# vlc-robot/robot-3dlotus

Measured on AMD Instinct MI355X. Metric: keystep-samples/sec (train fwd+bwd) 3D-LOTUS GemBench, higher is better.
Workload: dtype f32; 1 GPU; 3D-LOTUS v1 (68.18M params), 16 key-step clouds x 4096 pts per GPU, fwd+loss+bwd, train mode (dropout on), fp32 exact (MFMA f32); global_batch=16, parallelism=dp1, rccl_ranks=0

## Files before the change

### include/lotus_hip.h

```cpp
#ifndef LOTUS_HIP_H
#define LOTUS_HIP_H
#include <stddef.h>
#ifdef __cplusplus
extern "C" {
#endif

#define LOTUS_OK 0
#define LOTUS_E_ARG (-1)
#define LOTUS_E_LAUNCH (-2)
#define LOTUS_E_UNSUPPORTED (-3)
#define LOTUS_E_WORKSPACE (-4)
#ifdef LOTUS_ACT_BF16
typedef unsigned short lotus_act_t;
#else
typedef float lotus_act_t;
#endif

#define LOTUS_ACT_NONE 0
#define LOTUS_ACT_GELU 1
#define LOTUS_ACT_LEAKY 2

const char* lotus_last_error(void);
int lotus_abi_version(void);

unsigned long long lotus_streamlink_create(int nevents);
int lotus_streamlink_wait(unsigned long long link, void* from_stream, void* to_stream);
int lotus_streamlink_destroy(unsigned long long link);

int lotus_comm_load(const char* path);
int lotus_comm_version(void);
int lotus_comm_unique_id(void* id128_host);
unsigned long long lotus_comm_create(const void* id128_host, int nranks, int rank);
int lotus_comm_allreduce(unsigned long long comm, void* buf, size_t count, int dtype, int op, void* stream);
int lotus_comm_destroy(unsigned long long comm);
int lotus_stream_probe(void* blocked, void* other, int timeout_ms);


int lotus_fe_grid(const float* coord, long ld, int n, float grid_size, int* grid, int* gmax, unsigned* scratch,
                  void* stream);
int lotus_fe_encode(const int* grid, const int* batch, int n, const int* gmax, const int* perm4, int depth_bound,
                    int* state, long long* code, long slot_stride, void* stream);
size_t lotus_fe_sort_workspace(int n_max);
int lotus_fe_sort(const long long* code, long slot_stride, const int* n_ptr, int n_max, int key_bits,
                  long long* skeys, int* order, int* inverse, void* workspace, size_t workspace_bytes, void* stream);
int lotus_fe_pool(const long long* pcode, const long long* skey0, const int* order0, const int* pgrid,
                  const int* pbatch, const int* n_ptr, int n_max, const int* perm4, int nbatch, int* cluster,
                  int* seg_start, int* n_child, long long* ccode, int* cgrid, int* cbatch, int* ccounts,
                  int* n_dup, void* stream);
int lotus_fe_pool_coord(const float* pcoord, const int* order0, const int* seg_start, int n_child, float* ccoord,
                        void* stream);
int lotus_fe_patch(const int* order, const int* off, const int* offp, int B, int K, int npad, int* gidx, int* owner,
                   int* kext, int* ext_pos, void* stream);
size_t lotus_fe_neighbours_workspace(int n);
int lotus_fe_neighbours(const int* grid, const int* batch, int n, int ksize, int* nbr, void* workspace,
                        size_t workspace_bytes, void* stream);
size_t lotus_fe_tap_plan_ints(int n);
int lotus_fe_tap_plan(const int* nbr27, const int* rowidx, int n, int* plan, void* stream);

size_t lotus_linear_workspace(int M, int N, int K);
size_t lotus_splitk_counters_bytes(void);
int lotus_linear_fwd(const lotus_act_t* x, const float* w, const float* bias, const lotus_act_t* residual, lotus_act_t* y,
                     lotus_act_t* pre, int M, int N, int K, int act, float drop_p, unsigned long long drop_seed,
                     int precision, void* workspace, size_t workspace_bytes, void* counters, void* stream);
int lotus_linear_dgrad(const lotus_act_t* dy, const float* w, lotus_act_t* dx, const lotus_act_t* pre, const lotus_act_t* add, int M,
                       int N, int K, int act, float drop_p, unsigned long long drop_seed, int precision, void* workspace,
                       size_t workspace_bytes, void* counters, void* stream);
size_t lotus_linear_wgrad_workspace(int M, int N, int K);
int lotus_linear_wgrad(const lotus_act_t* dy, const lotus_act_t* x, float* dw, float* db, int M, int N, int K,
                       int accumulate, int precision, void* workspace, size_t workspace_bytes, void* counters,
                       void* stream);

size_t lotus_subm_conv_workspace(int n, int cin, int cout);
int lotus_conv_tap_eligible(int n, int cin, int cout);
int lotus_conv_weight_transpose(const float* w, float* w_t, int cout, int T, int cin, int precision, void* stream);
int lotus_subm_conv(int mode, const lotus_act_t* x, const float* w, const float* w_t, const float* bias, const lotus_act_t* add,
                    lotus_act_t* y, const int* nbr, const int* rowidx, int n, int T, int cin, int cout, int precision,
                    const int* tap_plan, void* workspace, size_t workspace_bytes, void* stream);
int lotus_conv_dup_fold(const lotus_act_t* dy, const long long* code0, const int* order0, int n, int C, lotus_act_t* dyr,
                        void* stream);
int lotus_conv_dup_mask(lotus_act_t* dx, const lotus_act_t* add, const int* rep, int n, int C, void* stream);
size_t lotus_subm_conv_wgrad_workspace(int n, int T, int cin, int cout);
int lotus_subm_conv_wgrad(const lotus_act_t* dy, const lotus_act_t* x, float* dw, float* db, const int* nbr, int n, int T,
                          int cin, int cout, int accumulate, int precision, void* workspace, size_t workspace_bytes,
                          void* stream);

int lotus_layernorm_fwd(const lotus_act_t* x, const lotus_act_t* res, const float* gamma, const float* beta, lotus_act_t* y,
                        float* mean, float* rstd, int M, int C, float eps, void* stream);
size_t lotus_layernorm_bwd_workspace(int M, int C);
int lotus_layernorm_bwd(const lotus_act_t* dy, const lotus_act_t* x, const float* mean, const float* rstd, const float* gamma,
                        const lotus_act_t* add, lotus_act_t* dx, float* dgamma, float* dbeta, int M, int C, int accumulate,
                        lotus_act_t* dz, float drop_p, unsigned long long drop_seed, void* workspace, size_t workspace_bytes,
                        void* stream);
int lotus_layernorm_bwd_parts(int M, int C);
int lotus_layernorm_bwd_params_n(const void* workspace, int nparts, int C, float* dgamma, float* dbeta, int accumulate, void* stream);
int lotus_linear_dgrad_ln(const lotus_act_t* dy, const float* w, const lotus_act_t* x, const float* mean, const float* rstd,
                          const float* gamma, const lotus_act_t* add, lotus_act_t* dx, lotus_act_t* dn, lotus_act_t* dz, float dz_p,
                          unsigned long long dz_seed, int M, int N, int K, int precision, void* workspace, size_t workspace_bytes,
                          void* counters, void* ln_workspace, size_t ln_workspace_bytes, int* nparts, void* stream);
int lotus_layernorm_bwd_params(const void* workspace, int M, int C, float* dgamma, float* dbeta, int accumulate,
                               void* stream);
size_t lotus_batchnorm_workspace(int M, int C);
int lotus_batchnorm_stats(const lotus_act_t* x, double* sums, int M, int C, void* workspace, size_t workspace_bytes,
                          void* stream);
int lotus_batchnorm_finalize(const double* sums, float* mean, float* invstd, float* running_mean,
                             float* running_var, int C, float eps, float momentum, void* stream);
size_t lotus_bn_counters_offset(void);
int lotus_batchnorm_stats_fused(const lotus_act_t* x, double* sums, float* mean, float* invstd, float* running_mean, float* running_var,
                                int M, int C, float eps, float momentum, void* workspace, size_t workspace_bytes, void* counter,
                                void* stream);
int lotus_batchnorm_bwd_stats_fused(const lotus_act_t* dy, const lotus_act_t* x, const float* mean, const float* invstd, const float* gamma,
                                    const float* beta, double* sums, int M, int C, int act, void* workspace, size_t workspace_bytes,
                                    void* counter, void* stream);
int lotus_batchnorm_bwd_stats_fused_params(const lotus_act_t* dy, const lotus_act_t* x, const float* mean, const float* invstd,
                                           const float* gamma, const float* beta, double* sums, float* dgamma, float* dbeta, int M,
                                           int C, int act, void* workspace, size_t workspace_bytes, void* counter, void* stream);
int lotus_batchnorm_eval_stats(const float* running_mean, const float* running_var, float* mean, float* invstd, int C,
                               float eps, void* stream);
int lotus_batchnorm_apply(const lotus_act_t* x, const float* mean, const float* invstd, const float* gamma,
                          const float* beta, lotus_act_t* y, int M, int C, int act, void* stream);
int lotus_batchnorm_apply_sums(const lotus_act_t* x, const double* sums, const float* gamma, const float* beta, lotus_act_t* y,
                               float* mean, float* invstd, float* running_mean, float* running_var, int M, int C, int act,
                               float eps, float momentum, void* stream);
int lotus_batchnorm_bwd_stats(const lotus_act_t* dy, const lotus_act_t* x, const float* mean, const float* invstd,
                              const float* gamma, const float* beta, double* sums, int M, int C, int act,
                              void* workspace, size_t workspace_bytes, void* stream);
int lotus_batchnorm_bwd_apply(const lotus_act_t* dy, const lotus_act_t* x, const float* mean, const float* invstd,
                              const float* gamma, const float* beta, const double* sums, lotus_act_t* dx, float* dgamma,
                              float* dbeta, int M, int C, int act, int train, int accumulate, void* stream);

int lotus_attention_fwd(const lotus_act_t* q, long q_ld, int q_off, const lotus_act_t* kv, long kv_ld, int k_off, int v_off,
                        const int* qidx, const int* kidx, const int* owner, const int* tiles, int ntiles,
                        const float* qn_w, const float* qn_b, const float* kn_w, const float* kn_b, lotus_act_t* out,
                        long out_ld, float* lse, int H, int d, float scale, float eps, float drop_p,
                        unsigned long long drop_seed, int precision, int k_max, void* stream);
size_t lotus_attention_bwd_workspace(int nblocks, int H);
int lotus_attention_bwd(const lotus_act_t* q, long q_ld, int q_off, const lotus_act_t* kv, long kv_ld, int k_off, int v_off,
                        const int* qidx, const int* kidx, const int* owner, const int* tiles, const int* blocks,
                        int nblocks, const float* qn_w, const float* qn_b, const float* kn_w, const float* kn_b,
                        const lotus_act_t* out, const lotus_act_t* dout, long out_ld, const float* lse, lotus_act_t* dq, long dq_ld,
                        int dq_off, lotus_act_t* dkv, long dkv_ld, int dk_off, int dv_off, long dkv_part_stride,
                        int atomic_out, const int* kext, const int* ext_pos, int n_extra, lotus_act_t* dkv_extra, float* dqn_w, float* dqn_b, float* dkn_w, float* dkn_b, int accumulate,
                        int H, int d, float scale, float eps, float drop_p, unsigned long long drop_seed,
                        int precision, int k_max, void* workspace, size_t workspace_bytes, void* stream);

size_t lotus_ffn_saved_floats(int M, int C, int Hd);
size_t lotus_ffn_grads_floats(int C, int Hd);
size_t lotus_ffn_tmp_floats(int M, int C, int Hd);
size_t lotus_ffn_ws_main_bytes(int M, int C, int Hd);
size_t lotus_ffn_ws_side_bytes(int M, int C, int Hd);
int lotus_ffn_fwd(const lotus_act_t* x, const float* g, const float* b, const float* w1, const float* b1, const float* w2,
                  const float* b2, lotus_act_t* y, float* saved, int M, int C, int Hd, float drop_p, unsigned long long seed1,
                  unsigned long long seed2, int precision, void* ws, size_t ws_bytes, void* counters, void* stream);
int lotus_ffn_bwd(const lotus_act_t* dy, const lotus_act_t* dz_in, const lotus_act_t* x, const float* g, const float* w1, const float* w2,
                  const float* saved, lotus_act_t* dx, lotus_act_t* dz_out, float dz_out_p, unsigned long long dz_out_seed, float* grads,
                  float* tmp, int M, int C, int Hd, float drop_p, unsigned long long seed1, unsigned long long seed2,
                  int precision, void* ws_main, size_t ws_main_bytes, void* ws_side, size_t ws_side_bytes, void* counters_main,
                  void* counters_side, unsigned long long link, int join, void* stream, void* side);

size_t lotus_selfattn_saved_floats(int M, int C, int H, int npad);
size_t lotus_selfattn_grads_floats(int C, int H);
size_t lotus_selfattn_tmp_floats(int M, int C, int n_extra);
size_t lotus_selfattn_ws_main_bytes(int M, int C, int H, int nblocks);
size_t lotus_selfattn_ws_side_bytes(int M, int C);
int lotus_selfattn_fwd(const lotus_act_t* x, const float* g, const float* b, const float* wqkv, const float* bqkv, const float* qnw,
                       const float* qnb, const float* knw, const float* knb, const float* wp, const float* bp, lotus_act_t* y,
                       float* saved, const int* gidx, const int* owner, const int* tiles, int ntiles, int npad, int M, int C,
                       int H, float scale, float drop_p, unsigned long long seed, float attn_p, unsigned long long attn_seed,
                       int precision, void* ws, size_t ws_bytes, void* counters, void* stream);
int lotus_selfattn_bwd(const lotus_act_t* dy, const lotus_act_t* dz_in, const lotus_act_t* x, const float* g, const float* wqkv, const float* qnw,
                       const float* qnb, const float* knw, const float* knb, const float* wp, const float* saved, lotus_act_t* dx,
                       float* grads, float* tmp, const int* gidx, const int* owner, const int* tiles, const int* blocks, int nblocks,
                       const int* kext, const int* ext_pos, int n_extra, int npad, int M, int C, int H, float scale, float drop_p,
                       unsigned long long seed, float attn_p, unsigned long long attn_seed, int precision, void* ws_main,
                       size_t ws_main_bytes, void* ws_side, size_t ws_side_bytes, void* counters_main, void* counters_side,
                       unsigned long long link, int join, void* stream, void* side);
size_t lotus_crossattn_saved_floats(int M, int C, int H, int L);
size_t lotus_crossattn_grads_floats(int C, int H, int Cc);
size_t lotus_crossattn_tmp_floats(int M, int C, int L, int G);
size_t lotus_crossattn_ws_main_bytes(int M, int C, int H, int L, int Cc, int nblocks);
size_t lotus_crossattn_ws_side_bytes(int M, int C, int L, int Cc);
int lotus_crossattn_fwd(const lotus_act_t* x, const lotus_act_t* context, const float* g, const float* b, const float* wq, const float* bq,
// ... 148 lines not shown
```

### include/lotus_hip_b16.h

```cpp
#ifndef LOTUS_HIP_B16_H
#define LOTUS_HIP_B16_H
#include <stddef.h>
#include "lotus_hip.h"
#ifdef __cplusplus
extern "C" {
#endif

typedef unsigned short lotus_bf16_t;

size_t lotus_b16_linear_workspace(int M, int N, int K);
size_t lotus_b16_splitk_counters_bytes(void);
int lotus_b16_linear_fwd(const lotus_bf16_t* x, const float* w, const float* bias, const lotus_bf16_t* residual, lotus_bf16_t* y, lotus_bf16_t* pre, int M, int N, int K, int act, float drop_p, unsigned long long drop_seed, int precision, void* workspace, size_t workspace_bytes, void* counters, void* stream);
int lotus_b16_linear_dgrad(const lotus_bf16_t* dy, const float* w, lotus_bf16_t* dx, const lotus_bf16_t* pre, const lotus_bf16_t* add, int M, int N, int K, int act, float drop_p, unsigned long long drop_seed, int precision, void* workspace, size_t workspace_bytes, void* counters, void* stream);
size_t lotus_b16_linear_wgrad_workspace(int M, int N, int K);
int lotus_b16_linear_wgrad(const lotus_bf16_t* dy, const lotus_bf16_t* x, float* dw, float* db, int M, int N, int K, int accumulate, int precision, void* workspace, size_t workspace_bytes, void* counters, void* stream);
size_t lotus_b16_subm_conv_workspace(int n, int cin, int cout);
int lotus_b16_conv_tap_eligible(int n, int cin, int cout);
int lotus_b16_conv_weight_transpose(const float* w, float* w_t, int cout, int T, int cin, int precision, void* stream);
int lotus_b16_subm_conv(int mode, const lotus_bf16_t* x, const float* w, const float* w_t, const float* bias, const lotus_bf16_t* add, lotus_bf16_t* y, const int* nbr, const int* rowidx, int n, int T, int cin, int cout, int precision, const int* tap_plan, void* workspace, size_t workspace_bytes, void* stream);
int lotus_b16_conv_dup_fold(const lotus_bf16_t* dy, const long long* code0, const int* order0, int n, int C, lotus_bf16_t* dyr, void* stream);
int lotus_b16_conv_dup_mask(lotus_bf16_t* dx, const lotus_bf16_t* add, const int* rep, int n, int C, void* stream);
size_t lotus_b16_subm_conv_wgrad_workspace(int n, int T, int cin, int cout);
int lotus_b16_subm_conv_wgrad(const lotus_bf16_t* dy, const lotus_bf16_t* x, float* dw, float* db, const int* nbr, int n, int T, int cin, int cout, int accumulate, int precision, void* workspace, size_t workspace_bytes, void* stream);
int lotus_b16_layernorm_fwd(const lotus_bf16_t* x, const lotus_bf16_t* res, const float* gamma, const float* beta, lotus_bf16_t* y, float* mean, float* rstd, int M, int C, float eps, void* stream);
size_t lotus_b16_layernorm_bwd_workspace(int M, int C);
int lotus_b16_layernorm_bwd(const lotus_bf16_t* dy, const lotus_bf16_t* x, const float* mean, const float* rstd, const float* gamma, const lotus_bf16_t* add, lotus_bf16_t* dx, float* dgamma, float* dbeta, int M, int C, int accumulate, lotus_bf16_t* dz, float drop_p, unsigned long long drop_seed, void* workspace, size_t workspace_bytes, void* stream);
int lotus_b16_layernorm_bwd_parts(int M, int C);
int lotus_b16_layernorm_bwd_params_n(const void* workspace, int nparts, int C, float* dgamma, float* dbeta, int accumulate, void* stream);
int lotus_b16_linear_dgrad_ln(const lotus_bf16_t* dy, const float* w, const lotus_bf16_t* x, const float* mean, const float* rstd, const float* gamma, const lotus_bf16_t* add, lotus_bf16_t* dx, lotus_bf16_t* dn, lotus_bf16_t* dz, float dz_p, unsigned long long dz_seed, int M, int N, int K, int precision, void* workspace, size_t workspace_bytes, void* counters, void* ln_workspace, size_t ln_workspace_bytes, int* nparts, void* stream);
int lotus_b16_layernorm_bwd_params(const void* workspace, int M, int C, float* dgamma, float* dbeta, int accumulate, void* stream);
size_t lotus_b16_batchnorm_workspace(int M, int C);
int lotus_b16_batchnorm_stats(const lotus_bf16_t* x, double* sums, int M, int C, void* workspace, size_t workspace_bytes, void* stream);
int lotus_b16_batchnorm_finalize(const double* sums, float* mean, float* invstd, float* running_mean, float* running_var, int C, float eps, float momentum, void* stream);
size_t lotus_b16_bn_counters_offset(void);
int lotus_b16_batchnorm_stats_fused(const lotus_bf16_t* x, double* sums, float* mean, float* invstd, float* running_mean, float* running_var, int M, int C, float eps, float momentum, void* workspace, size_t workspace_bytes, void* counter, void* stream);
int lotus_b16_batchnorm_bwd_stats_fused(const lotus_bf16_t* dy, const lotus_bf16_t* x, const float* mean, const float* invstd, const float* gamma, const float* beta, double* sums, int M, int C, int act, void* workspace, size_t workspace_bytes, void* counter, void* stream);
int lotus_b16_batchnorm_bwd_stats_fused_params(const lotus_bf16_t* dy, const lotus_bf16_t* x, const float* mean, const float* invstd, const float* gamma, const float* beta, double* sums, float* dgamma, float* dbeta, int M, int C, int act, void* workspace, size_t workspace_bytes, void* counter, void* stream);
int lotus_b16_batchnorm_eval_stats(const float* running_mean, const float* running_var, float* mean, float* invstd, int C, float eps, void* stream);
int lotus_b16_batchnorm_apply(const lotus_bf16_t* x, const float* mean, const float* invstd, const float* gamma, const float* beta, lotus_bf16_t* y, int M, int C, int act, void* stream);
int lotus_b16_batchnorm_apply_sums(const lotus_bf16_t* x, const double* sums, const float* gamma, const float* beta, lotus_bf16_t* y, float* mean, float* invstd, float* running_mean, float* running_var, int M, int C, int act, float eps, float momentum, void* stream);
int lotus_b16_batchnorm_bwd_stats(const lotus_bf16_t* dy, const lotus_bf16_t* x, const float* mean, const float* invstd, const float* gamma, const float* beta, double* sums, int M, int C, int act, void* workspace, size_t workspace_bytes, void* stream);
int lotus_b16_batchnorm_bwd_apply(const lotus_bf16_t* dy, const lotus_bf16_t* x, const float* mean, const float* invstd, const float* gamma, const float* beta, const double* sums, lotus_bf16_t* dx, float* dgamma, float* dbeta, int M, int C, int act, int train, int accumulate, void* stream);
int lotus_b16_attention_fwd(const lotus_bf16_t* q, long q_ld, int q_off, const lotus_bf16_t* kv, long kv_ld, int k_off, int v_off, const int* qidx, const int* kidx, const int* owner, const int* tiles, int ntiles, const float* qn_w, const float* qn_b, const float* kn_w, const float* kn_b, lotus_bf16_t* out, long out_ld, float* lse, int H, int d, float scale, float eps, float drop_p, unsigned long long drop_seed, int precision, int k_max, void* stream);
size_t lotus_b16_attention_bwd_workspace(int nblocks, int H);
int lotus_b16_attention_bwd(const lotus_bf16_t* q, long q_ld, int q_off, const lotus_bf16_t* kv, long kv_ld, int k_off, int v_off, const int* qidx, const int* kidx, const int* owner, const int* tiles, const int* blocks, int nblocks, const float* qn_w, const float* qn_b, const float* kn_w, const float* kn_b, const lotus_bf16_t* out, const lotus_bf16_t* dout, long out_ld, const float* lse, lotus_bf16_t* dq, long dq_ld, int dq_off, lotus_bf16_t* dkv, long dkv_ld, int dk_off, int dv_off, long dkv_part_stride, int atomic_out, const int* kext, const int* ext_pos, int n_extra, lotus_bf16_t* dkv_extra, float* dqn_w, float* dqn_b, float* dkn_w, float* dkn_b, int accumulate, int H, int d, float scale, float eps, float drop_p, unsigned long long drop_seed, int precision, int k_max, void* workspace, size_t workspace_bytes, void* stream);
size_t lotus_b16_ffn_saved_floats(int M, int C, int Hd);
size_t lotus_b16_ffn_grads_floats(int C, int Hd);
size_t lotus_b16_ffn_tmp_floats(int M, int C, int Hd);
size_t lotus_b16_ffn_ws_main_bytes(int M, int C, int Hd);
size_t lotus_b16_ffn_ws_side_bytes(int M, int C, int Hd);
int lotus_b16_ffn_fwd(const lotus_bf16_t* x, const float* g, const float* b, const float* w1, const float* b1, const float* w2, const float* b2, lotus_bf16_t* y, float* saved, int M, int C, int Hd, float drop_p, unsigned long long seed1, unsigned long long seed2, int precision, void* ws, size_t ws_bytes, void* counters, void* stream);
int lotus_b16_ffn_bwd(const lotus_bf16_t* dy, const lotus_bf16_t* dz_in, const lotus_bf16_t* x, const float* g, const float* w1, const float* w2, const float* saved, lotus_bf16_t* dx, lotus_bf16_t* dz_out, float dz_out_p, unsigned long long dz_out_seed, float* grads, float* tmp, int M, int C, int Hd, float drop_p, unsigned long long seed1, unsigned long long seed2, int precision, void* ws_main, size_t ws_main_bytes, void* ws_side, size_t ws_side_bytes, void* counters_main, void* counters_side, unsigned long long link, int join, void* stream, void* side);
size_t lotus_b16_selfattn_saved_floats(int M, int C, int H, int npad);
size_t lotus_b16_selfattn_grads_floats(int C, int H);
size_t lotus_b16_selfattn_tmp_floats(int M, int C, int n_extra);
size_t lotus_b16_selfattn_ws_main_bytes(int M, int C, int H, int nblocks);
size_t lotus_b16_selfattn_ws_side_bytes(int M, int C);
int lotus_b16_selfattn_fwd(const lotus_bf16_t* x, const float* g, const float* b, const float* wqkv, const float* bqkv, const float* qnw, const float* qnb, const float* knw, const float* knb, const float* wp, const float* bp, lotus_bf16_t* y, float* saved, const int* gidx, const int* owner, const int* tiles, int ntiles, int npad, int M, int C, int H, float scale, float drop_p, unsigned long long seed, float attn_p, unsigned long long attn_seed, int precision, void* ws, size_t ws_bytes, void* counters, void* stream);
int lotus_b16_selfattn_bwd(const lotus_bf16_t* dy, const lotus_bf16_t* dz_in, const lotus_bf16_t* x, const float* g, const float* wqkv, const float* qnw, const float* qnb, const float* knw, const float* knb, const float* wp, const float* saved, lotus_bf16_t* dx, float* grads, float* tmp, const int* gidx, const int* owner, const int* tiles, const int* blocks, int nblocks, const int* kext, const int* ext_pos, int n_extra, int npad, int M, int C, int H, float scale, float drop_p, unsigned long long seed, float attn_p, unsigned long long attn_seed, int precision, void* ws_main, size_t ws_main_bytes, void* ws_side, size_t ws_side_bytes, void* counters_main, void* counters_side, unsigned long long link, int join, void* stream, void* side);
size_t lotus_b16_crossattn_saved_floats(int M, int C, int H, int L);
size_t lotus_b16_crossattn_grads_floats(int C, int H, int Cc);
size_t lotus_b16_crossattn_tmp_floats(int M, int C, int L, int G);
size_t lotus_b16_crossattn_ws_main_bytes(int M, int C, int H, int L, int Cc, int nblocks);
size_t lotus_b16_crossattn_ws_side_bytes(int M, int C, int L, int Cc);
int lotus_b16_crossattn_fwd(const lotus_bf16_t* x, const lotus_bf16_t* context, const float* g, const float* b, const float* wq, const float* bq, const float* wkv, const float* bkv, const float* qnw, const float* qnb, const float* knw, const float* knb, const float* wp, const float* bp, lotus_bf16_t* y, float* saved, const int* tiles, int ntiles, int M, int C, int H, int L, int Cc, float scale, float drop_p, unsigned long long seed, float attn_p, unsigned long long attn_seed, int precision, int k_max, void* ws, size_t ws_bytes, void* counters, void* stream);
int lotus_b16_crossattn_bwd(const lotus_bf16_t* dy, const lotus_bf16_t* dz_in, const lotus_bf16_t* x, const lotus_bf16_t* context, const float* g, const float* wq, const float* wkv, const float* qnw, const float* qnb, const float* knw, const float* knb, const float* wp, const float* saved, lotus_bf16_t* dx, lotus_bf16_t* dctx, lotus_bf16_t* dz_out, float dz_out_p, unsigned long long dz_out_seed, float* grads, float* tmp, const int* tiles, const int* blocks, int nblocks, int G, int M, int C, int H, int L, int Cc, float scale, float drop_p, unsigned long long seed, float attn_p, unsigned long long attn_seed, int precision, int k_max, void* ws_main, size_t ws_main_bytes, void* ws_side, size_t ws_side_bytes, void* counters_main, void* counters_side, unsigned long long link, int join, void* stream, void* side);
size_t lotus_b16_cpe_saved_floats(int n, int C);
size_t lotus_b16_cpe_grads_floats(int C);
size_t lotus_b16_cpe_tmp_floats(int n, int C);
size_t lotus_b16_cpe_ws_main_bytes(int n, int C);
size_t lotus_b16_cpe_ws_conv_bytes(int n, int C);
size_t lotus_b16_cpe_ws_side_bytes(int n, int C);
int lotus_b16_cpe_fwd(const lotus_bf16_t* x, const lotus_bf16_t* xs, const float* cw, const float* cw_packed, const float* cb, const float* lw, const float* lb, const float* g, const float* b, lotus_bf16_t* y, float* saved, const int* nbr27, const int* order0, const int* tap_plan, int n, int C, int precision, void* ws, size_t ws_bytes, void* ws_conv, size_t ws_conv_bytes, void* counters, void* stream);
int lotus_b16_cpe_bwd(const lotus_bf16_t* dy, const lotus_bf16_t* xs, const float* cw, const float* cw_packed, const float* lw, const float* g, const float* saved, lotus_bf16_t* dx_conv, int add_dy, float* grads, float* tmp, const int* nbr27, const int* order0, const int* tap_plan, const long long* code0, int n_dup, int n, int C, int precision, void* ws_main, size_t ws_main_bytes, void* ws_conv, size_t ws_conv_bytes, void* ws_side, size_t ws_side_bytes, void* counters_main, void* counters_side, unsigned long long link, int join, void* stream, void* side);
size_t lotus_b16_pair_acts_floats(int M, int C);
size_t lotus_b16_pair_saved_floats(int M, int C, int H, int Hd, int npad);
size_t lotus_b16_pair_grads_floats(int C, int H, int Hd);
size_t lotus_b16_pair_tmp_floats(int M, int C, int Hd, int n_extra, int L, int G);
size_t lotus_b16_pair_ws_main_bytes(int M, int C, int H, int Hd, int nblocks_self, int nblocks_ca);
size_t lotus_b16_pair_ws_side_bytes(int M, int C, int Hd);
size_t lotus_b16_pair_ws_conv_bytes(int M, int C);
int lotus_b16_pair_nptr(void);
int lotus_b16_pair_nint(void);
int lotus_b16_pair_fwd(const void* const* P, const long long* I, const double* F);
int lotus_b16_pair_bwd(const void* const* P, const long long* I, const double* F);
int lotus_b16_sum_slabs(const lotus_bf16_t* part, lotus_bf16_t* out, long n, long stride, int nz, void* stream);
int lotus_b16_sum_slabs_ld(const lotus_bf16_t* part, lotus_bf16_t* out, int rows, int cols, long out_ld, long stride, int nz, void* stream);
size_t lotus_b16_crossattn_kv_saved_floats(int M, int C, int H);
size_t lotus_b16_crossattn_kv_grads_floats(int C, int H);
size_t lotus_b16_crossattn_kv_tmp_floats(int M, int C, int L, int G);
size_t lotus_b16_crossattn_kv_ws_main_bytes(int M, int C, int H, int nblocks);
size_t lotus_b16_crossattn_kv_ws_side_bytes(int M, int C);
int lotus_b16_crossattn_kv_fwd(const lotus_bf16_t* x, const lotus_bf16_t* kv, long kv_ld, const float* g, const float* b, const float* wq, const float* bq, const float* qnw, const float* qnb, const float* knw, const float* knb, const float* wp, const float* bp, lotus_bf16_t* y, float* saved, const int* tiles, int ntiles, int M, int C, int H, float scale, float drop_p, unsigned long long seed, float attn_p, unsigned long long attn_seed, int precision, int k_max, void* ws, size_t ws_bytes, void* counters, void* stream);
int lotus_b16_crossattn_kv_bwd(const lotus_bf16_t* dy, const lotus_bf16_t* dz_in, const lotus_bf16_t* x, const lotus_bf16_t* kv, long kv_ld, const float* g, const float* wq, const float* qnw, const float* qnb, const float* knw, const float* knb, const float* wp, const float* saved, lotus_bf16_t* dx, lotus_bf16_t* dkv, long dkv_ld, lotus_bf16_t* dz_out, float dz_out_p, unsigned long long dz_out_seed, float* grads, float* tmp, const int* tiles, const int* blocks, int nblocks, int G, int M, int C, int H, int L, float scale, float drop_p, unsigned long long seed, float attn_p, unsigned long long attn_seed, int precision, int k_max, void* ws_main, size_t ws_main_bytes, void* ws_side, size_t ws_side_bytes, void* counters_main, void* counters_side, unsigned long long link, int join, void* stream, void* side);
int lotus_b16_pool_max_fwd(const lotus_bf16_t* x, const int* members, const int* seg, int nc, int C, lotus_bf16_t* y, int* arg, void* stream);
int lotus_b16_pool_max_bwd(const lotus_bf16_t* dy, const int* arg, const int* cluster, int n, int C, lotus_bf16_t* dx, void* stream);
int lotus_b16_unpool_fwd(const lotus_bf16_t* skip, const lotus_bf16_t* up, const int* cluster, int n, int C, lotus_bf16_t* x, void* stream);
int lotus_b16_unpool_bwd(const lotus_bf16_t* dx, const int* members, const int* seg, int nc, int C, lotus_bf16_t* dup, void* stream);
size_t lotus_b16_cloud_max_workspace(int B, int C);
int lotus_b16_cloud_max_fwd(const lotus_bf16_t* x, const int* off, int B, int C, lotus_bf16_t* y, int* arg, void* workspace, size_t workspace_bytes, void* stream);
int lotus_b16_cloud_max_bwd(const lotus_bf16_t* dy, const int* arg, const int* batch, int n, int C, const lotus_bf16_t* add, lotus_bf16_t* dx, void* stream);
size_t lotus_b16_loss_stats_floats(int B);
int lotus_b16_loss_fwd(const lotus_bf16_t* xt, const lotus_bf16_t* ae, const float* tgt, const float* gt, const int* off, int B, int nb, int nrot, int ga, float pos_w, float rot_w, float* losses, float* pos_stats, float* dae, void* stream);
int lotus_b16_loss_bwd(const lotus_bf16_t* xt, const float* tgt, const int* off, const int* batch, const float* pos_stats, const float* dae_saved, const float* gl, float pos_w, float rot_w, int B, int n, int nb, int nrot, lotus_bf16_t* dxt, lotus_bf16_t* dae_out, void* stream);
int lotus_b16_pos_ce_fwd(const lotus_bf16_t* xt, const float* tgt, const int* off, int B, int nb, float* pos_stats, void* stream);
int lotus_b16_pos_ce_bwd(const lotus_bf16_t* xt, const float* tgt, const int* off, const int* batch, const float* pos_stats, const float* g, int B, int n, int nb, lotus_bf16_t* dxt, void* stream);
int lotus_b16_mp_loss_fwd(const lotus_bf16_t* ae, const float* gt, const float* stop, const float* mask, const float* ce, int B, int T, int nrot, int ga, float pos_w, float rot_w, float* losses, float* dae, float* dce, void* stream);
int lotus_b16_mp_loss_bwd(const float* dae, const float* dce, const float* g, float pos_w, float rot_w, int B, int T, int nrot, lotus_bf16_t* dae_out, float* dce_out, void* stream);
int lotus_b16_step_act_fwd(const lotus_bf16_t* base, const float* bias, lotus_bf16_t* out, int M, int C, int act, float drop_p, unsigned long long drop_seed, void* stream);
size_t lotus_b16_step_act_bwd_workspace(int M, int C);
int lotus_b16_step_act_bwd(const lotus_bf16_t* dh, const lotus_bf16_t* base, const float* bias, lotus_bf16_t* dbase, float* dbias, int M, int C, int act, float drop_p, unsigned long long drop_seed, int accumulate, void* workspace, size_t workspace_bytes, void* stream);
int lotus_b16_add(const lotus_bf16_t* a, const lotus_bf16_t* b, lotus_bf16_t* y, long n, void* stream);
// ... 11 lines not shown
```

### robot-3dlotus_amd/csrc/blocks.cpp

```cpp
#include <stddef.h>
#include <stdint.h>

#include <hip/hip_runtime.h>

#include "../../include/lotus_hip.h"

extern __attribute__((visibility("hidden"))) __thread hipEvent_t lotus_tls_stop_event;
hipEvent_t lotus_link_next_event(unsigned long long link);
void lotus_set_error(const char* fmt, ...);

#define CHECK(x)        \
  do {                  \
    int rc_ = (x);      \
    if (rc_) return rc_; \
  } while (0)

static inline size_t al4(size_t n) { return (n + 3) & ~(size_t)3; }

typedef lotus_act_t act_t;
static inline size_t actf(size_t n) { return al4((n * sizeof(act_t) + 3) / 4); }
struct Carve {
  char* p;
  explicit Carve(const void* base) : p((char*)base) {}
  act_t* act(size_t n) { act_t* r = (act_t*)p; p += actf(n) * 4; return r; }
  float* f32(size_t n) { float* r = (float*)p; p += al4(n) * 4; return r; }
};

static inline int noshadow(int precision) { return precision == 5 ? 1 : precision; }

static inline int fork_side(unsigned long long link, void* main_s, void* side) {
  return side ? lotus_streamlink_wait(link, main_s, side) : 0;
}

struct ForkAfter {
  hipEvent_t ev;
  void* side;
  ForkAfter(unsigned long long link, void* side_) : ev(side_ ? lotus_link_next_event(link) : nullptr), side(side_) {
    lotus_tls_stop_event = ev;
  }
  ~ForkAfter() { lotus_tls_stop_event = nullptr; }
  int wait() {
    lotus_tls_stop_event = nullptr;
    if (!side) return 0;
    hipError_t e = hipStreamWaitEvent((hipStream_t)side, ev, 0);
    if (e != hipSuccess) {
      lotus_set_error("lotus composite: hipStreamWaitEvent: %s", hipGetErrorString(e));
      return LOTUS_E_LAUNCH;
    }
    return 0;
  }
};
#define PRODUCE_THEN_FORK(call) \
  do {                          \
    ForkAfter fa_(link, side);  \
    CHECK(call);                \
    CHECK(fa_.wait());          \
  } while (0)

static int dgrad_ln(const act_t* dyl, const float* w, act_t* dn, const act_t* x, const float* mean, const float* rstd, const float* g,
                    const act_t* add, act_t* dx, act_t* dz, float dz_p, unsigned long long dz_seed, float* dg, float* db, int M, int N,
                    int C, int precision, void* ws, size_t ws_bytes, void* counters, float* lnp, size_t lnp_bytes,
                    unsigned long long link, void* stream, void* side) {
  int nparts = 0;
  act_t* dzo = dz_p > 0.f ? dz : nullptr;
  if (side) {
    PRODUCE_THEN_FORK(lotus_linear_dgrad_ln(dyl, w, x, mean, rstd, g, add, dx, dn, dzo, dz_p, dz_seed, M, N, C, precision, ws, ws_bytes,
                                            counters, lnp, lnp_bytes, &nparts, stream));
    CHECK(lotus_layernorm_bwd_params_n(lnp, nparts, C, dg, db, 0, side));
  } else {
    CHECK(lotus_linear_dgrad_ln(dyl, w, x, mean, rstd, g, add, dx, dn, dzo, dz_p, dz_seed, M, N, C, precision, ws, ws_bytes, counters, lnp,
                                lnp_bytes, &nparts, stream));
    CHECK(lotus_layernorm_bwd_params_n(lnp, nparts, C, dg, db, 0, stream));
  }
  return LOTUS_OK;
}

extern "C" {

size_t lotus_ffn_saved_floats(int M, int C, int Hd) { return actf((size_t)M * C) + 2 * actf((size_t)M * Hd) + 2 * al4((size_t)M); }
size_t lotus_ffn_grads_floats(int C, int Hd) { return 2 * al4(C) + al4((size_t)Hd * C + Hd) + al4((size_t)C * Hd + C); }
size_t lotus_ffn_tmp_floats(int M, int C, int Hd) {
  return 2 * actf((size_t)M * C) + actf((size_t)M * Hd) + lotus_layernorm_bwd_workspace(M, C) / sizeof(float);
}
size_t lotus_ffn_ws_main_bytes(int M, int C, int Hd) {
  const size_t a = lotus_linear_workspace(M, Hd, C), b = lotus_linear_workspace(M, C, Hd);
  return a > b ? a : b;
}
size_t lotus_ffn_ws_side_bytes(int M, int C, int Hd) {
  const size_t a = lotus_linear_wgrad_workspace(M, Hd, C), b = lotus_linear_wgrad_workspace(M, C, Hd);
  return a > b ? a : b;
}

int lotus_ffn_fwd(const act_t* x, const float* g, const float* b, const float* w1, const float* b1, const float* w2,
                  const float* b2, act_t* y, float* saved, int M, int C, int Hd, float drop_p, unsigned long long seed1,
                  unsigned long long seed2, int precision, void* ws, size_t ws_bytes, void* counters, void* stream) {
  Carve sv(saved);
  act_t* n = sv.act((size_t)M * C);
  act_t* hpre = sv.act((size_t)M * Hd);
  act_t* a = sv.act((size_t)M * Hd);
  float* mean = sv.f32(M);
  float* rstd = sv.f32(M);
  const bool big = M > 8192;
  CHECK(lotus_layernorm_fwd(x, nullptr, g, b, n, mean, rstd, M, C, 1e-5f, stream));
  CHECK(lotus_linear_fwd(n, w1, b1, nullptr, a, hpre, M, Hd, C, LOTUS_ACT_GELU, drop_p, seed1, precision, big ? nullptr : ws,
                         big ? 0 : ws_bytes, big ? nullptr : counters, stream));
  return lotus_linear_fwd(a, w2, b2, x, y, nullptr, M, C, Hd, LOTUS_ACT_NONE, drop_p, seed2, precision, big ? nullptr : ws,
                          big ? 0 : ws_bytes, big ? nullptr : counters, stream);
}

int lotus_ffn_bwd(const act_t* dy, const act_t* dz_in, const act_t* x, const float* g, const float* w1, const float* w2,
                  const float* saved, act_t* dx, act_t* dz_out, float dz_out_p, unsigned long long dz_out_seed, float* grads,
                  float* tmp, int M, int C, int Hd, float drop_p, unsigned long long seed1, unsigned long long seed2,
                  int precision, void* ws_main, size_t ws_main_bytes, void* ws_side, size_t ws_side_bytes, void* counters_main,
                  void* counters_side, unsigned long long link, int join, void* stream, void* side) {
  Carve sv(saved);
  const act_t* n = sv.act((size_t)M * C);
  const act_t* hpre = sv.act((size_t)M * Hd);
  const act_t* a = sv.act((size_t)M * Hd);
  const float* mean = sv.f32(M);
  const float* rstd = sv.f32(M);
  float* dg = grads;
  float* db = dg + al4(C);
  float* dw1 = db + al4(C);
  float* db1 = dw1 + (size_t)Hd * C;
  float* dw2 = dw1 + al4((size_t)Hd * C + Hd);
  float* db2 = dw2 + (size_t)C * Hd;
  Carve tp(tmp);
  act_t* dz2 = tp.act((size_t)M * C);
  act_t* dh = tp.act((size_t)M * Hd);
  act_t* dn = tp.act((size_t)M * C);
  float* lnp = tp.f32(0);
  const size_t lnp_bytes = lotus_layernorm_bwd_workspace(M, C);
  void* sw = side ? side : stream;
  void* wws = side ? ws_side : ws_main;
  const size_t wws_bytes = side ? ws_side_bytes : ws_main_bytes;
  void* wcnt = side ? counters_side : counters_main;
  const bool big = M > 8192;
  const act_t* dz = dz_in;
  if (!dz) {
    if (drop_p > 0.f) {
      PRODUCE_THEN_FORK(lotus_dropout(dy, dz2, (long)M * C, drop_p, seed2, stream));
      dz = dz2;
    } else {
      dz = dy;
      CHECK(fork_side(link, stream, side));
    }
  }
  CHECK(lotus_linear_wgrad(dz, a, dw2, db2, M, C, Hd, 0, precision, wws, wws_bytes, wcnt, sw));
  PRODUCE_THEN_FORK(lotus_linear_dgrad(dz, w2, dh, hpre, nullptr, M, C, Hd, LOTUS_ACT_GELU, drop_p, seed1, precision,
                                       big ? nullptr : ws_main, big ? 0 : ws_main_bytes, big ? nullptr : counters_main, stream));
  CHECK(lotus_linear_wgrad(dh, n, dw1, db1, M, Hd, C, 0, precision, wws, wws_bytes, wcnt, sw));
  CHECK(dgrad_ln(dh, w1, dn, x, mean, rstd, g, dy, dx, dz_out, dz_out_p, dz_out_seed, dg, db, M, Hd, C, precision, big ? nullptr : ws_main,
                 big ? 0 : ws_main_bytes, big ? nullptr : counters_main, lnp, lnp_bytes, link, stream, side));
  if (side && join) CHECK(lotus_streamlink_wait(link, side, stream));
  return LOTUS_OK;
}

size_t lotus_selfattn_saved_floats(int M, int C, int H, int npad) {
  return 2 * actf((size_t)M * C) + actf((size_t)M * 3 * C) + al4((size_t)npad * H) + 2 * al4((size_t)M);
}
size_t lotus_selfattn_grads_floats(int C, int H) {
  return 2 * al4(C) + al4((size_t)3 * C * C + 3 * C) + 4 * al4(C / H) + al4((size_t)C * C + C);
}
size_t lotus_selfattn_tmp_floats(int M, int C, int n_extra) {
  return 3 * actf((size_t)M * C) + actf((size_t)M * 3 * C) + actf((size_t)(n_extra > 1 ? n_extra : 1) * 2 * C) +
         lotus_layernorm_bwd_workspace(M, C) / sizeof(float);
}
size_t lotus_selfattn_ws_main_bytes(int M, int C, int H, int nblocks) {
  size_t a = lotus_linear_workspace(M, 3 * C, C), b = lotus_linear_workspace(M, C, C), c = lotus_attention_bwd_workspace(nblocks, H);
  if (b > a) a = b;
  return c > a ? c : a;
}
size_t lotus_selfattn_ws_side_bytes(int M, int C) {
  const size_t a = lotus_linear_wgrad_workspace(M, 3 * C, C), b = lotus_linear_wgrad_workspace(M, C, C);
  return a > b ? a : b;
}

int lotus_selfattn_fwd(const act_t* x, const float* g, const float* b, const float* wqkv, const float* bqkv, const float* qnw,
                       const float* qnb, const float* knw, const float* knb, const float* wp, const float* bp, act_t* y,
                       float* saved, const int* gidx, const int* owner, const int* tiles, int ntiles, int npad, int M, int C,
                       int H, float scale, float drop_p, unsigned long long seed, float attn_p, unsigned long long attn_seed,
                       int precision, void* ws, size_t ws_bytes, void* counters, void* stream) {
  const int d = C / H;
  Carve sv(saved);
  act_t* n = sv.act((size_t)M * C);
  act_t* qkv = sv.act((size_t)M * 3 * C);
  act_t* att = sv.act((size_t)M * C);
  float* lse = sv.f32((size_t)npad * H);
  float* mean = sv.f32(M);
  float* rstd = sv.f32(M);
  const bool big = M > 8192;
  CHECK(lotus_layernorm_fwd(x, nullptr, g, b, n, mean, rstd, M, C, 1e-5f, stream));
  CHECK(lotus_linear_fwd(n, wqkv, bqkv, nullptr, qkv, nullptr, M, 3 * C, C, LOTUS_ACT_NONE, 0.f, 0, precision, big ? nullptr : ws,
                         big ? 0 : ws_bytes, big ? nullptr : counters, stream));
  CHECK(lotus_attention_fwd(qkv, 3L * C, 0, qkv, 3L * C, C, 2 * C, gidx, gidx, owner, tiles, ntiles, qnw, qnb, knw, knb, att, (long)C, lse,
                            H, d, scale, 1e-6f, attn_p, attn_seed, noshadow(precision), 0, stream));
  return lotus_linear_fwd(att, wp, bp, x, y, nullptr, M, C, C, LOTUS_ACT_NONE, drop_p, seed, precision, big ? nullptr : ws,
                          big ? 0 : ws_bytes, big ? nullptr : counters, stream);
}

int lotus_selfattn_bwd(const act_t* dy, const act_t* dz_in, const act_t* x, const float* g, const float* wqkv, const float* qnw,
                       const float* qnb, const float* knw, const float* knb, const float* wp, const float* saved, act_t* dx,
                       float* grads, float* tmp, const int* gidx, const int* owner, const int* tiles, const int* blocks, int nblocks,
                       const int* kext, const int* ext_pos, int n_extra, int npad, int M, int C, int H, float scale, float drop_p,
                       unsigned long long seed, float attn_p, unsigned long long attn_seed, int precision, void* ws_main,
                       size_t ws_main_bytes, void* ws_side, size_t ws_side_bytes, void* counters_main, void* counters_side,
                       unsigned long long link, int join, void* stream, void* side) {
  const int d = C / H;
  Carve sv(saved);
  const act_t* n = sv.act((size_t)M * C);
  const act_t* qkv = sv.act((size_t)M * 3 * C);
  const act_t* att = sv.act((size_t)M * C);
  const float* lse = sv.f32((size_t)npad * H);
  const float* mean = sv.f32(M);
  const float* rstd = sv.f32(M);
  float* dg = grads;
  float* db = dg + al4(C);
  float* dwqkv = db + al4(C);
  float* dbqkv = dwqkv + (size_t)3 * C * C;
  float* gq = dwqkv + al4((size_t)3 * C * C + 3 * C);
  float* bq = gq + al4(d);
  float* gk = bq + al4(d);
  float* bk = gk + al4(d);
  float* dwp = bk + al4(d);
  float* dbp = dwp + (size_t)C * C;
  Carve tp(tmp);
  act_t* dzb = tp.act((size_t)M * C);
  act_t* datt = tp.act((size_t)M * C);
  act_t* dqkv = tp.act((size_t)M * 3 * C);
  act_t* extra = tp.act((size_t)(n_extra > 1 ? n_extra : 1) * 2 * C);
  act_t* dn = tp.act((size_t)M * C);
  float* lnp = tp.f32(0);
  const size_t lnp_bytes = lotus_layernorm_bwd_workspace(M, C);
  void* sw = side ? side : stream;
  void* wws = side ? ws_side : ws_main;
  const size_t wws_bytes = side ? ws_side_bytes : ws_main_bytes;
  void* wcnt = side ? counters_side : counters_main;
  const bool big = M > 8192;
  const act_t* dz = dz_in;
  if (!dz) {
    if (drop_p > 0.f) {
      PRODUCE_THEN_FORK(lotus_dropout(dy, dzb, (long)M * C, drop_p, seed, stream));
      dz = dzb;
    } else {
      dz = dy;
      CHECK(fork_side(link, stream, side));
    }
  }
  CHECK(lotus_linear_wgrad(dz, att, dwp, dbp, M, C, C, 0, precision, wws, wws_bytes, wcnt, sw));
  CHECK(lotus_linear_dgrad(dz, wp, datt, nullptr, nullptr, M, C, C, LOTUS_ACT_NONE, 0.f, 0, precision, big ? nullptr : ws_main,
                           big ? 0 : ws_main_bytes, big ? nullptr : counters_main, stream));
  PRODUCE_THEN_FORK(lotus_attention_bwd(qkv, 3L * C, 0, qkv, 3L * C, C, 2 * C, gidx, gidx, owner, tiles, blocks, nblocks, qnw, qnb, knw, knb,
                                        att, datt, (long)C, lse, dqkv, 3L * C, 0, dqkv, 3L * C, C, 2 * C, 0, 0, kext, ext_pos, n_extra, extra,
                                        gq, bq, gk, bk, 0, H, d, scale, 1e-6f, attn_p, attn_seed, noshadow(precision), 0, ws_main, ws_main_bytes, stream));
  CHECK(lotus_linear_wgrad(dqkv, n, dwqkv, dbqkv, M, 3 * C, C, 0, precision, wws, wws_bytes, wcnt, sw));
  CHECK(dgrad_ln(dqkv, wqkv, dn, x, mean, rstd, g, dy, dx, nullptr, 0.f, 0, dg, db, M, 3 * C, C, precision, big ? nullptr : ws_main,
                 big ? 0 : ws_main_bytes, big ? nullptr : counters_main, lnp, lnp_bytes, link, stream, side));
  if (side && join) CHECK(lotus_streamlink_wait(link, side, stream));
  return LOTUS_OK;
}

size_t lotus_crossattn_saved_floats(int M, int C, int H, int L) {
  return 3 * actf((size_t)M * C) + actf((size_t)L * 2 * C) + al4((size_t)M * H) + 2 * al4((size_t)M);
}
size_t lotus_crossattn_grads_floats(int C, int H, int Cc) {
  return 2 * al4(C) + 2 * al4((size_t)C * C + C) + al4((size_t)2 * C * Cc + 2 * C) + 4 * al4(C / H);
}
size_t lotus_crossattn_tmp_floats(int M, int C, int L, int G) {
  return 4 * actf((size_t)M * C) + actf((size_t)G * L * 2 * C) + actf((size_t)L * 2 * C) + lotus_layernorm_bwd_workspace(M, C) / sizeof(float);
}
size_t lotus_crossattn_ws_main_bytes(int M, int C, int H, int L, int Cc, int nblocks) {
  size_t a = lotus_linear_workspace(M, C, C), b = lotus_linear_workspace(L, 2 * C, Cc), c = lotus_attention_bwd_workspace(nblocks, H);
  if (b > a) a = b;
  return c > a ? c : a;
}
size_t lotus_crossattn_ws_side_bytes(int M, int C, int L, int Cc) {
  const size_t a = lotus_linear_wgrad_workspace(M, C, C), b = lotus_linear_wgrad_workspace(L, 2 * C, Cc);
  return a > b ? a : b;
}

int lotus_crossattn_fwd(const act_t* x, const act_t* context, const float* g, const float* b, const float* wq, const float* bq,
                        const float* wkv, const float* bkv, const float* qnw, const float* qnb, const float* knw, const float* knb,
                        const float* wp, const float* bp, act_t* y, float* saved, const int* tiles, int ntiles, int M, int C, int H,
                        int L, int Cc, float scale, float drop_p, unsigned long long seed, float attn_p, unsigned long long attn_seed,
                        int precision, int k_max, void* ws, size_t ws_bytes, void* counters, void* stream) {
  const int d = C / H;
  Carve sv(saved);
  act_t* n = sv.act((size_t)M * C);
  act_t* q = sv.act((size_t)M * C);
  act_t* kv = sv.act((size_t)L * 2 * C);
  act_t* att = sv.act((size_t)M * C);
  float* lse = sv.f32((size_t)M * H);
  float* mean = sv.f32(M);
  float* rstd = sv.f32(M);
  const bool big = M > 8192, bigL = L > 8192;
  CHECK(lotus_layernorm_fwd(x, nullptr, g, b, n, mean, rstd, M, C, 1e-5f, stream));
  CHECK(lotus_linear_fwd(n, wq, bq, nullptr, q, nullptr, M, C, C, LOTUS_ACT_NONE, 0.f, 0, precision, big ? nullptr : ws, big ? 0 : ws_bytes,
                         big ? nullptr : counters, stream));
  CHECK(lotus_linear_fwd(context, wkv, bkv, nullptr, kv, nullptr, L, 2 * C, Cc, LOTUS_ACT_NONE, 0.f, 0, precision, bigL ? nullptr : ws,
                         bigL ? 0 : ws_bytes, bigL ? nullptr : counters, stream));
  CHECK(lotus_attention_fwd(q, (long)C, 0, kv, 2L * C, 0, C, nullptr, nullptr, nullptr, tiles, ntiles, qnw, qnb, knw, knb, att, (long)C, lse, H,
                            d, scale, 1e-6f, attn_p, attn_seed, noshadow(precision), k_max, stream));
  return lotus_linear_fwd(att, wp, bp, x, y, nullptr, M, C, C, LOTUS_ACT_NONE, drop_p, seed, precision, big ? nullptr : ws,
                          big ? 0 : ws_bytes, big ? nullptr : counters, stream);
}

int lotus_crossattn_bwd(const act_t* dy, const act_t* dz_in, const act_t* x, const act_t* context, const float* g, const float* wq,
                        const float* wkv, const float* qnw, const float* qnb, const float* knw, const float* knb, const float* wp,
                        const float* saved, act_t* dx, act_t* dctx, act_t* dz_out, float dz_out_p, unsigned long long dz_out_seed,
                        float* grads, float* tmp, const int* tiles, const int* blocks, int nblocks, int G, int M, int C, int H, int L,
                        int Cc, float scale, float drop_p, unsigned long long seed, float attn_p, unsigned long long attn_seed,
                        int precision, int k_max, void* ws_main, size_t ws_main_bytes, void* ws_side, size_t ws_side_bytes, void* counters_main,
                        void* counters_side, unsigned long long link, int join, void* stream, void* side) {
  const int d = C / H;
  Carve sv(saved);
  const act_t* n = sv.act((size_t)M * C);
  const act_t* q = sv.act((size_t)M * C);
  const act_t* kv = sv.act((size_t)L * 2 * C);
  const act_t* att = sv.act((size_t)M * C);
  const float* lse = sv.f32((size_t)M * H);
  const float* mean = sv.f32(M);
  const float* rstd = sv.f32(M);
  float* dg = grads;
  float* db = dg + al4(C);
  float* dwq = db + al4(C);
  float* dbq = dwq + (size_t)C * C;
  float* dwkv = dwq + al4((size_t)C * C + C);
  float* dbkv = dwkv + (size_t)2 * C * Cc;
  float* gq = dwkv + al4((size_t)2 * C * Cc + 2 * C);
  float* bq_ = gq + al4(d);
  float* gk = bq_ + al4(d);
  float* bk_ = gk + al4(d);
  float* dwp = bk_ + al4(d);
  float* dbp = dwp + (size_t)C * C;
  Carve tp(tmp);
  act_t* dzb = tp.act((size_t)M * C);
  act_t* datt = tp.act((size_t)M * C);
  act_t* dq = tp.act((size_t)M * C);
  act_t* dkv_part = tp.act((size_t)G * L * 2 * C);
  act_t* dkv = tp.act((size_t)L * 2 * C);
  act_t* dn = tp.act((size_t)M * C);
  float* lnp = tp.f32(0);
// ... 69 lines not shown
  CHECK(lotus_layernorm_fwd(x, nullptr, g, b, n, mean, rstd, M, C, 1e-5f, stream));
  CHECK(lotus_linear_fwd(n, wq, bq, nullptr, q, nullptr, M, C, C, LOTUS_ACT_NONE, 0.f, 0, precision, big ? nullptr : ws, big ? 0 : ws_bytes,
                         big ? nullptr : counters, stream));
  CHECK(lotus_attention_fwd(q, (long)C, 0, kv, kv_ld, 0, C, nullptr, nullptr, nullptr, tiles, ntiles, qnw, qnb, knw, knb, att, (long)C, lse, H,
                            d, scale, 1e-6f, attn_p, attn_seed, noshadow(precision), k_max, stream));
  return lotus_linear_fwd(att, wp, bp, x, y, nullptr, M, C, C, LOTUS_ACT_NONE, drop_p, seed, precision, big ? nullptr : ws,
                          big ? 0 : ws_bytes, big ? nullptr : counters, stream);
}

int lotus_crossattn_kv_bwd(const act_t* dy, const act_t* dz_in, const act_t* x, const act_t* kv, long kv_ld, const float* g,
                           const float* wq, const float* qnw, const float* qnb, const float* knw, const float* knb, const float* wp,
                           const float* saved, act_t* dx, act_t* dkv, long dkv_ld, act_t* dz_out, float dz_out_p,
                           unsigned long long dz_out_seed, float* grads, float* tmp, const int* tiles, const int* blocks, int nblocks,
                           int G, int M, int C, int H, int L, float scale, float drop_p, unsigned long long seed, float attn_p,
                           unsigned long long attn_seed, int precision, int k_max, void* ws_main, size_t ws_main_bytes, void* ws_side,
                           size_t ws_side_bytes, void* counters_main, void* counters_side, unsigned long long link, int join,
                           void* stream, void* side) {
  const int d = C / H;
  Carve sv(saved);
  const act_t* n = sv.act((size_t)M * C);
  const act_t* q = sv.act((size_t)M * C);
  const act_t* att = sv.act((size_t)M * C);
  const float* lse = sv.f32((size_t)M * H);
  const float* mean = sv.f32(M);
  const float* rstd = sv.f32(M);
  float* dg = grads;
  float* db = dg + al4(C);
  float* dwq = db + al4(C);
  float* dbq = dwq + (size_t)C * C;
  float* gq = dwq + al4((size_t)C * C + C);
  float* bq_ = gq + al4(d);
  float* gk = bq_ + al4(d);
  float* bk_ = gk + al4(d);
  float* dwp = bk_ + al4(d);
  float* dbp = dwp + (size_t)C * C;
  Carve tp(tmp);
  act_t* dzb = tp.act((size_t)M * C);
  act_t* datt = tp.act((size_t)M * C);
  act_t* dq = tp.act((size_t)M * C);
  act_t* dkv_part = G > 1 ? tp.act((size_t)G * L * 2 * C) : nullptr;
  act_t* dn = tp.act((size_t)M * C);
  float* lnp = tp.f32(0);
  const size_t lnp_bytes = lotus_layernorm_bwd_workspace(M, C);
  void* sw = side ? side : stream;
  void* wws = side ? ws_side : ws_main;
  const size_t wws_bytes = side ? ws_side_bytes : ws_main_bytes;
  void* wcnt = side ? counters_side : counters_main;
  const bool big = M > 8192;
  const act_t* dz = dz_in;
  if (!dz) {
    if (drop_p > 0.f) {
      PRODUCE_THEN_FORK(lotus_dropout(dy, dzb, (long)M * C, drop_p, seed, stream));
      dz = dzb;
    } else {
      dz = dy;
      CHECK(fork_side(link, stream, side));
    }
  }
  CHECK(lotus_linear_wgrad(dz, att, dwp, dbp, M, C, C, 0, precision, wws, wws_bytes, wcnt, sw));
  CHECK(lotus_linear_dgrad(dz, wp, datt, nullptr, nullptr, M, C, C, LOTUS_ACT_NONE, 0.f, 0, precision, big ? nullptr : ws_main,
                           big ? 0 : ws_main_bytes, big ? nullptr : counters_main, stream));
  PRODUCE_THEN_FORK(lotus_attention_bwd(q, (long)C, 0, kv, kv_ld, 0, C, nullptr, nullptr, nullptr, tiles, blocks, nblocks, qnw, qnb, knw, knb,
                                        att, datt, (long)C, lse, dq, (long)C, 0, G > 1 ? dkv_part : dkv, G > 1 ? 2L * C : dkv_ld, 0, C,
                                        G > 1 ? (long)L * 2 * C : 0, 0, nullptr, nullptr, 0, nullptr, gq, bq_, gk, bk_, 0, H, d, scale,
                                        1e-6f, attn_p, attn_seed, noshadow(precision), k_max, ws_main, ws_main_bytes, stream));
  if (G > 1) CHECK(lotus_sum_slabs_ld(dkv_part, dkv, L, 2 * C, dkv_ld, (long)L * 2 * C, G, stream));
  CHECK(lotus_linear_wgrad(dq, n, dwq, dbq, M, C, C, 0, precision, wws, wws_bytes, wcnt, sw));
  CHECK(dgrad_ln(dq, wq, dn, x, mean, rstd, g, dy, dx, dz_out, dz_out_p, dz_out_seed, dg, db, M, C, C, precision, big ? nullptr : ws_main,
                 big ? 0 : ws_main_bytes, big ? nullptr : counters_main, lnp, lnp_bytes, link, stream, side));
  if (side && join) CHECK(lotus_streamlink_wait(link, side, stream));
  return LOTUS_OK;
}

size_t lotus_cpe_saved_floats(int n, int C) { return 2 * actf((size_t)n * C) + 2 * al4((size_t)n); }
size_t lotus_cpe_grads_floats(int C) { return 2 * al4(C) + al4((size_t)C * C + C) + al4((size_t)C * 27 * C + C); }
size_t lotus_cpe_tmp_floats(int n, int C) { return 3 * actf((size_t)n * C) + lotus_layernorm_bwd_workspace(n, C) / sizeof(float); }
size_t lotus_cpe_ws_main_bytes(int n, int C) { return lotus_linear_workspace(n, C, C); }
size_t lotus_cpe_ws_conv_bytes(int n, int C) { return lotus_subm_conv_workspace(n, C, C); }
size_t lotus_cpe_ws_side_bytes(int n, int C) {
  const size_t a = lotus_linear_wgrad_workspace(n, C, C), b = lotus_subm_conv_wgrad_workspace(n, 27, C, C);
  return a > b ? a : b;
}

int lotus_cpe_fwd(const act_t* x, const act_t* xs, const float* cw, const float* cw_packed, const float* cb, const float* lw,
                  const float* lb, const float* g, const float* b, act_t* y, float* saved, const int* nbr27, const int* order0,
                  const int* tap_plan, int n, int C, int precision, void* ws, size_t ws_bytes, void* ws_conv, size_t ws_conv_bytes, void* counters, void* stream) {
  Carve sv(saved);
  act_t* c = sv.act((size_t)n * C);
  act_t* l = sv.act((size_t)n * C);
  float* mean = sv.f32(n);
  float* rstd = sv.f32(n);
  const bool big = n > 8192;
  CHECK(lotus_subm_conv(0, xs, cw, cw_packed, cb, nullptr, c, nbr27, order0, n, 27, C, C, noshadow(precision), tap_plan, ws_conv, ws_conv_bytes, stream));
  CHECK(lotus_linear_fwd(c, lw, lb, nullptr, l, nullptr, n, C, C, LOTUS_ACT_NONE, 0.f, 0, precision, big ? nullptr : ws, big ? 0 : ws_bytes,
                         big ? nullptr : counters, stream));
  return lotus_layernorm_fwd(l, x, g, b, y, mean, rstd, n, C, 1e-5f, stream);
}

int lotus_cpe_bwd(const act_t* dy, const act_t* xs, const float* cw, const float* cw_packed, const float* lw, const float* g,
                  const float* saved, act_t* dx_conv, int add_dy, float* grads, float* tmp, const int* nbr27, const int* order0,
                  const int* tap_plan, const long long* code0, int n_dup, int n, int C, int precision, void* ws_main, size_t ws_main_bytes, void* ws_conv,
                  size_t ws_conv_bytes, void* ws_side, size_t ws_side_bytes, void* counters_main, void* counters_side,
                  unsigned long long link, int join, void* stream, void* side) {
  Carve sv(saved);
  const act_t* c = sv.act((size_t)n * C);
  const act_t* l = sv.act((size_t)n * C);
  const float* mean = sv.f32(n);
  const float* rstd = sv.f32(n);
  float* dg = grads;
  float* db = dg + al4(C);
  float* dlw = db + al4(C);
  float* dlb = dlw + (size_t)C * C;
  float* dcw = dlw + al4((size_t)C * C + C);
  float* dcb = dcw + (size_t)C * 27 * C;
  Carve tp(tmp);
  act_t* dl = tp.act((size_t)n * C);
  act_t* dc = tp.act((size_t)n * C);
  act_t* dyr = tp.act((size_t)n * C);
  float* lnp = tp.f32(0);
  const size_t lnp_bytes = lotus_layernorm_bwd_workspace(n, C);
  void* sw = side ? side : stream;
  void* wws = side ? ws_side : ws_main;
  const size_t wws_bytes = side ? ws_side_bytes : ws_main_bytes;
  void* wcnt = side ? counters_side : counters_main;
  const bool big = n > 8192;
  if (side) {
    PRODUCE_THEN_FORK(lotus_layernorm_bwd(dy, l, mean, rstd, g, nullptr, dl, nullptr, nullptr, n, C, 0, nullptr, 0.f, 0, lnp, lnp_bytes, stream));
    CHECK(lotus_layernorm_bwd_params(lnp, n, C, dg, db, 0, side));
  } else {
    CHECK(lotus_layernorm_bwd(dy, l, mean, rstd, g, nullptr, dl, dg, db, n, C, 0, nullptr, 0.f, 0, lnp, lnp_bytes, stream));
  }
  CHECK(lotus_linear_wgrad(dl, c, dlw, dlb, n, C, C, 0, precision, wws, wws_bytes, wcnt, sw));
  PRODUCE_THEN_FORK(lotus_linear_dgrad(dl, lw, dc, nullptr, nullptr, n, C, C, LOTUS_ACT_NONE, 0.f, 0, precision, big ? nullptr : ws_main,
                                       big ? 0 : ws_main_bytes, big ? nullptr : counters_main, stream));
  CHECK(lotus_subm_conv_wgrad(dc, xs, dcw, dcb, nbr27, n, 27, C, C, 0, noshadow(precision), wws, wws_bytes, sw));
  const act_t* dsrc = dc;
  if (n_dup != 0) {
    CHECK(lotus_conv_dup_fold(dc, code0, order0, n, C, dyr, stream));
    dsrc = dyr;
  }
  CHECK(lotus_subm_conv(1, dsrc, cw, cw_packed, nullptr, add_dy ? dy : nullptr, dx_conv, nbr27, order0, n, 27, C, C, noshadow(precision), tap_plan, ws_conv,
                        ws_conv_bytes, stream));
  if (n_dup != 0) CHECK(lotus_conv_dup_mask(dx_conv, add_dy ? dy : nullptr, nbr27 + (size_t)13 * n, n, C, stream));
  if (side && join) CHECK(lotus_streamlink_wait(link, side, stream));
  return LOTUS_OK;
}

enum PairPtr {
  PP_X, PP_XS, PP_KV, PP_Y, PP_ACTS, PP_SAVED, PP_CW, PP_CWP, PP_CB, PP_LW, PP_LB, PP_G0, PP_B0,
  PP_G1, PP_B1, PP_WQKV, PP_BQKV, PP_QNW, PP_QNB, PP_KNW, PP_KNB, PP_WP, PP_BP,
  PP_G2, PP_B2, PP_W1, PP_B1F, PP_W2, PP_B2F,
  PP_G3, PP_B3, PP_WQ, PP_BQ, PP_CQNW, PP_CQNB, PP_CKNW, PP_CKNB, PP_CWP2, PP_CBP2,
  PP_G4, PP_B4, PP_W3, PP_B3F, PP_W4, PP_B4F,
  PP_NBR27, PP_ORDER0, PP_TAPPLAN, PP_CODE0, PP_GIDX, PP_OWNER, PP_STILES, PP_SBLOCKS, PP_KEXT, PP_EXTPOS, PP_CATILES, PP_CABLOCKS,
  PP_WS_MAIN, PP_WS_SIDE, PP_WS_CONV, PP_CNT_MAIN, PP_CNT_SIDE, PP_STREAM, PP_SIDE,
  PP_DY, PP_DX, PP_DXS, PP_DKV, PP_GRADS, PP_TMP,
  PP_COUNT
};
enum PairInt {
  PI_M, PI_C, PI_H, PI_HD, PI_NPAD, PI_NSTILES, PI_NEXTRA, PI_L, PI_NCATILES, PI_NCABLOCKS, PI_G, PI_KMAX, PI_NDUP, PI_SAME,
  PI_PREC, PI_KV_LD, PI_DKV_LD, PI_WS_MAIN, PI_WS_SIDE, PI_WS_CONV, PI_LINK, PI_SEED_SELF, PI_SEED_FFN1, PI_SEED_CROSS, PI_SEED_FFN2,
  PI_COUNT
};
enum PairFlt { PF_DROP, PF_ATTN, PF_SCALE, PF_COUNT };

static inline unsigned long long pair_mix(unsigned long long seed, unsigned long long k) {
  unsigned long long z = seed + 0x9E3779B97F4A7C15ULL * (k + 1);
  z = (z ^ (z >> 30)) * 0xBF58476D1CE4E5B9ULL;
  z = (z ^ (z >> 27)) * 0x94D049BB133111EBULL;
  return z ^ (z >> 31);
}

static inline size_t al64(size_t n) { return (n + 63) & ~(size_t)63; }
size_t lotus_pair_acts_floats(int M, int C) { return 4 * al64(actf((size_t)M * C)); }
size_t lotus_pair_saved_floats(int M, int C, int H, int Hd, int npad) {
  return al64(lotus_cpe_saved_floats(M, C)) + al64(lotus_selfattn_saved_floats(M, C, H, npad)) + 2 * al64(lotus_ffn_saved_floats(M, C, Hd)) +
         al64(lotus_crossattn_kv_saved_floats(M, C, H));
}
size_t lotus_pair_grads_floats(int C, int H, int Hd) {
  return lotus_cpe_grads_floats(C) + lotus_selfattn_grads_floats(C, H) + 2 * lotus_ffn_grads_floats(C, Hd) + lotus_crossattn_kv_grads_floats(C, H);
}
size_t lotus_pair_tmp_floats(int M, int C, int Hd, int n_extra, int L, int G) {
  return al64(lotus_cpe_tmp_floats(M, C)) + al64(lotus_selfattn_tmp_floats(M, C, n_extra)) + 2 * al64(lotus_ffn_tmp_floats(M, C, Hd)) +
         al64(lotus_crossattn_kv_tmp_floats(M, C, L, G)) + 4 * al64(actf((size_t)M * C));
}
static inline size_t max3(size_t a, size_t b, size_t c) { return a > b ? (a > c ? a : c) : (b > c ? b : c); }
size_t lotus_pair_ws_main_bytes(int M, int C, int H, int Hd, int nblocks_self, int nblocks_ca) {
  return max3(max3(lotus_cpe_ws_main_bytes(M, C), lotus_selfattn_ws_main_bytes(M, C, H, nblocks_self), lotus_ffn_ws_main_bytes(M, C, Hd)),
              lotus_crossattn_kv_ws_main_bytes(M, C, H, nblocks_ca), 0);
}
size_t lotus_pair_ws_side_bytes(int M, int C, int Hd) {
  return max3(max3(lotus_cpe_ws_side_bytes(M, C), lotus_selfattn_ws_side_bytes(M, C), lotus_ffn_ws_side_bytes(M, C, Hd)),
              lotus_crossattn_kv_ws_side_bytes(M, C), 0);
}
size_t lotus_pair_ws_conv_bytes(int M, int C) { return lotus_cpe_ws_conv_bytes(M, C); }
int lotus_pair_nptr(void) { return PP_COUNT; }
int lotus_pair_nint(void) { return PI_COUNT; }

#define PPTR(T, i) ((T)P[i])
int lotus_pair_fwd(const void* const* P, const long long* I, const double* F) {
  const int M = (int)I[PI_M], C = (int)I[PI_C], H = (int)I[PI_H], Hd = (int)I[PI_HD], npad = (int)I[PI_NPAD];
  const int prec = (int)I[PI_PREC];
  const float drop = (float)F[PF_DROP], attn_p = (float)F[PF_ATTN], scale = (float)F[PF_SCALE];
  void* ws = PPTR(void*, PP_WS_MAIN);
  const size_t ws_b = (size_t)I[PI_WS_MAIN];
  void* cnt = PPTR(void*, PP_CNT_MAIN);
  void* st = PPTR(void*, PP_STREAM);
  const size_t a = al64(actf((size_t)M * C));
  float* acts = PPTR(float*, PP_ACTS);
  act_t* x1 = (act_t*)acts;
  act_t* x2 = (act_t*)(acts + a);
  act_t* x3 = (act_t*)(acts + 2 * a);
  act_t* x4 = (act_t*)(acts + 3 * a);
  float* sv_cpe = PPTR(float*, PP_SAVED);
  float* sv_self = sv_cpe + al64(lotus_cpe_saved_floats(M, C));
  float* sv_ffn1 = sv_self + al64(lotus_selfattn_saved_floats(M, C, H, npad));
  float* sv_cross = sv_ffn1 + al64(lotus_ffn_saved_floats(M, C, Hd));
  float* sv_ffn2 = sv_cross + al64(lotus_crossattn_kv_saved_floats(M, C, H));
  const unsigned long long s_self = (unsigned long long)I[PI_SEED_SELF], s_f1 = (unsigned long long)I[PI_SEED_FFN1];
  const unsigned long long s_cross = (unsigned long long)I[PI_SEED_CROSS], s_f2 = (unsigned long long)I[PI_SEED_FFN2];
  CHECK(lotus_cpe_fwd(PPTR(const act_t*, PP_X), PPTR(const act_t*, PP_XS), PPTR(const float*, PP_CW), PPTR(const float*, PP_CWP),
                      PPTR(const float*, PP_CB), PPTR(const float*, PP_LW), PPTR(const float*, PP_LB), PPTR(const float*, PP_G0),
                      PPTR(const float*, PP_B0), x1, sv_cpe, PPTR(const int*, PP_NBR27), PPTR(const int*, PP_ORDER0), PPTR(const int*, PP_TAPPLAN), M, C, prec, ws, ws_b,
                      PPTR(void*, PP_WS_CONV), (size_t)I[PI_WS_CONV], cnt, st));
  CHECK(lotus_selfattn_fwd(x1, PPTR(const float*, PP_G1), PPTR(const float*, PP_B1), PPTR(const float*, PP_WQKV), PPTR(const float*, PP_BQKV),
                           PPTR(const float*, PP_QNW), PPTR(const float*, PP_QNB), PPTR(const float*, PP_KNW), PPTR(const float*, PP_KNB),
                           PPTR(const float*, PP_WP), PPTR(const float*, PP_BP), x2, sv_self, PPTR(const int*, PP_GIDX),
                           PPTR(const int*, PP_OWNER), PPTR(const int*, PP_STILES), (int)I[PI_NSTILES], npad, M, C, H, scale, drop, s_self,
                           attn_p, pair_mix(s_self, 1), prec, ws, ws_b, cnt, st));
  CHECK(lotus_ffn_fwd(x2, PPTR(const float*, PP_G2), PPTR(const float*, PP_B2), PPTR(const float*, PP_W1), PPTR(const float*, PP_B1F),
                      PPTR(const float*, PP_W2), PPTR(const float*, PP_B2F), x3, sv_ffn1, M, C, Hd, drop, s_f1, pair_mix(s_f1, 1), prec, ws,
                      ws_b, cnt, st));
  CHECK(lotus_crossattn_kv_fwd(x3, PPTR(const act_t*, PP_KV), (long)I[PI_KV_LD], PPTR(const float*, PP_G3), PPTR(const float*, PP_B3),
                               PPTR(const float*, PP_WQ), PPTR(const float*, PP_BQ), PPTR(const float*, PP_CQNW), PPTR(const float*, PP_CQNB),
                               PPTR(const float*, PP_CKNW), PPTR(const float*, PP_CKNB), PPTR(const float*, PP_CWP2),
                               PPTR(const float*, PP_CBP2), x4, sv_cross, PPTR(const int*, PP_CATILES), (int)I[PI_NCATILES], M, C, H, scale,
                               drop, s_cross, attn_p, pair_mix(s_cross, 1), prec, (int)I[PI_KMAX], ws, ws_b, cnt, st));
  return lotus_ffn_fwd(x4, PPTR(const float*, PP_G4), PPTR(const float*, PP_B4), PPTR(const float*, PP_W3), PPTR(const float*, PP_B3F),
                       PPTR(const float*, PP_W4), PPTR(const float*, PP_B4F), PPTR(act_t*, PP_Y), sv_ffn2, M, C, Hd, drop, s_f2,
                       pair_mix(s_f2, 1), prec, ws, ws_b, cnt, st);
}

int lotus_pair_bwd(const void* const* P, const long long* I, const double* F) {
  const int M = (int)I[PI_M], C = (int)I[PI_C], H = (int)I[PI_H], Hd = (int)I[PI_HD], npad = (int)I[PI_NPAD];
  const int n_extra = (int)I[PI_NEXTRA], L = (int)I[PI_L], G = (int)I[PI_G], prec = (int)I[PI_PREC];
  const float drop = (float)F[PF_DROP], attn_p = (float)F[PF_ATTN], scale = (float)F[PF_SCALE];
  void* wm = PPTR(void*, PP_WS_MAIN);
  void* wsd = PPTR(void*, PP_WS_SIDE);
  const size_t wm_b = (size_t)I[PI_WS_MAIN], wsd_b = (size_t)I[PI_WS_SIDE];
  void* cm = PPTR(void*, PP_CNT_MAIN);
  void* cs = PPTR(void*, PP_CNT_SIDE);
  void* st = PPTR(void*, PP_STREAM);
  void* side = PPTR(void*, PP_SIDE);
  const unsigned long long link = (unsigned long long)I[PI_LINK];
  const size_t a = al64(actf((size_t)M * C));
  float* acts = PPTR(float*, PP_ACTS);
  const act_t* x1 = (const act_t*)acts;
  const act_t* x2 = (const act_t*)(acts + a);
  const act_t* x3 = (const act_t*)(acts + 2 * a);
  const act_t* x4 = (const act_t*)(acts + 3 * a);
  const float* sv_cpe = PPTR(const float*, PP_SAVED);
  const float* sv_self = sv_cpe + al64(lotus_cpe_saved_floats(M, C));
  const float* sv_ffn1 = sv_self + al64(lotus_selfattn_saved_floats(M, C, H, npad));
  const float* sv_cross = sv_ffn1 + al64(lotus_ffn_saved_floats(M, C, Hd));
  const float* sv_ffn2 = sv_cross + al64(lotus_crossattn_kv_saved_floats(M, C, H));
  float* g_cpe = PPTR(float*, PP_GRADS);
  float* g_self = g_cpe + lotus_cpe_grads_floats(C);
  float* g_ffn1 = g_self + lotus_selfattn_grads_floats(C, H);
  float* g_cross = g_ffn1 + lotus_ffn_grads_floats(C, Hd);
  float* g_ffn2 = g_cross + lotus_crossattn_kv_grads_floats(C, H);
  float* t_cpe = PPTR(float*, PP_TMP);
  float* t_self = t_cpe + al64(lotus_cpe_tmp_floats(M, C));
  float* t_ffn1 = t_self + al64(lotus_selfattn_tmp_floats(M, C, n_extra));
  float* t_cross = t_ffn1 + al64(lotus_ffn_tmp_floats(M, C, Hd));
  float* t_ffn2 = t_cross + al64(lotus_crossattn_kv_tmp_floats(M, C, L, G));
  float* t_rest = t_ffn2 + al64(lotus_ffn_tmp_floats(M, C, Hd));
  act_t* d4 = (act_t*)t_rest;
  act_t* d3 = (act_t*)(t_rest + a);
  act_t* d2 = (act_t*)(t_rest + 2 * a);
  act_t* dz_cross = (act_t*)t_cross;
  act_t* dz_ffn1 = (act_t*)t_ffn1;
  act_t* dz_self = (act_t*)t_self;
  const unsigned long long s_self = (unsigned long long)I[PI_SEED_SELF], s_f1 = (unsigned long long)I[PI_SEED_FFN1];
  const unsigned long long s_cross = (unsigned long long)I[PI_SEED_CROSS], s_f2 = (unsigned long long)I[PI_SEED_FFN2];
  const bool hand = drop > 0.f;
  const int same = (int)I[PI_SAME];
  act_t* d1 = same ? (act_t*)(t_rest + 3 * a) : PPTR(act_t*, PP_DX);
  CHECK(lotus_ffn_bwd(PPTR(const act_t*, PP_DY), nullptr, x4, PPTR(const float*, PP_G4), PPTR(const float*, PP_W3), PPTR(const float*, PP_W4),
                      sv_ffn2, d4, hand ? dz_cross : nullptr, hand ? drop : 0.f, s_cross, g_ffn2, t_ffn2, M, C, Hd, drop, s_f2, pair_mix(s_f2, 1),
                      prec, wm, wm_b, wsd, wsd_b, cm, cs, link, 0, st, side));
  CHECK(lotus_crossattn_kv_bwd(d4, hand ? dz_cross : nullptr, x3, PPTR(const act_t*, PP_KV), (long)I[PI_KV_LD], PPTR(const float*, PP_G3),
                               PPTR(const float*, PP_WQ), PPTR(const float*, PP_CQNW), PPTR(const float*, PP_CQNB), PPTR(const float*, PP_CKNW),
                               PPTR(const float*, PP_CKNB), PPTR(const float*, PP_CWP2), sv_cross, d3, PPTR(act_t*, PP_DKV), (long)I[PI_DKV_LD],
                               hand ? dz_ffn1 : nullptr, hand ? drop : 0.f, pair_mix(s_f1, 1), g_cross, t_cross, PPTR(const int*, PP_CATILES),
                               PPTR(const int*, PP_CABLOCKS), (int)I[PI_NCABLOCKS], G, M, C, H, L, scale, drop, s_cross, attn_p,
                               pair_mix(s_cross, 1), prec, (int)I[PI_KMAX], wm, wm_b, wsd, wsd_b, cm, cs, link, 0, st, side));
  CHECK(lotus_ffn_bwd(d3, hand ? dz_ffn1 : nullptr, x2, PPTR(const float*, PP_G2), PPTR(const float*, PP_W1), PPTR(const float*, PP_W2), sv_ffn1,
                      d2, hand ? dz_self : nullptr, hand ? drop : 0.f, s_self, g_ffn1, t_ffn1, M, C, Hd, drop, s_f1, pair_mix(s_f1, 1), prec, wm,
                      wm_b, wsd, wsd_b, cm, cs, link, 0, st, side));
  CHECK(lotus_selfattn_bwd(d2, hand ? dz_self : nullptr, x1, PPTR(const float*, PP_G1), PPTR(const float*, PP_WQKV), PPTR(const float*, PP_QNW),
                           PPTR(const float*, PP_QNB), PPTR(const float*, PP_KNW), PPTR(const float*, PP_KNB), PPTR(const float*, PP_WP), sv_self,
                           d1, g_self, t_self, PPTR(const int*, PP_GIDX), PPTR(const int*, PP_OWNER), PPTR(const int*, PP_STILES),
                           PPTR(const int*, PP_SBLOCKS), (int)I[PI_NSTILES], PPTR(const int*, PP_KEXT), PPTR(const int*, PP_EXTPOS), n_extra, npad,
                           M, C, H, scale, drop, s_self, attn_p, pair_mix(s_self, 1), prec, wm, wm_b, wsd, wsd_b, cm, cs, link, 0, st, side));
  return lotus_cpe_bwd(d1, PPTR(const act_t*, PP_XS), PPTR(const float*, PP_CW), PPTR(const float*, PP_CWP), PPTR(const float*, PP_LW),
                       PPTR(const float*, PP_G0), sv_cpe, same ? PPTR(act_t*, PP_DX) : PPTR(act_t*, PP_DXS), same, g_cpe, t_cpe,
                       PPTR(const int*, PP_NBR27), PPTR(const int*, PP_ORDER0), PPTR(const int*, PP_TAPPLAN), PPTR(const long long*, PP_CODE0), (int)I[PI_NDUP], M, C, prec, wm,
                       wm_b, PPTR(void*, PP_WS_CONV), (size_t)I[PI_WS_CONV], wsd, wsd_b, cm, cs, link, 0, st, side);
}
#undef PPTR

}
```

### robot-3dlotus_amd/csrc/gemm.hip

```cpp
#include "gemm_common.h"
#include <stdlib.h>
#include <type_traits>

namespace LOTUS_NS {


template <int R, bool KC, int BK>
struct GTile {
  static constexpr int kLd = KC ? BK + 4 : R;
  static constexpr int kFloats = KC ? R * (BK + 4) : BK * R;
};

template <int BM, int BN, int BK, bool A_KC, bool B_KC, bool SUM_A>
__device__ __forceinline__ void gemm_slab(const float* __restrict__ As, const float* __restrict__ Bs, int wr0, int wc0,
                                          f32x16 (&acc)[BM / 64][BN / 64], float (&asum)[BM / 64]) {
  constexpr int TM = BM / 64, TN = BN / 64, KS = BK / 2;
  const int l31 = threadIdx.x & 31, h = (threadIdx.x >> 5) & 1;
  float a[TM][KS], b[TN][KS];
#pragma unroll
  for (int tm = 0; tm < TM; ++tm) {
    if (A_KC) {
      const float* row = As + (wr0 + tm * 32 + l31) * GTile<BM, true, BK>::kLd + h * KS;
#pragma unroll
      for (int q = 0; q < KS / 4; ++q) {
// ... 715 lines not shown
    memset(&p, 0, sizeof(p));
    p.A = x; p.B = w; p.C = part;
    p.M = 27 * n64;
    p.N = mode == 0 ? cout : cin;
    p.K = mode == 0 ? cin : cout;
    p.lda = p.K; p.ldb = 27L * cin; p.ldc = p.N;
    p.act = LOTUS_ACT_NONE;
    p.klen = cdiv(p.K, GEMM_KALIGN) * GEMM_KALIGN;
    p.a_vec = vec_ok(x, p.K); p.b_vec = vec_ok(w, cin) && cin % 4 == 0; p.prec = 0;
    p.drop_inv_keep = 1.f;
    p.a_rows = tg_in; p.tap_cnt = tg_cnt; p.tap_rows = n64; p.b_tap_mirror = mode == 1; p.b_tap_stride = cin;
    p.a_src_rows = src_rows;
    {
      GemmP q = p;
      const int rc = launch_gemm_dma_tap(q, mode, st);
      if (rc != LOTUS_GEMM_DMA_NA) return rc;
    }
    if (!(fast_ok<true, true>(p))) {
      lotus_set_error("lotus_subm_conv(tap-grouped): rows, weights and the partial slab must be 16-byte aligned with widths that are multiples of 4");
      return LOTUS_E_UNSUPPORTED;
    }
    return mode == 0 ? launch_gemm<true, true, false>(p, 1, st) : launch_gemm<true, false, false>(p, 1, st);
  }
}

extern "C" {

size_t lotus_splitk_counters_bytes(void) { return (size_t)(LOTUS_SPLITK_MAX_TILES + 64) * sizeof(unsigned); }
size_t lotus_bn_counters_offset(void) { return (size_t)LOTUS_SPLITK_MAX_TILES * sizeof(unsigned); }

size_t lotus_linear_workspace(int M, int N, int K) {
  const int a = fwd_splits(M, N, K), b = fwd_splits(M, K, N);
  const size_t wa = a > 1 ? (size_t)a * M * N * sizeof(float) : 0, wb = b > 1 ? (size_t)b * M * K * sizeof(float) : 0;
  return wa > wb ? wa : wb;
}

int lotus_linear_fwd(const act_t* x, const float* w, const float* bias, const act_t* residual, act_t* y,
                     act_t* pre, int M, int N, int K, int act, float drop_p, unsigned long long drop_seed,
                     int precision, void* workspace, size_t workspace_bytes, void* counters, void* stream) {
  LOTUS_CHECK_ARG(x && w && y && M >= 0 && N > 0 && K > 0, "lotus_linear_fwd: bad arguments");
  const int w_shadow = precision == 5;
  LOTUS_CHECK_ARG(!w_shadow || LOTUS_ACT_IS_BF16, "lotus_linear_fwd: precision 5 (bf16 weight shadow) exists in the bf16-storage build only");
  if (w_shadow) precision = 1;
  LOTUS_CHECK_ARG(precision == 0 || precision == 1 || precision == 3, "lotus_linear_fwd: precision must be 0, 1 or 3 (5 with bf16 weights)");
  LOTUS_CHECK_ARG(!(LOTUS_ACT_IS_BF16 && precision == 3), "lotus_linear_fwd: bf16x3 operands (precision 3) are not built for bf16 activation storage; use 1 (bf16) or 0");
  if (M == 0) return LOTUS_OK;
  GemmP p;
  memset(&p, 0, sizeof(p));
  p.A = x; p.B = w; p.C = y; p.M = M; p.N = N; p.K = K;
  p.lda = K; p.ldb = K; p.ldc = N;
  p.bias = bias; p.residual = residual; p.pre = pre; p.act = act;
  p.klen = cdiv(K, GEMM_KALIGN) * GEMM_KALIGN;
  p.a_vec = vec_ok(x, K); p.b_vec = vec_ok(w, K); p.prec = precision; p.b_act = w_shadow;
  set_drop(p, drop_p, drop_seed);
  return run_gemm_splitk<true, true>(p, workspace, workspace_bytes, (unsigned*)counters, (hipStream_t)stream);
}

int lotus_linear_dgrad(const act_t* dy, const float* w, act_t* dx, const act_t* pre, const act_t* add, int M,
                       int N, int K, int act, float drop_p, unsigned long long drop_seed, int precision, void* workspace,
                       size_t workspace_bytes, void* counters, void* stream) {
  LOTUS_CHECK_ARG(dy && w && dx && M >= 0 && N > 0 && K > 0, "lotus_linear_dgrad: bad arguments");
  const int w_shadow = precision == 5;
  LOTUS_CHECK_ARG(!w_shadow || LOTUS_ACT_IS_BF16, "lotus_linear_dgrad: precision 5 (bf16 weight shadow) exists in the bf16-storage build only");
  if (w_shadow) precision = 1;
  LOTUS_CHECK_ARG(precision == 0 || precision == 1 || precision == 3, "lotus_linear_dgrad: precision must be 0, 1 or 3 (5 with bf16 weights)");
  LOTUS_CHECK_ARG(!(LOTUS_ACT_IS_BF16 && precision == 3), "lotus_linear_dgrad: bf16x3 operands (precision 3) are not built for bf16 activation storage; use 1 (bf16) or 0");
  if (M == 0) return LOTUS_OK;
  GemmP p;
  memset(&p, 0, sizeof(p));
  p.A = dy; p.B = w; p.C = dx; p.M = M; p.N = K; p.K = N;
  p.lda = N; p.ldb = K; p.ldc = K;
  p.act = LOTUS_ACT_NONE;
  p.mulpre = pre; p.dact = act; p.residual = add;
  p.klen = cdiv(N, GEMM_KALIGN) * GEMM_KALIGN;
  p.a_vec = vec_ok(dy, N); p.b_vec = vec_ok(w, K); p.prec = precision; p.b_act = w_shadow;
  set_drop(p, drop_p, drop_seed);
  return run_gemm_splitk<true, false>(p, workspace, workspace_bytes, (unsigned*)counters, (hipStream_t)stream);
}

int lotus_layernorm_bwd(const act_t* dy, const act_t* x, const float* mean, const float* rstd, const float* gamma, const act_t* add,
                        act_t* dx, float* dgamma, float* dbeta, int M, int C, int accumulate, act_t* dz, float drop_p,
                        unsigned long long drop_seed, void* workspace, size_t workspace_bytes, void* stream);
int lotus_layernorm_bwd_parts(int M, int C);
int lotus_linear_dgrad_ln(const act_t* dy, const float* w, const act_t* x, const float* mean, const float* rstd, const float* gamma,
                          const act_t* add, act_t* dx, act_t* dn, act_t* dz, float dz_p, unsigned long long dz_seed, int M, int N,
                          int K, int precision, void* workspace, size_t workspace_bytes, void* counters, void* ln_workspace,
                          size_t ln_workspace_bytes, int* nparts, void* stream) {
  LOTUS_CHECK_ARG(dy && w && x && mean && rstd && gamma && dx && dn && nparts && ln_workspace && M >= 0 && N > 0 && K > 0,
                  "lotus_linear_dgrad_ln: bad arguments");
  LOTUS_CHECK_ARG(!dz || dz_p > 0.f, "lotus_linear_dgrad_ln: dz needs dz_p > 0");
  if (M == 0) { *nparts = 0; return LOTUS_OK; }
  if (precision == 0 && !LOTUS_ACT_IS_BF16 && (size_t)cdiv(M, 128) * 2 * K * sizeof(float) <= ln_workspace_bytes) {
    GemmP p;
    memset(&p, 0, sizeof(p));
    p.A = dy; p.B = w; p.C = dx; p.M = M; p.N = K; p.K = N;
    p.lda = N; p.ldb = K; p.ldc = K;
    p.act = LOTUS_ACT_NONE; p.residual = add;
    p.klen = cdiv(N, GEMM_KALIGN) * GEMM_KALIGN;
    p.a_vec = vec_ok(dy, N); p.b_vec = vec_ok(w, K); p.prec = 0;
    set_drop(p, dz ? dz_p : 0.f, dz_seed);
    p.ln_x = x; p.ln_mean = mean; p.ln_rstd = rstd; p.ln_gamma = gamma; p.ln_part = (float*)ln_workspace; p.ln_dz = dz;
    if (p.a_vec && p.b_vec && vec_ok(dx, K) && vec_ok(x, K) && (!add || vec_ok(add, K))) {
      const int rc = launch_gemm_dma(p, 1, 1, (hipStream_t)stream);
      if (rc != LOTUS_GEMM_DMA_NA) { *nparts = cdiv(M, 128); return rc; }
    }
  }
  StopEventOnLast stop_ev;
  int rc = lotus_linear_dgrad(dy, w, dn, nullptr, nullptr, M, N, K, LOTUS_ACT_NONE, 0.f, 0, precision, workspace, workspace_bytes, counters, stream);
  if (rc) return rc;
  stop_ev.last();
  rc = lotus_layernorm_bwd(dn, x, mean, rstd, gamma, add, dx, nullptr, nullptr, M, K, 0, dz, dz ? dz_p : 0.f, dz_seed, ln_workspace,
                           ln_workspace_bytes, stream);
  *nparts = lotus_layernorm_bwd_parts(M, K);
  return rc;
}

static int wgrad_splits(int M, int N, int K) {
  if (const int dz = gemm_dma_wgrad_splits(M, N, K)) return dz;
  int nz = 1;
  const long tiles = (long)cdiv(N, 64) * cdiv(K, 64);
  if (tiles >= 128 && M < 1024) return 1;
  while (nz < 256 && tiles * nz < 1024 && M / (nz * 2) >= 128) nz *= 2;
  return nz;
}

size_t lotus_linear_wgrad_workspace(int M, int N, int K) {
  return (size_t)wgrad_splits(M, N, K) * ((size_t)N * K + N) * sizeof(float);
}

int lotus_linear_wgrad(const act_t* dy, const act_t* x, float* dw, float* db, int M, int N, int K,
                       int accumulate, int precision, void* workspace, size_t workspace_bytes, void* counters,
                       void* stream) {
  LOTUS_CHECK_ARG(dy && x && dw && M >= 0 && N > 0 && K > 0, "lotus_linear_wgrad: bad arguments");
  if (precision == 5) precision = 1;
  LOTUS_CHECK_ARG(precision == 0 || precision == 1 || precision == 3, "lotus_linear_wgrad: precision must be 0, 1 or 3");
  LOTUS_CHECK_ARG(!(LOTUS_ACT_IS_BF16 && precision == 3), "lotus_linear_wgrad: bf16x3 operands (precision 3) are not built for bf16 activation storage; use 1 (bf16) or 0");
  hipStream_t st = (hipStream_t)stream;
  const int nz = wgrad_splits(M, N, K);
  const size_t slab = (size_t)N * K + N;
  LOTUS_CHECK_ARG(workspace && workspace_bytes >= (size_t)nz * slab * sizeof(float),
                  "lotus_linear_wgrad: workspace too small (%zu < %zu)", workspace_bytes, (size_t)nz * slab * sizeof(float));
  const bool direct = nz == 1 && !accumulate;
  float* part = (float*)workspace;
  GemmP p;
  memset(&p, 0, sizeof(p));
  p.A = dy; p.B = x; p.M = N; p.N = K; p.K = M;
  p.lda = N; p.ldb = K; p.ldc = K;
  p.klen = cdiv(cdiv(M > 0 ? M : 1, nz), GEMM_KALIGN) * GEMM_KALIGN;
  p.a_vec = vec_ok(dy, N); p.b_vec = vec_ok(x, K); p.prec = precision;
  set_drop(p, 0.f, 0);
  constexpr int fuse_max = 4;
  const long wtiles = (long)cdiv(N, 64) * cdiv(K, 64);
  if (!direct && counters && splitk_fused_enabled() && nz <= fuse_max && wtiles <= LOTUS_SPLITK_MAX_TILES) {
    GemmP q = p;
    q.C = dw; q.part = part; q.part_stride = (long)slab; q.cnt = (unsigned*)counters;
    q.bias_part = db ? part + (size_t)N * K : nullptr; q.bias_stride = (long)slab; q.bias_out = db; q.accumulate = accumulate;
    if (fast_ok<false, false>(q)) return launch_gemm<false, false, true>(q, nz, st);
  }
  if (direct) {
    p.C = dw; p.bias_part = db;
  } else {
    p.C = part; p.part_stride = (long)slab;
    p.bias_part = db ? part + (size_t)N * K : nullptr; p.bias_stride = (long)slab;
  }
  int rc = launch_gemm<false, false, true>(p, nz, st);
  if (rc || direct) return rc;
  const long n = (long)N * K;
  if (db && db == dw + n) return lotus_reduce_parts(part, dw, (long)slab, (long)slab, nz, accumulate, st);
  rc = lotus_reduce_parts(part, dw, n, (long)slab, nz, accumulate, st);
  if (!rc && db) rc = lotus_reduce_parts(part + n, db, (long)N, (long)slab, nz, accumulate, st);
  return rc;
}

}

}
```

### robot-3dlotus_amd/csrc/lotus_rename_b16.h

```cpp
#define lotus_add lotus_b16_add
#define lotus_attention_bwd lotus_b16_attention_bwd
#define lotus_attention_bwd_workspace lotus_b16_attention_bwd_workspace
#define lotus_attention_fwd lotus_b16_attention_fwd
#define lotus_batchnorm_apply lotus_b16_batchnorm_apply
#define lotus_batchnorm_apply_sums lotus_b16_batchnorm_apply_sums
#define lotus_batchnorm_bwd_apply lotus_b16_batchnorm_bwd_apply
#define lotus_batchnorm_bwd_stats lotus_b16_batchnorm_bwd_stats
#define lotus_batchnorm_bwd_stats_fused lotus_b16_batchnorm_bwd_stats_fused
#define lotus_batchnorm_bwd_stats_fused_params lotus_b16_batchnorm_bwd_stats_fused_params
#define lotus_batchnorm_eval_stats lotus_b16_batchnorm_eval_stats
#define lotus_batchnorm_finalize lotus_b16_batchnorm_finalize
#define lotus_batchnorm_stats lotus_b16_batchnorm_stats
#define lotus_batchnorm_stats_fused lotus_b16_batchnorm_stats_fused
#define lotus_batchnorm_workspace lotus_b16_batchnorm_workspace
#define lotus_bn_counters_offset lotus_b16_bn_counters_offset
#define lotus_cloud_max_bwd lotus_b16_cloud_max_bwd
#define lotus_cloud_max_fwd lotus_b16_cloud_max_fwd
#define lotus_cloud_max_workspace lotus_b16_cloud_max_workspace
#define lotus_conv_dup_fold lotus_b16_conv_dup_fold
#define lotus_conv_dup_mask lotus_b16_conv_dup_mask
#define lotus_conv_pairs_try lotus_b16_conv_pairs_try
#define lotus_conv_pairs_workspace lotus_b16_conv_pairs_workspace
#define lotus_conv_tap_eligible lotus_b16_conv_tap_eligible
#define lotus_conv_tap_gemm lotus_b16_conv_tap_gemm
#define lotus_conv_weight_transpose lotus_b16_conv_weight_transpose
#define lotus_conv_weight_transpose_impl lotus_b16_conv_weight_transpose_impl
#define lotus_cpe_bwd lotus_b16_cpe_bwd
#define lotus_cpe_fwd lotus_b16_cpe_fwd
#define lotus_cpe_grads_floats lotus_b16_cpe_grads_floats
#define lotus_cpe_saved_floats lotus_b16_cpe_saved_floats
#define lotus_cpe_tmp_floats lotus_b16_cpe_tmp_floats
#define lotus_cpe_ws_conv_bytes lotus_b16_cpe_ws_conv_bytes
#define lotus_cpe_ws_main_bytes lotus_b16_cpe_ws_main_bytes
#define lotus_cpe_ws_side_bytes lotus_b16_cpe_ws_side_bytes
#define lotus_crossattn_bwd lotus_b16_crossattn_bwd
#define lotus_crossattn_fwd lotus_b16_crossattn_fwd
#define lotus_crossattn_grads_floats lotus_b16_crossattn_grads_floats
#define lotus_crossattn_kv_bwd lotus_b16_crossattn_kv_bwd
#define lotus_crossattn_kv_fwd lotus_b16_crossattn_kv_fwd
#define lotus_crossattn_kv_grads_floats lotus_b16_crossattn_kv_grads_floats
#define lotus_crossattn_kv_saved_floats lotus_b16_crossattn_kv_saved_floats
#define lotus_crossattn_kv_tmp_floats lotus_b16_crossattn_kv_tmp_floats
#define lotus_crossattn_kv_ws_main_bytes lotus_b16_crossattn_kv_ws_main_bytes
#define lotus_crossattn_kv_ws_side_bytes lotus_b16_crossattn_kv_ws_side_bytes
#define lotus_crossattn_saved_floats lotus_b16_crossattn_saved_floats
#define lotus_crossattn_tmp_floats lotus_b16_crossattn_tmp_floats
#define lotus_crossattn_ws_main_bytes lotus_b16_crossattn_ws_main_bytes
#define lotus_crossattn_ws_side_bytes lotus_b16_crossattn_ws_side_bytes
#define lotus_drop_path lotus_b16_drop_path
#define lotus_dropout lotus_b16_dropout
#define lotus_ffn_bwd lotus_b16_ffn_bwd
#define lotus_ffn_fwd lotus_b16_ffn_fwd
#define lotus_ffn_grads_floats lotus_b16_ffn_grads_floats
#define lotus_ffn_saved_floats lotus_b16_ffn_saved_floats
#define lotus_ffn_tmp_floats lotus_b16_ffn_tmp_floats
#define lotus_ffn_ws_main_bytes lotus_b16_ffn_ws_main_bytes
#define lotus_ffn_ws_side_bytes lotus_b16_ffn_ws_side_bytes
#define lotus_layernorm_bwd lotus_b16_layernorm_bwd
#define lotus_layernorm_bwd_params lotus_b16_layernorm_bwd_params
#define lotus_layernorm_bwd_params_n lotus_b16_layernorm_bwd_params_n
#define lotus_layernorm_bwd_parts lotus_b16_layernorm_bwd_parts
#define lotus_layernorm_bwd_workspace lotus_b16_layernorm_bwd_workspace
#define lotus_layernorm_fwd lotus_b16_layernorm_fwd
#define lotus_linear_dgrad lotus_b16_linear_dgrad
#define lotus_linear_dgrad_ln lotus_b16_linear_dgrad_ln
#define lotus_linear_fwd lotus_b16_linear_fwd
#define lotus_linear_wgrad lotus_b16_linear_wgrad
#define lotus_linear_wgrad_workspace lotus_b16_linear_wgrad_workspace
#define lotus_linear_workspace lotus_b16_linear_workspace
#define lotus_loss_bwd lotus_b16_loss_bwd
#define lotus_loss_fwd lotus_b16_loss_fwd
#define lotus_loss_stats_floats lotus_b16_loss_stats_floats
#define lotus_mp_loss_bwd lotus_b16_mp_loss_bwd
#define lotus_mp_loss_fwd lotus_b16_mp_loss_fwd
#define lotus_pair_acts_floats lotus_b16_pair_acts_floats
#define lotus_pair_bwd lotus_b16_pair_bwd
#define lotus_pair_fwd lotus_b16_pair_fwd
#define lotus_pair_grads_floats lotus_b16_pair_grads_floats
#define lotus_pair_nint lotus_b16_pair_nint
#define lotus_pair_nptr lotus_b16_pair_nptr
#define lotus_pair_saved_floats lotus_b16_pair_saved_floats
#define lotus_pair_tmp_floats lotus_b16_pair_tmp_floats
#define lotus_pair_ws_conv_bytes lotus_b16_pair_ws_conv_bytes
#define lotus_pair_ws_main_bytes lotus_b16_pair_ws_main_bytes
#define lotus_pair_ws_side_bytes lotus_b16_pair_ws_side_bytes
#define lotus_pool_max_bwd lotus_b16_pool_max_bwd
#define lotus_pool_max_fwd lotus_b16_pool_max_fwd
#define lotus_pos_ce_bwd lotus_b16_pos_ce_bwd
#define lotus_pos_ce_fwd lotus_b16_pos_ce_fwd
#define lotus_pos_decode_max lotus_b16_pos_decode_max
#define lotus_pos_targets lotus_b16_pos_targets
#define lotus_pos_workspace lotus_b16_pos_workspace
#define lotus_reduce_parts lotus_b16_reduce_parts
#define lotus_selfattn_bwd lotus_b16_selfattn_bwd
#define lotus_selfattn_fwd lotus_b16_selfattn_fwd
#define lotus_selfattn_grads_floats lotus_b16_selfattn_grads_floats
#define lotus_selfattn_saved_floats lotus_b16_selfattn_saved_floats
#define lotus_selfattn_tmp_floats lotus_b16_selfattn_tmp_floats
#define lotus_selfattn_ws_main_bytes lotus_b16_selfattn_ws_main_bytes
#define lotus_selfattn_ws_side_bytes lotus_b16_selfattn_ws_side_bytes
#define lotus_splitk_counters_bytes lotus_b16_splitk_counters_bytes
#define lotus_step_act_bwd lotus_b16_step_act_bwd
#define lotus_step_act_bwd_workspace lotus_b16_step_act_bwd_workspace
#define lotus_step_act_fwd lotus_b16_step_act_fwd
#define lotus_subm_conv lotus_b16_subm_conv
#define lotus_subm_conv_wgrad lotus_b16_subm_conv_wgrad
#define lotus_subm_conv_wgrad_workspace lotus_b16_subm_conv_wgrad_workspace
#define lotus_subm_conv_workspace lotus_b16_subm_conv_workspace
#define lotus_sum_slabs lotus_b16_sum_slabs
#define lotus_sum_slabs_ld lotus_b16_sum_slabs_ld
#define lotus_unpool_bwd lotus_b16_unpool_bwd
#define lotus_unpool_fwd lotus_b16_unpool_fwd
```

### robot-3dlotus_amd/csrc/norm.hip

```cpp
#include "common.h"
#include <stdlib.h>

namespace LOTUS_NS {

struct LnP {
  const act_t* x;
  const act_t* res;
  const float* gamma;
  const float* beta;
  act_t* y;
  float* mean;
  float* rstd;
  int M, C, LPR, NV;
  float eps;
};

__device__ __forceinline__ float group_sum(float v, int lpr) {
  for (int o = lpr >> 1; o > 0; o >>= 1) v += __shfl_xor(v, o, 64);
  return v;
}

__global__ __launch_bounds__(256) void ln_fwd_kernel(LnP p) {
  LOTUS_T_PRIO();
  const int rpb = 256 / p.LPR;
// ... 53 lines not shown
  const act_t* x;
  const float* mean;
  const float* rstd;
  const float* gamma;
  const act_t* add;
  act_t* dx;
  float* part;
  int M, C, LPR, NV;
  act_t* dz;
  unsigned long long drop_seed;
  unsigned drop_thresh;
  float drop_inv_keep;
};

__global__ __launch_bounds__(256) void ln_bwd_kernel(LnBwdP p) {
  LOTUS_T_PRIO();
  extern __shared__ float red[];
  const int rpb = 256 / p.LPR;
  const int rslot = threadIdx.x / p.LPR, l = threadIdx.x % p.LPR;
  const int c4 = p.C / 4;
  float4 pg[4], pb[4];
#pragma unroll
  for (int j = 0; j < 4; ++j) pg[j] = pb[j] = make_float4(0.f, 0.f, 0.f, 0.f);
  for (int row0 = blockIdx.x * rpb; row0 < p.M; row0 += gridDim.x * rpb) {
    const int row = row0 + rslot;
    const bool valid = row < p.M;
    const float mean = valid ? p.mean[row] : 0.f, rstd = valid ? p.rstd[row] : 0.f;
    float4 xh[4], g[4], av[4];
    float s1 = 0.f, s2 = 0.f;
#pragma unroll
    for (int j = 0; j < 4; ++j) {
      const int q = l + j * p.LPR;
      xh[j] = g[j] = av[j] = make_float4(0.f, 0.f, 0.f, 0.f);
      if (valid && j < p.NV && q < c4) {
        const float4 xv = ld4q(p.x + (long)row * p.C, q);
        const float4 dv = ld4q(p.dy + (long)row * p.C, q);
        if (p.add) av[j] = ld4q(p.add + (long)row * p.C, q);
        const float4 gm = ld4q(p.gamma, q);
        xh[j] = make_float4((xv.x - mean) * rstd, (xv.y - mean) * rstd, (xv.z - mean) * rstd, (xv.w - mean) * rstd);
        pg[j].x += dv.x * xh[j].x; pg[j].y += dv.y * xh[j].y; pg[j].z += dv.z * xh[j].z; pg[j].w += dv.w * xh[j].w;
        pb[j].x += dv.x; pb[j].y += dv.y; pb[j].z += dv.z; pb[j].w += dv.w;
        g[j] = make_float4(dv.x * gm.x, dv.y * gm.y, dv.z * gm.z, dv.w * gm.w);
        s1 += g[j].x + g[j].y + g[j].z + g[j].w;
        s2 += g[j].x * xh[j].x + g[j].y * xh[j].y + g[j].z * xh[j].z + g[j].w * xh[j].w;
      }
    }
    s1 = group_sum(s1, p.LPR) / p.C;
    s2 = group_sum(s2, p.LPR) / p.C;
#pragma unroll
    for (int j = 0; j < 4; ++j) {
      const int q = l + j * p.LPR;
      if (valid && j < p.NV && q < c4) {
        float4 o;
        o.x = rstd * (g[j].x - s1 - xh[j].x * s2);
        o.y = rstd * (g[j].y - s1 - xh[j].y * s2);
        o.z = rstd * (g[j].z - s1 - xh[j].z * s2);
        o.w = rstd * (g[j].w - s1 - xh[j].w * s2);
        o.x += av[j].x; o.y += av[j].y; o.z += av[j].z; o.w += av[j].w;
        st4q(p.dx + (long)row * p.C, q, o);
        if (p.dz) {
          const unsigned long long e = (unsigned long long)row * p.C + 4 * q;
          float dm[4];
          dropout_scale4(p.drop_seed, e, p.drop_thresh, p.drop_inv_keep, dm);
          const float4 z = make_float4(o.x * dm[0], o.y * dm[1], o.z * dm[2], o.w * dm[3]);
          st4q(p.dz + (long)row * p.C, q, z);
        }
      }
    }
  }
#pragma unroll
  for (int j = 0; j < 4; ++j) {
    const int q = l + j * p.LPR;
    if (j < p.NV && q < c4) {
      st4q(red + (long)(rslot * 2 + 0) * p.C, q, pg[j]);
      st4q(red + (long)(rslot * 2 + 1) * p.C, q, pb[j]);
    }
  }
  __syncthreads();
  for (int c = threadIdx.x; c < 2 * p.C; c += 256) {
    const int which = c / p.C, col = c % p.C;
    float s = 0.f;
    for (int r = 0; r < rpb; ++r) s += red[(long)(r * 2 + which) * p.C + col];
    p.part[((long)blockIdx.x * 2 + which) * p.C + col] = s;
  }
}

__global__ __launch_bounds__(1024) void colpart_reduce_kernel(const float* __restrict__ part, float* __restrict__ o0,
                                                              float* __restrict__ o1, int nb, int C, int accumulate) {
  __shared__ float red[32][33];
  const int cl = threadIdx.x & 31, r = threadIdx.x >> 5;
  const int c = blockIdx.x * 32 + cl;
  float s = 0.f;
  if (c < 2 * C) {
    int b = r;
    for (; b + 96 < nb; b += 128) {
      const float v0 = part[(long)b * 2 * C + c], v1 = part[(long)(b + 32) * 2 * C + c];
      const float v2 = part[(long)(b + 64) * 2 * C + c], v3 = part[(long)(b + 96) * 2 * C + c];
      s += (v0 + v1) + (v2 + v3);
    }
    for (; b < nb; b += 32) s += part[(long)b * 2 * C + c];
  }
  red[r][cl] = s;
  __syncthreads();
  if (r == 0 && c < 2 * C) {
    float t = 0.f;
    for (int k = 0; k < 32; ++k) t += red[k][cl];
    const int which = c / C, col = c % C;
    float* o = which ? o1 : o0;
    if (o) o[col] = accumulate ? o[col] + t : t;
  }
}

static int ln_geometry(int C, int* LPR, int* NV) {
  if (C % 4) return -1;
  const int c4 = C / 4;
  int lpr = 64;
  if (c4 <= 16) lpr = 16;
  else if (c4 <= 32) lpr = 32;
  const int nv = (c4 + lpr - 1) / lpr;
  if (nv > 4) return -1;
  *LPR = lpr;
  *NV = nv;
  return 0;
}

static int ln_geometry_bwd(int C, int* LPR, int* NV) {
  if (C % 4) return -1;
  const int c4 = C / 4;
  int lpr = 64;
  while (lpr > 4 && c4 <= (lpr / 2) * 4) lpr /= 2;
  const int nv = (c4 + lpr - 1) / lpr;
  if (nv > 4) return -1;
  *LPR = lpr;
  *NV = nv;
  return 0;
}

#define BN_GS 16
#define BN_FUSED_MAX_GRID 256
#define BN_COUNTERS (1 + BN_FUSED_MAX_GRID / BN_GS)
struct BnStatP {
  const act_t* x;
  const act_t* dy;
  const float* mean;
  const float* invstd;
  const float* gamma;
  const float* beta;
  double* part;
  int M, C, act;
  unsigned* cnt;
  double* sums;
  float* out_mean;
  float* out_invstd;
  float* running_mean;
  float* running_var;
  float eps, momentum;
};

__global__ __launch_bounds__(256) void bn_stat_kernel(BnStatP p) {
  LOTUS_T_PRIO();
  extern __shared__ double dred[];
  const int c4 = p.C / 4;
  const int tpr = c4 < 256 ? c4 : 256;
  const int rslots = 256 / tpr;
  const int rslot = threadIdx.x / tpr, l = threadIdx.x % tpr;
  const bool live = rslot < rslots;
// ... 332 lines not shown
  size_t n = (size_t)(256 / tpr) * 2 * C;
  if (n < 256) n = 256;
  return n * sizeof(double);
}
static int bn_grid_fused(int M, int C) {
  const int g = bn_grid(M, C);
  return g > BN_FUSED_MAX_GRID ? BN_FUSED_MAX_GRID : g;
}

extern "C" {

int lotus_layernorm_fwd(const act_t* x, const act_t* res, const float* gamma, const float* beta, act_t* y,
                        float* mean, float* rstd, int M, int C, float eps, void* stream) {
  LnP p;
  p.x = x; p.res = res; p.gamma = gamma; p.beta = beta; p.y = y; p.mean = mean; p.rstd = rstd;
  p.M = M; p.C = C; p.eps = eps;
  LOTUS_CHECK_ARG(x && gamma && beta && y && M >= 0, "lotus_layernorm_fwd: bad arguments");
  LOTUS_CHECK_ARG(ln_geometry(C, &p.LPR, &p.NV) == 0, "lotus_layernorm_fwd: unsupported C=%d", C);
  if (M == 0) return LOTUS_OK;
  LOTUS_LAUNCH(ln_fwd_kernel, dim3(cdiv(M, 256 / p.LPR)), dim3(256), 0, (hipStream_t)stream, p);
  LOTUS_LAUNCH_CHECK("lotus_layernorm_fwd");
  return LOTUS_OK;
}

#define LN_BWD_MAX_GRID 1024
static int ln_bwd_grid(int M, int rpb) {
  int grid = cdiv(M > 0 ? M : 1, rpb * 2);
  return grid > LN_BWD_MAX_GRID ? LN_BWD_MAX_GRID : grid;
}
size_t lotus_layernorm_bwd_workspace(int M, int C) { return (size_t)LN_BWD_MAX_GRID * 2 * C * sizeof(float); }

int lotus_layernorm_bwd(const act_t* dy, const act_t* x, const float* mean, const float* rstd, const float* gamma,
                        const act_t* add, act_t* dx, float* dgamma, float* dbeta, int M, int C, int accumulate,
                        act_t* dz, float drop_p, unsigned long long drop_seed, void* workspace, size_t workspace_bytes,
                        void* stream) {
  LnBwdP p;
  p.dz = (dz && drop_p > 0.f) ? dz : nullptr;
  p.drop_seed = drop_seed;
  lotus_drop_setup(drop_p, &p.drop_thresh, &p.drop_inv_keep);
  LOTUS_CHECK_ARG(!dz || drop_p > 0.f, "lotus_layernorm_bwd: dz needs drop_p > 0");
  p.dy = dy; p.x = x; p.mean = mean; p.rstd = rstd; p.gamma = gamma; p.add = add; p.dx = dx;
  p.part = (float*)workspace; p.M = M; p.C = C;
  LOTUS_CHECK_ARG(dy && x && mean && rstd && gamma && dx && M >= 0, "lotus_layernorm_bwd: bad arguments");
  LOTUS_CHECK_ARG(ln_geometry_bwd(C, &p.LPR, &p.NV) == 0, "lotus_layernorm_bwd: unsupported C=%d", C);
  const int rpb = 256 / p.LPR;
  const int grid = ln_bwd_grid(M, rpb);
  LOTUS_CHECK_ARG(workspace && workspace_bytes >= (size_t)grid * 2 * C * sizeof(float),
                  "lotus_layernorm_bwd: workspace too small");
  hipStream_t st = (hipStream_t)stream;
  LOTUS_LAUNCH(ln_bwd_kernel, dim3(grid), dim3(256), (size_t)rpb * 2 * C * sizeof(float), st, p);
  if (dgamma && dbeta)
    LOTUS_LAUNCH(colpart_reduce_kernel, dim3(cdiv(2 * C, 32)), dim3(1024), 0, st, p.part, dgamma, dbeta, grid, C,
                       accumulate);
  LOTUS_LAUNCH_CHECK("lotus_layernorm_bwd");
  return LOTUS_OK;
}

int lotus_layernorm_bwd_params(const void* workspace, int M, int C, float* dgamma, float* dbeta, int accumulate,
                               void* stream) {
  int lpr, nv;
  LOTUS_CHECK_ARG(workspace && dgamma && dbeta && M >= 0, "lotus_layernorm_bwd_params: bad arguments");
  LOTUS_CHECK_ARG(ln_geometry_bwd(C, &lpr, &nv) == 0, "lotus_layernorm_bwd_params: unsupported C=%d", C);
  const int grid = ln_bwd_grid(M, 256 / lpr);
  LOTUS_LAUNCH(colpart_reduce_kernel, dim3(cdiv(2 * C, 32)), dim3(1024), 0, (hipStream_t)stream,
                     (const float*)workspace, dgamma, dbeta, grid, C, accumulate);
  LOTUS_LAUNCH_CHECK("lotus_layernorm_bwd_params");
  return LOTUS_OK;
}

int lotus_layernorm_bwd_parts(int M, int C) {
  int lpr, nv;
  if (ln_geometry_bwd(C, &lpr, &nv)) return 0;
  return ln_bwd_grid(M, 256 / lpr);
}
int lotus_layernorm_bwd_params_n(const void* workspace, int nparts, int C, float* dgamma, float* dbeta, int accumulate, void* stream) {
  LOTUS_CHECK_ARG(workspace && dgamma && dbeta && nparts >= 0 && C > 0, "lotus_layernorm_bwd_params_n: bad arguments");
  if (nparts == 0 && accumulate) return LOTUS_OK;
  LOTUS_LAUNCH(colpart_reduce_kernel, dim3(cdiv(2 * C, 32)), dim3(1024), 0, (hipStream_t)stream, (const float*)workspace, dgamma, dbeta,
               nparts, C, accumulate);
  LOTUS_LAUNCH_CHECK("lotus_layernorm_bwd_params_n");
  return LOTUS_OK;
}

size_t lotus_batchnorm_workspace(int M, int C) { return (size_t)BN_MAX_GRID * 2 * C * sizeof(double); }

int lotus_batchnorm_stats(const act_t* x, double* sums, int M, int C, void* workspace, size_t workspace_bytes,
                          void* stream) {
  LOTUS_CHECK_ARG(x && sums && C % 4 == 0 && M >= 0, "lotus_batchnorm_stats: bad arguments (C=%d)", C);
  const int grid = bn_grid(M, C);
  LOTUS_CHECK_ARG(workspace && workspace_bytes >= (size_t)grid * 2 * C * sizeof(double),
                  "lotus_batchnorm_stats: workspace too small");
  BnStatP p;
  memset(&p, 0, sizeof(p));
  p.x = x; p.part = (double*)workspace; p.M = M; p.C = C;
  hipStream_t st = (hipStream_t)stream;
  LOTUS_LAUNCH(bn_stat_kernel, dim3(grid), dim3(256), bn_dyn_lds(C), st, p);
  LOTUS_LAUNCH(bn_part_reduce_kernel, dim3(cdiv(2 * C, 32)), dim3(256), 0, st, p.part, sums, grid, C, M);
  LOTUS_LAUNCH_CHECK("lotus_batchnorm_stats");
  return LOTUS_OK;
}

int lotus_batchnorm_stats_fused(const act_t* x, double* sums, float* mean, float* invstd, float* running_mean, float* running_var,
                                int M, int C, float eps, float momentum, void* workspace, size_t workspace_bytes, void* counter,
                                void* stream) {
  LOTUS_CHECK_ARG(x && sums && (!mean == !invstd) && counter && C % 4 == 0 && M > 0, "lotus_batchnorm_stats_fused: bad arguments (C=%d)", C);
  const int grid = bn_grid_fused(M, C);
  LOTUS_CHECK_ARG(workspace && workspace_bytes >= (size_t)(grid + BN_COUNTERS) * 2 * C * sizeof(double), "lotus_batchnorm_stats_fused: workspace too small");
  BnStatP p;
  memset(&p, 0, sizeof(p));
  p.x = x; p.part = (double*)workspace; p.M = M; p.C = C;
  p.cnt = (unsigned*)counter; p.sums = sums; p.out_mean = mean; p.out_invstd = invstd;
  p.running_mean = running_mean; p.running_var = running_var; p.eps = eps; p.momentum = momentum;
  LOTUS_LAUNCH(bn_stat_kernel, dim3(grid), dim3(256), bn_dyn_lds(C), (hipStream_t)stream, p);
  LOTUS_LAUNCH_CHECK("lotus_batchnorm_stats_fused");
  return LOTUS_OK;
}

int lotus_batchnorm_bwd_stats_fused_params(const act_t* dy, const act_t* x, const float* mean, const float* invstd, const float* gamma,
                                           const float* beta, double* sums, float* dgamma, float* dbeta, int M, int C, int act,
                                           void* workspace, size_t workspace_bytes, void* counter, void* stream);
int lotus_batchnorm_bwd_stats_fused(const act_t* dy, const act_t* x, const float* mean, const float* invstd, const float* gamma,
                                    const float* beta, double* sums, int M, int C, int act, void* workspace, size_t workspace_bytes,
                                    void* counter, void* stream) {
  LOTUS_CHECK_ARG(dy && x && sums && counter && C % 4 == 0 && M > 0, "lotus_batchnorm_bwd_stats_fused: bad arguments");
  const int grid = bn_grid_fused(M, C);
  LOTUS_CHECK_ARG(workspace && workspace_bytes >= (size_t)(grid + BN_COUNTERS) * 2 * C * sizeof(double), "lotus_batchnorm_bwd_stats_fused: workspace too small");
  BnStatP p;
  memset(&p, 0, sizeof(p));
  p.x = x; p.dy = dy; p.mean = mean; p.invstd = invstd; p.gamma = gamma; p.beta = beta;
  p.part = (double*)workspace; p.M = M; p.C = C; p.act = act;
  p.cnt = (unsigned*)counter; p.sums = sums;
  LOTUS_LAUNCH(bn_stat_kernel, dim3(grid), dim3(256), bn_dyn_lds(C), (hipStream_t)stream, p);
  LOTUS_LAUNCH_CHECK("lotus_batchnorm_bwd_stats_fused");
  return LOTUS_OK;
}

int lotus_batchnorm_bwd_stats_fused_params(const act_t* dy, const act_t* x, const float* mean, const float* invstd, const float* gamma,
                                           const float* beta, double* sums, float* dgamma, float* dbeta, int M, int C, int act,
                                           void* workspace, size_t workspace_bytes, void* counter, void* stream) {
  LOTUS_CHECK_ARG(dy && x && sums && dgamma && dbeta && counter && C % 4 == 0 && M > 0, "lotus_batchnorm_bwd_stats_fused_params: bad arguments");
  const int grid = bn_grid_fused(M, C);
  LOTUS_CHECK_ARG(workspace && workspace_bytes >= (size_t)(grid + BN_COUNTERS) * 2 * C * sizeof(double), "lotus_batchnorm_bwd_stats_fused_params: workspace too small");
  BnStatP p;
  memset(&p, 0, sizeof(p));
  p.x = x; p.dy = dy; p.mean = mean; p.invstd = invstd; p.gamma = gamma; p.beta = beta;
  p.part = (double*)workspace; p.M = M; p.C = C; p.act = act;
  p.cnt = (unsigned*)counter; p.sums = sums; p.out_mean = dbeta; p.out_invstd = dgamma;
  LOTUS_LAUNCH(bn_stat_kernel, dim3(grid), dim3(256), bn_dyn_lds(C), (hipStream_t)stream, p);
  LOTUS_LAUNCH_CHECK("lotus_batchnorm_bwd_stats_fused_params");
  return LOTUS_OK;
}

int lotus_batchnorm_finalize(const double* sums, float* mean, float* invstd, float* running_mean,
                             float* running_var, int C, float eps, float momentum, void* stream) {
  LOTUS_CHECK_ARG(sums && mean && invstd, "lotus_batchnorm_finalize: bad arguments");
  LOTUS_LAUNCH(bn_finalize_kernel, dim3(cdiv(C, 256)), dim3(256), 0, (hipStream_t)stream, sums, mean,
                     invstd, running_mean, running_var, C, eps, momentum);
  LOTUS_LAUNCH_CHECK("lotus_batchnorm_finalize");
  return LOTUS_OK;
}

int lotus_batchnorm_eval_stats(const float* running_mean, const float* running_var, float* mean, float* invstd, int C,
                               float eps, void* stream) {
  LOTUS_LAUNCH(bn_eval_stats_kernel, dim3(cdiv(C, 256)), dim3(256), 0, (hipStream_t)stream, running_mean,
                     running_var, mean, invstd, C, eps);
  LOTUS_LAUNCH_CHECK("lotus_batchnorm_eval_stats");
// ... 84 lines not shown
```

### robot-3dlotus_amd/ops.py

```python
import os

import torch

from . import _capi
from ._capi import call, query, WS

ACT_NONE, ACT_GELU, ACT_LEAKY = 0, 1, 2
BN_EPS, BN_MOMENTUM = 1e-3, 0.01
CALL_LOG = None
EVENT_LOG = None


class _Timed:

    def __init__(self, key):
        self.key = key

    def __enter__(self):
        if EVENT_LOG is None:
            return self
        self.st = _SIDES[_CUR][0] if _capi.STREAM_OVERRIDE else torch.cuda.current_stream()
        self.e0 = torch.cuda.Event(enable_timing=True)
        self.e0.record(self.st)
        return self
# ... 360 lines not shown
        dw, db = into
    if CALL_LOG is not None:
        CALL_LOG.append(("wgrad", M, N, K))
    nbytes = query("lotus_linear_wgrad_workspace", M, N, K)
    with _OnSide(dy, x):
        ws = _side_ws(nbytes, dy.device) if _side() is not None else WS.get(nbytes, dy.device, slot=0)
        with _Timed(("wgrad", M, N, K)):
            call("lotus_linear_wgrad", dy, x, dw, db, M, N, K, 0 if into is None else 1, _pa(prec), ws,
                 ws.numel(), _counters(dy.device))
    return dw, db


def ln_fwd(x, g, b, res=None, eps=1e-5, save=True):
    M, C = x.shape
    y = torch.empty_like(x)
    mean = torch.empty(M, dtype=torch.float32, device=x.device) if save else None
    rstd = torch.empty(M, dtype=torch.float32, device=x.device) if save else None
    call("lotus_layernorm_fwd", x, res, g, b, y, mean, rstd, M, C, float(eps))
    return y, mean, rstd


class Handoff:
    __slots__ = ("drop", "ptr", "dz")

    def __init__(self):
        self.drop, self.ptr, self.dz = None, 0, None

    def arm(self, p, seed):
        self.drop, self.ptr, self.dz = ((float(p), int(seed)) if p > 0.0 else None), 0, None

    def take(self, dy):
        dz, self.dz = self.dz, None
        return dz if (dz is not None and self.ptr == dy.data_ptr() and dz.shape == dy.shape) else None


def _masked(dy, p, seed, hand):
    if hand is not None:
        dz = hand.take(dy)
        if dz is not None:
            return dz
    return dropout(dy, p, seed)


def ln_bwd(dy, x, mean, rstd, g, add=None, hand=None):
    M, C = x.shape
    dx = torch.empty_like(x)
    dg = torch.empty(C, dtype=torch.float32, device=x.device)
    db = torch.empty(C, dtype=torch.float32, device=x.device)
    dz, dp, dseed = None, 0.0, 0
    if hand is not None and hand.drop is not None:
        dp, dseed = hand.drop
        dz = torch.empty_like(x)
        hand.ptr, hand.dz = dx.data_ptr(), dz
    nbytes = query("lotus_layernorm_bwd_workspace", M, C)
    if _side() is None:
        ws = _ws(nbytes, x.device)
        call("lotus_layernorm_bwd", dy, x, mean, rstd, g, add, dx, dg, db, M, C, 0, dz, dp, dseed, ws, ws.numel())
        return dx, dg, db
    ws = WS.get(nbytes, x.device, slot=4) if _JOIN == "node" else torch.empty(nbytes, dtype=torch.uint8, device=x.device)
    call("lotus_layernorm_bwd", dy, x, mean, rstd, g, add, dx, None, None, M, C, 0, dz, dp, dseed, ws, ws.numel())
    with _OnSide(ws):
        call("lotus_layernorm_bwd_params", ws, M, C, dg, db, 0)
    return dx, dg, db


def linear_dgrad_ln(dy, w, x, mean, rstd, g, add=None, drop=None):
    import numpy as np
    M, N = dy.shape
    K = w.shape[1]
    dx, dn = torch.empty_like(x), torch.empty_like(x)
    dg = torch.empty(K, dtype=torch.float32, device=x.device)
    db = torch.empty(K, dtype=torch.float32, device=x.device)
    dz = torch.empty_like(x) if drop else None
    dp, dseed = drop if drop else (0.0, 0)
    nbytes = query("lotus_layernorm_bwd_workspace", M, K)
    lws = _ws(nbytes, x.device)
    nb = query("lotus_linear_workspace", M, N, K) if M <= 8192 else 0
    ws = WS.get(nb, x.device, slot=5) if nb else None
    nparts = np.zeros(1, dtype=np.int32)
    call("lotus_linear_dgrad_ln", dy, w, x, mean, rstd, g, add, dx, dn, dz, float(dp), int(dseed), M, N, K, _pa(None), ws, nb,
         _counters(x.device) if nb else None, lws, lws.numel(), int(nparts.ctypes.data))
    call("lotus_layernorm_bwd_params_n", lws, int(nparts[0]), K, dg, db, 0)
    return dx, dg, db, dz, int(nparts[0])


def conv_weight_t(w, prec=None):
    cout, cin = w.shape[0], w.shape[-1]
    T = w.numel() // (cout * cin)
    wt = torch.empty(2 * w.numel(), dtype=torch.float32, device=w.device)
    call("lotus_conv_weight_transpose", w, wt, cout, T, cin, _pa(prec))
    return wt


_NO_PACK = {}


def conv_tap_active(lvl, C):
    return _PREC == 0 and not _capi.BF16 and getattr(lvl, "tap_plan", None) is not None and \
        query("lotus_conv_tap_eligible", lvl.n, C, C) == 1


def no_pack(dev):
    t = _NO_PACK.get(dev)
    if t is None:
        t = _NO_PACK[dev] = torch.empty(0, dtype=torch.float32, device=dev)
    return t


def prepack_conv_weights(weights):
    global _IN_NODE
    outs = [torch.empty(2 * w.numel(), dtype=torch.float32, device=w.device) for w in weights]
    _IN_NODE += 1
    try:
        with _OnSide(*weights):
            for w, o in zip(weights, outs):
                cout, cin = w.shape[0], w.shape[-1]
                call("lotus_conv_weight_transpose", w, o, cout, w.numel() // (cout * cin), cin, _pa())
    finally:
        _IN_NODE -= 1
    return outs


def _conv_ws(n, cin, cout, dev):
    nbytes = query("lotus_subm_conv_workspace", n, cin, cout)
    return WS.get(nbytes, dev, slot=2) if nbytes else None


def conv_fwd(x, w, b, nbr, rowidx, add=None, w_t=None, prec=None, tap_plan=None):
    n, cin = x.shape
    cout, T = w.shape[0], nbr.shape[0]
    y = torch.empty(n, cout, dtype=x.dtype, device=x.device)
    if T == 27:
        ws = _conv_ws(n, cin, cout, x.device)
    else:
        ws = WS.get(4 * T * cin * cout, x.device, slot=2) if cin <= 8 else None
    call("lotus_subm_conv", 0, x, w, w_t, b, add, y, nbr, rowidx, n, T, cin, cout, _pa(prec), tap_plan, ws,
         ws.numel() if ws is not None else 0)
    return y


def conv_dgrad(dy, w, nbr, rowidx, add=None, w_t=None, lvl=None, prec=None, tap_plan=None):
    n, cout = dy.shape
    cin, T = w.shape[-1], nbr.shape[0]
    dups = lvl is not None and lvl.n_dup != 0
    if dups:
        dyr = torch.empty_like(dy)
        call("lotus_conv_dup_fold", dy, lvl.code[0], lvl.order[0], n, cout, dyr)
        dy = dyr
    dx = torch.empty(n, cin, dtype=dy.dtype, device=dy.device)
    ws = _conv_ws(n, cin, cout, dy.device) if T == 27 else None
    call("lotus_subm_conv", 1, dy, w, w_t, None, add, dx, nbr, rowidx, n, T, cin, cout, _pa(prec), tap_plan, ws,
         ws.numel() if ws is not None else 0)
    if dups:
        call("lotus_conv_dup_mask", dx, add, nbr[T // 2], n, cin)
    return dx


def conv_wgrad(dy, x, w_shape, nbr, need_bias=True, prec=None, side=True):
    n, cout = dy.shape
    cin, T = x.shape[1], nbr.shape[0]
    nw = cout * T * cin
    buf = _grad_slab(nw + (cout if need_bias else 0), dy.device)
    dw = buf[:nw].view(w_shape)
    db = buf[nw:] if need_bias else None
    nbytes = query("lotus_subm_conv_wgrad_workspace", n, T, cin, cout)
    if not side:
# ... 700 lines not shown
            n_saved, _, _, ws_main, _ = _sizes("crosskv", N, C, H, L, lvl.n_ca_blocks, lvl.ca_groups)
            saved = torch.empty(n_saved, dtype=torch.float32, device=x.device)
            y = torch.empty_like(x)
            ws = _ws(ws_main, x.device)
            _capi.call_raw("lotus_crossattn_kv_fwd", x, kv, kv_ld, g, b, wqk, bq, qnw, qnb, knw, knb, wpk, bp, y, saved, lvl.ca_tiles,
                           lvl.n_ca_tiles, N, C, H, float(d ** -0.5), float(drop_p), int(seed), float(attn_p), mix_seed(seed, 1), pc,
                           lvl.ca_kmax, ws, ws.numel(), _counters(x.device), _capi.stream_ptr())
            ctx.save_for_backward(x, kv, g, wq, qnw, qnb, knw, knb, wp, saved)
            return y
        n, mean, rstd = ln_fwd(x, g, b)
        q, _ = linear_fwd(n, wqk, bq)
        att = torch.empty(N, C, dtype=x.dtype, device=x.device)
        lse = torch.empty(N, H, dtype=torch.float32, device=x.device)
        attention_fwd(q, C, 0, kv, kv_ld, 0, C, None, None, None, lvl.ca_tiles, lvl.n_ca_tiles, (qnw, qnb), (knw, knb),
                      att, lse, H, d, attn_p, mix_seed(seed, 1), k_max=lvl.ca_kmax)
        y, _ = linear_fwd(att, wpk, bp, residual=x, drop_p=drop_p, seed=seed)
        ctx.save_for_backward(x, kv, g, wq, qnw, qnb, knw, knb, wp, n, q, att, lse, mean, rstd)
        return y

    @_joined
    def backward(ctx, dy):
        lvl, H, d, p, seed, attn_p, bank, bidx = ctx.meta
        hand_in, hand_out = ctx.hands
        dy = dy.contiguous()
        dkv = bank.grad_slice(bidx)
        if ctx.comp:
            x, kv, g, wq, qnw, qnb, knw, knb, wp, saved = ctx.saved_tensors
            N, C = x.shape
            L, dev, G = kv.shape[0], x.device, lvl.ca_groups
            _, n_grads, n_tmp, ws_main, ws_side = _sizes("crosskv", N, C, H, L, lvl.n_ca_blocks, G)
            grads = _grad_slab(n_grads, dev)
            tmp = torch.empty(n_tmp, dtype=torch.float32, device=dev)
            dx = torch.empty_like(x)
            dz_in = hand_in.take(dy) if hand_in is not None else None
            dz_out, po, so = None, 0.0, 0
            if hand_out is not None and hand_out.drop is not None:
                po, so = hand_out.drop
                dz_out = torch.empty_like(x)
                hand_out.ptr, hand_out.dz = dx.data_ptr(), dz_out
            side, wss, cs = _side_ctx(dev, ws_side, (saved, tmp, dy, dz_in), N)
            wsm = _ws(ws_main if side else max(ws_main, ws_side), dev)
            _capi.call_raw("lotus_crossattn_kv_bwd", dy, dz_in, x, kv, kv.stride(0), g, ctx.wk[0], qnw, qnb, knw, knb, ctx.wk[1], saved, dx, dkv,
                           dkv.stride(0), dz_out, po, so, grads, tmp, lvl.ca_tiles, lvl.ca_blocks, lvl.n_ca_blocks, G, N, C, H, L,
                           float(d ** -0.5), float(p), int(seed), float(attn_p), mix_seed(seed, 1), ctx.pc, lvl.ca_kmax, wsm, wsm.numel(),
                           wss, wss.numel() if wss is not None else 0, _counters(dev), cs, _LINK, 0, _capi.stream_ptr(), side)
            d4 = _al4(d)
            o1 = 2 * _al4(C)
            o2 = o1 + _al4(C * C + C)
            o3 = o2 + 4 * d4
            return (dx, dkv, grads[:C], grads[_al4(C):_al4(C) + C], grads[o1:o1 + C * C].view(C, C), grads[o1 + C * C:o1 + C * C + C],
                    grads[o2:o2 + d], grads[o2 + d4:o2 + d4 + d], grads[o2 + 2 * d4:o2 + 2 * d4 + d], grads[o2 + 3 * d4:o2 + 3 * d4 + d],
                    grads[o3:o3 + C * C].view(C, C), grads[o3 + C * C:o3 + C * C + C]) + (None,) * 9
        x, kv, g, wq, qnw, qnb, knw, knb, wp, n, q, att, lse, mean, rstd = ctx.saved_tensors
        N, C = x.shape
        dev = x.device
        dz = _masked(dy, p, seed, hand_in)
        dwp, dbp = linear_wgrad(dz, att)
        datt = linear_dgrad(dz, ctx.wk[1])
        dq = torch.empty(N, C, dtype=x.dtype, device=dev)
        G, L = lvl.ca_groups, kv.shape[0]
        if G > 1:
            dkv_part = torch.empty(G, L, 2 * C, dtype=x.dtype, device=dev)
            tgt, tld, tps = dkv_part, 2 * C, L * 2 * C
        else:
            tgt, tld, tps = dkv, dkv.stride(0), 0
        gq, bq_, gk, bk_ = attention_bwd(q, C, 0, kv, kv.stride(0), 0, C, None, None, None, lvl.ca_tiles, lvl.ca_blocks,
                                         lvl.n_ca_blocks, (qnw, qnb), (knw, knb), att, datt, lse, dq, C, 0, tgt, tld, 0, C, tps, 0, H, d,
                                         attn_p, mix_seed(seed, 1), k_max=lvl.ca_kmax)
        if G > 1:
            call("lotus_sum_slabs_ld", dkv_part, dkv, L, 2 * C, dkv.stride(0), L * 2 * C, G)
        dwq, dbq = linear_wgrad(dq, n)
        dn = linear_dgrad(dq, ctx.wk[0])
        dx, dg, db = ln_bwd(dn, x, mean, rstd, g, add=dy, hand=hand_out)
        return (dx, dkv, dg, db, dwq, dbq, gq, bq_, gk, bk_, dwp, dbp) + (None,) * 9


_PAIR = {"0": False, "1": True}.get(os.environ.get("LOTUS_PAIR", "auto"), "auto")
_PAIR_AUTO_ROWS = 40000
_PP = None
_PP_NAMES = ("X XS KV Y ACTS SAVED CW CWP CB LW LB G0 B0 G1 B1 WQKV BQKV QNW QNB KNW KNB WP BP G2 B2 W1 B1F W2 B2F G3 B3 WQ BQ CQNW CQNB "
             "CKNW CKNB CWP2 CBP2 G4 B4 W3 B3F W4 B4F NBR27 ORDER0 TAPPLAN CODE0 GIDX OWNER STILES SBLOCKS KEXT EXTPOS CATILES CABLOCKS WS_MAIN "
             "WS_SIDE WS_CONV CNT_MAIN CNT_SIDE STREAM SIDE DY DX DXS DKV GRADS TMP").split()
_PI_NAMES = ("M C H HD NPAD NSTILES NEXTRA L NCATILES NCABLOCKS G KMAX NDUP SAME PREC KV_LD DKV_LD WS_MAIN WS_SIDE WS_CONV LINK SEED_SELF "
             "SEED_FFN1 SEED_CROSS SEED_FFN2").split()
_PAIR_PARAM_SLOTS = ("CW CB LW LB G0 B0 G1 B1 WQKV BQKV QNW QNB KNW KNB WP BP G2 B2 W1 B1F W2 B2F G3 B3 WQ BQ CQNW CQNB CKNW CKNB CWP2 CBP2 "
                     "G4 B4 W3 B3F W4 B4F").split()
_PAIR_LINEAR = (2, 8, 14, 18, 20, 24, 30, 34, 36)


def pair_enabled(rows, rows0=None):
    if not composites_enabled():
        return False
    if _PAIR == "auto":
        if _capi.BF16:
            return True
        if BnState.reduce is not None or GRAD_ARENA is not None:
            return (rows if rows0 is None else rows0) <= _PAIR_AUTO_ROWS
        return rows <= _PAIR_AUTO_ROWS
    return _PAIR


def set_pair(on):
    global _PAIR
    _PAIR = on if on == "auto" else bool(on)


def _pair_tables():
    global _PP
    if _PP is None:
        import numpy as np
        assert query("lotus_pair_nptr") == len(_PP_NAMES) and query("lotus_pair_nint") == len(_PI_NAMES), \
            "ops._PP_NAMES / _PI_NAMES are out of step with enum PairPtr / PairInt of csrc/blocks.cpp"
        _PP = (np, {n: i for i, n in enumerate(_PP_NAMES)}, {n: i for i, n in enumerate(_PI_NAMES)},
               [_PP_NAMES.index(n) for n in _PAIR_PARAM_SLOTS])
    return _PP


def _pair_grad_sizes(C, H, Hd):
    key = ("pairgrads", C, H, Hd)
    v = _SIZE_CACHE.get(key)
    if v is None:
        d = C // H
        assert C % 4 == 0 and d % 4 == 0 and Hd % 4 == 0
        cpe = [C, C, C * C, C, 27 * C * C, C]
        att = [C, C, 3 * C * C, 3 * C, d, d, d, d, C * C, C]
        ffn = [C, C, Hd * C, Hd, C * Hd, C]
        ca = [C, C, C * C, C, d, d, d, d, C * C, C]
        v = _SIZE_CACHE[key] = cpe + att + ffn + ca + ffn
    return v


class PairFn(torch.autograd.Function):

    @_fwd
    def forward(ctx, x, xs, kv, wt, *rest):
        np, PP, PI, slots = _pair_tables()
        params, meta = rest[:38], rest[38]
        lvl, lvl_ca, H, Hd, drop_p, attn_p, s_self, s_f1, s_cross, s_f2, bank, bidx = meta
        M, C = x.shape
        L = kv.shape[0]
        same = xs is x
        dev = x.device
        n_acts, n_saved, n_grads, n_tmp, ws_main, ws_side, ws_conv = _sizes(
            "pair", M, C, H, Hd, lvl.npad, lvl.n_self_tiles, lvl.n_extra, L, lvl_ca.n_ca_blocks, lvl_ca.ca_groups)
        acts = torch.empty(n_acts, dtype=torch.float32, device=dev)
        saved = torch.empty(n_saved, dtype=torch.float32, device=dev)
        y = torch.empty_like(x)
        ws = _ws(ws_main, dev)
        wc = WS.get(ws_conv, dev, slot=2)
        lin = [params[i] for i in _PAIR_LINEAR]
        link, pc = _wk(*lin)
        P = np.zeros(len(_PP_NAMES), dtype=np.uint64)
        I = np.zeros(len(_PI_NAMES), dtype=np.uint64)
        for slot, t in zip(slots, params):
            P[slot] = t.data_ptr()
        for i, t in zip(_PAIR_LINEAR, link):
            P[slots[i]] = t.data_ptr()
        P[PP["X"]], P[PP["XS"]], P[PP["KV"]], P[PP["Y"]] = x.data_ptr(), xs.data_ptr(), kv.data_ptr(), y.data_ptr()
        P[PP["ACTS"]], P[PP["SAVED"]], P[PP["CWP"]] = acts.data_ptr(), saved.data_ptr(), wt.data_ptr()
        P[PP["NBR27"]], P[PP["ORDER0"]], P[PP["CODE0"]] = lvl.nbr27.data_ptr(), lvl.order[0].data_ptr(), lvl.code[0].data_ptr()
        P[PP["TAPPLAN"]] = lvl.tap_plan.data_ptr() if lvl.tap_plan is not None else 0
        P[PP["GIDX"]], P[PP["OWNER"]], P[PP["STILES"]] = lvl.gidx.data_ptr(), lvl.owner.data_ptr(), lvl.self_tiles.data_ptr()
        P[PP["SBLOCKS"]], P[PP["KEXT"]], P[PP["EXTPOS"]] = lvl.self_blocks.data_ptr(), lvl.kext.data_ptr(), lvl.ext_pos.data_ptr()
        P[PP["CATILES"]], P[PP["CABLOCKS"]] = lvl_ca.ca_tiles.data_ptr(), lvl_ca.ca_blocks.data_ptr()
        P[PP["WS_MAIN"]], P[PP["WS_CONV"]] = ws.data_ptr(), wc.data_ptr()
        P[PP["CNT_MAIN"]], P[PP["STREAM"]] = _counters(dev).data_ptr(), _capi.stream_ptr()
        for k, v_ in (("M", M), ("C", C), ("H", H), ("HD", Hd), ("NPAD", lvl.npad), ("NSTILES", lvl.n_self_tiles),
                      ("NEXTRA", lvl.n_extra), ("L", L), ("NCATILES", lvl_ca.n_ca_tiles), ("NCABLOCKS", lvl_ca.n_ca_blocks),
                      ("G", lvl_ca.ca_groups), ("KMAX", lvl_ca.ca_kmax), ("NDUP", lvl.n_dup & 0xFFFFFFFF), ("SAME", 1 if same else 0),
                      ("PREC", pc), ("KV_LD", kv.stride(0)), ("WS_MAIN", ws.numel()), ("WS_CONV", wc.numel()),
                      ("SEED_SELF", s_self), ("SEED_FFN1", s_f1), ("SEED_CROSS", s_cross), ("SEED_FFN2", s_f2)):
            I[PI[k]] = v_
        F = np.array([float(drop_p), float(attn_p), float((C // H) ** -0.5)], dtype=np.float64)
        _capi.call_raw("lotus_pair_fwd", P.ctypes.data, I.ctypes.data, F.ctypes.data)
        ctx.save_for_backward(xs, kv, wt, acts, saved)
        ctx.keep = (params, link)
        ctx.tabs = (P, I, F)
        ctx.meta = (lvl, lvl_ca, H, Hd, same, bank, bidx, M, C, L)
        return y

    @_joined
    def backward(ctx, dy):
        np, PP, PI, slots = _pair_tables()
        xs, kv, wt, acts, saved = ctx.saved_tensors
        params, _ = ctx.keep
        lvl, lvl_ca, H, Hd, same, bank, bidx, M, C, L = ctx.meta
        P, I, F = ctx.tabs
        dev = xs.device
        dy = dy.contiguous()
        _, _, n_grads, n_tmp, ws_main, ws_side, ws_conv = _sizes(
            "pair", M, C, H, Hd, lvl.npad, lvl.n_self_tiles, lvl.n_extra, L, lvl_ca.n_ca_blocks, lvl_ca.ca_groups)
        grads = _grad_slab(n_grads, dev)
        tmp = torch.empty(n_tmp, dtype=torch.float32, device=dev)
        dx = torch.empty_like(dy)
        dxs = None if same else torch.empty_like(xs)
        dkv = bank.grad_slice(bidx)
        side, wss, cs = _side_ctx(dev, ws_side, (saved, acts, tmp, dy, xs, kv, lvl.nbr27), M)
        wsm = _ws(ws_main if side else max(ws_main, ws_side), dev)
        wc = WS.get(ws_conv, dev, slot=2)
        P[PP["DY"]], P[PP["DX"]], P[PP["DXS"]] = dy.data_ptr(), dx.data_ptr(), (0 if dxs is None else dxs.data_ptr())
        P[PP["DKV"]], P[PP["GRADS"]], P[PP["TMP"]] = dkv.data_ptr(), grads.data_ptr(), tmp.data_ptr()
        P[PP["WS_MAIN"]], P[PP["WS_CONV"]], P[PP["WS_SIDE"]] = wsm.data_ptr(), wc.data_ptr(), (0 if wss is None else wss.data_ptr())
        P[PP["CNT_MAIN"]], P[PP["CNT_SIDE"]] = _counters(dev).data_ptr(), (0 if cs is None else cs.data_ptr())
        P[PP["STREAM"]], P[PP["SIDE"]] = _capi.stream_ptr(), side
        I[PI["WS_MAIN"]], I[PI["WS_CONV"]], I[PI["WS_SIDE"]] = wsm.numel(), wc.numel(), (0 if wss is None else wss.numel())
        I[PI["DKV_LD"]], I[PI["LINK"]] = dkv.stride(0), _LINK
        _capi.call_raw("lotus_pair_bwd", P.ctypes.data, I.ctypes.data, F.ctypes.data)
        g = grads.split(_pair_grad_sizes(C, H, Hd))
        cw = params[0]
        out = (g[4].view(cw.shape), g[5], g[2].view(C, C), g[3], g[0], g[1],
               g[6], g[7], g[8].view(3 * C, C), g[9], g[10], g[11], g[12], g[13], g[14].view(C, C), g[15],
               g[16], g[17], g[18].view(Hd, C), g[19], g[20].view(C, Hd), g[21],
               g[22], g[23], g[24].view(C, C), g[25], g[26], g[27], g[28], g[29], g[30].view(C, C), g[31],
               g[32], g[33], g[34].view(Hd, C), g[35], g[36].view(C, Hd), g[37])
        return (dx, dxs, dkv, None) + out + (None,)


class StemFn(torch.autograd.Function):

    @_fwd
    def forward(ctx, x, cw, g, b, rmean, rvar, lvl, training):
        c = conv_fwd(x, cw, None, lvl.nbr125, lvl.order[0])
        y, mean, invstd = bn_fwd(c, g, b, rmean, rvar, training, ACT_GELU)
        ctx.save_for_backward(x, cw, g, b, c, mean, invstd)
        ctx.meta = (lvl, training)
        return y

    @_joined
    def backward(ctx, dy):
        x, cw, g, b, c, mean, invstd = ctx.saved_tensors
        lvl, training = ctx.meta
        dc, dg, db = bn_bwd(dy.contiguous(), c, mean, invstd, g, b, training, ACT_GELU)
        dcw, _ = conv_wgrad(dc, x, cw.shape, lvl.nbr125, need_bias=False, side=ctx.needs_input_grad[0] or not _STEM_WGRAD_MAIN)
        dx = conv_dgrad(dc, cw, lvl.nbr125, lvl.order[0], lvl=lvl) if ctx.needs_input_grad[0] else None
        return dx, dcw, dg, db, None, None, None, None


class PoolFn(torch.autograd.Function):

    @_fwd
    def forward(ctx, x, w, bias, g, b, rmean, rvar, child, training):
        (wk,), _ = _wk(w)
        ctx.wk = wk
        proj, _ = linear_fwd(x, wk, bias)
        C = w.shape[0]
        pooled = torch.empty(child.n, C, dtype=x.dtype, device=x.device)
        arg = torch.empty(child.n, C, dtype=torch.int32, device=x.device)
        call("lotus_pool_max_fwd", proj, child.members, child.seg_start, child.n, C, pooled, arg)
        if ARG_TAP is not None or ARG_INJECT:
            arg = _arg_hook("pool", arg)
        y, mean, invstd = bn_fwd(pooled, g, b, rmean, rvar, training, ACT_GELU)
        ctx.save_for_backward(x, w, g, b, pooled, arg, mean, invstd)
        ctx.meta = (child, training)
        return y
# ... 338 lines not shown
```

Baseline: 1085 keystep-samples/s.

## Fuse back-to-back CPE and self-attention LayerNorms in forward and backward

Adds a two-LayerNorm forward kernel that computes the CPE output norm and the following self-attention pre-norm in one pass, so the self-attention forward skips its own LayerNorm. In backward it adds chained kernels (dgrad_ln2, layernorm_bwd2) that propagate the gradient through both LayerNorms and emit both sets of gamma/beta partials together. The aim is fewer launches and fewer full reads and writes of activations. The cost is extra workspace, a second partials buffer, and more complex kernels. It is enabled by default in fp32 mode through an LNFUSE flag in the pair composite.

New measurement: 1089 keystep-samples/s, median of 5. About the same (+0.4%).

```diff
diff --git a/include/lotus_hip.h b/include/lotus_hip.h
--- a/include/lotus_hip.h
+++ b/include/lotus_hip.h
@@ -97,6 +97,19 @@
                           const float* gamma, const lotus_act_t* add, lotus_act_t* dx, lotus_act_t* dn, lotus_act_t* dz, float dz_p,
                           unsigned long long dz_seed, int M, int N, int K, int precision, void* workspace, size_t workspace_bytes,
                           void* counters, void* ln_workspace, size_t ln_workspace_bytes, int* nparts, void* stream);
+int lotus_layernorm_fwd2(const lotus_act_t* l, const lotus_act_t* res, const float* g0, const float* b0, const float* g1, const float* b1,
+                         lotus_act_t* y, lotus_act_t* n, float* mean0, float* rstd0, float* mean1, float* rstd1, int M, int C, float eps,
+                         void* stream);
+int lotus_layernorm_bwd2(const lotus_act_t* dn, const lotus_act_t* x1, const float* mean1, const float* rstd1, const float* g1,
+                         const lotus_act_t* add, lotus_act_t* dx1, lotus_act_t* dz, float drop_p, unsigned long long drop_seed,
+                         const lotus_act_t* l, const float* mean0, const float* rstd0, const float* g0, lotus_act_t* dl, int M, int C,
+                         void* workspace1, size_t workspace1_bytes, void* workspace0, size_t workspace0_bytes, void* stream);
+int lotus_linear_dgrad_ln2(const lotus_act_t* dy, const float* w, const lotus_act_t* x, const float* mean, const float* rstd,
+                           const float* gamma, const lotus_act_t* add, lotus_act_t* dx, lotus_act_t* dn, lotus_act_t* dz, float dz_p,
+                           unsigned long long dz_seed, const lotus_act_t* l, const float* mean0, const float* rstd0, const float* gamma0,
+                           lotus_act_t* dl, int M, int N, int K, int precision, void* workspace, size_t workspace_bytes, void* counters,
+                           void* ln_workspace, size_t ln_workspace_bytes, void* ln0_workspace, size_t ln0_workspace_bytes, int* nparts,
+                           int* chained, void* stream);
 int lotus_layernorm_bwd_params(const void* workspace, int M, int C, float* dgamma, float* dbeta, int accumulate,
                                void* stream);
 size_t lotus_batchnorm_workspace(int M, int C);
diff --git a/include/lotus_hip_b16.h b/include/lotus_hip_b16.h
--- a/include/lotus_hip_b16.h
+++ b/include/lotus_hip_b16.h
@@ -28,6 +28,9 @@
 int lotus_b16_layernorm_bwd_parts(int M, int C);
 int lotus_b16_layernorm_bwd_params_n(const void* workspace, int nparts, int C, float* dgamma, float* dbeta, int accumulate, void* stream);
 int lotus_b16_linear_dgrad_ln(const lotus_bf16_t* dy, const float* w, const lotus_bf16_t* x, const float* mean, const float* rstd, const float* gamma, const lotus_bf16_t* add, lotus_bf16_t* dx, lotus_bf16_t* dn, lotus_bf16_t* dz, float dz_p, unsigned long long dz_seed, int M, int N, int K, int precision, void* workspace, size_t workspace_bytes, void* counters, void* ln_workspace, size_t ln_workspace_bytes, int* nparts, void* stream);
+int lotus_b16_layernorm_fwd2(const lotus_bf16_t* l, const lotus_bf16_t* res, const float* g0, const float* b0, const float* g1, const float* b1, lotus_bf16_t* y, lotus_bf16_t* n, float* mean0, float* rstd0, float* mean1, float* rstd1, int M, int C, float eps, void* stream);
+int lotus_b16_layernorm_bwd2(const lotus_bf16_t* dn, const lotus_bf16_t* x1, const float* mean1, const float* rstd1, const float* g1, const lotus_bf16_t* add, lotus_bf16_t* dx1, lotus_bf16_t* dz, float drop_p, unsigned long long drop_seed, const lotus_bf16_t* l, const float* mean0, const float* rstd0, const float* g0, lotus_bf16_t* dl, int M, int C, void* workspace1, size_t workspace1_bytes, void* workspace0, size_t workspace0_bytes, void* stream);
+int lotus_b16_linear_dgrad_ln2(const lotus_bf16_t* dy, const float* w, const lotus_bf16_t* x, const float* mean, const float* rstd, const float* gamma, const lotus_bf16_t* add, lotus_bf16_t* dx, lotus_bf16_t* dn, lotus_bf16_t* dz, float dz_p, unsigned long long dz_seed, const lotus_bf16_t* l, const float* mean0, const float* rstd0, const float* gamma0, lotus_bf16_t* dl, int M, int N, int K, int precision, void* workspace, size_t workspace_bytes, void* counters, void* ln_workspace, size_t ln_workspace_bytes, void* ln0_workspace, size_t ln0_workspace_bytes, int* nparts, int* chained, void* stream);
 int lotus_b16_layernorm_bwd_params(const void* workspace, int M, int C, float* dgamma, float* dbeta, int accumulate, void* stream);
 size_t lotus_b16_batchnorm_workspace(int M, int C);
 int lotus_b16_batchnorm_stats(const lotus_bf16_t* x, double* sums, int M, int C, void* workspace, size_t workspace_bytes, void* stream);
diff --git a/robot-3dlotus_amd/csrc/blocks.cpp b/robot-3dlotus_amd/csrc/blocks.cpp
--- a/robot-3dlotus_amd/csrc/blocks.cpp
+++ b/robot-3dlotus_amd/csrc/blocks.cpp
@@ -57,21 +57,39 @@
     CHECK(fa_.wait());          \
   } while (0)
 
+struct LnChain {
+  const act_t* l;
+  const float* mean0;
+  const float* rstd0;
+  const float* g0;
+  act_t* dl;
+  float* lnp0;
+  size_t lnp0_bytes;
+  float* dg0;
+  float* db0;
+  int chained;
+};
 static int dgrad_ln(const act_t* dyl, const float* w, act_t* dn, const act_t* x, const float* mean, const float* rstd, const float* g,
                     const act_t* add, act_t* dx, act_t* dz, float dz_p, unsigned long long dz_seed, float* dg, float* db, int M, int N,
                     int C, int precision, void* ws, size_t ws_bytes, void* counters, float* lnp, size_t lnp_bytes,
-                    unsigned long long link, void* stream, void* side) {
+                    unsigned long long link, void* stream, void* side, LnChain* ch = nullptr) {
   int nparts = 0;
   act_t* dzo = dz_p > 0.f ? dz : nullptr;
-  if (side) {
+  void* ps = side ? side : stream;
+  if (ch) {
+    ForkAfter fa(link, side);
+    CHECK(lotus_linear_dgrad_ln2(dyl, w, x, mean, rstd, g, add, dx, dn, dzo, dz_p, dz_seed, ch->l, ch->mean0, ch->rstd0, ch->g0, ch->dl, M, N, C,
+                                 precision, ws, ws_bytes, counters, lnp, lnp_bytes, ch->lnp0, ch->lnp0_bytes, &nparts, &ch->chained, stream));
+    CHECK(fa.wait());
+  } else if (side) {
     PRODUCE_THEN_FORK(lotus_linear_dgrad_ln(dyl, w, x, mean, rstd, g, add, dx, dn, dzo, dz_p, dz_seed, M, N, C, precision, ws, ws_bytes,
                                             counters, lnp, lnp_bytes, &nparts, stream));
-    CHECK(lotus_layernorm_bwd_params_n(lnp, nparts, C, dg, db, 0, side));
   } else {
     CHECK(lotus_linear_dgrad_ln(dyl, w, x, mean, rstd, g, add, dx, dn, dzo, dz_p, dz_seed, M, N, C, precision, ws, ws_bytes, counters, lnp,
                                 lnp_bytes, &nparts, stream));
-    CHECK(lotus_layernorm_bwd_params_n(lnp, nparts, C, dg, db, 0, stream));
-  }
+  }
+  CHECK(lotus_layernorm_bwd_params_n(lnp, nparts, C, dg, db, 0, ps));
+  if (ch && ch->chained) CHECK(lotus_layernorm_bwd_params(ch->lnp0, M, C, ch->dg0, ch->db0, 0, ps));
   return LOTUS_OK;
 }
 
@@ -176,11 +194,11 @@
   return a > b ? a : b;
 }
 
-int lotus_selfattn_fwd(const act_t* x, const float* g, const float* b, const float* wqkv, const float* bqkv, const float* qnw,
-                       const float* qnb, const float* knw, const float* knb, const float* wp, const float* bp, act_t* y,
-                       float* saved, const int* gidx, const int* owner, const int* tiles, int ntiles, int npad, int M, int C,
-                       int H, float scale, float drop_p, unsigned long long seed, float attn_p, unsigned long long attn_seed,
-                       int precision, void* ws, size_t ws_bytes, void* counters, void* stream) {
+static int selfattn_fwd(const act_t* x, const float* g, const float* b, const float* wqkv, const float* bqkv, const float* qnw,
+                        const float* qnb, const float* knw, const float* knb, const float* wp, const float* bp, act_t* y,
+                        float* saved, const int* gidx, const int* owner, const int* tiles, int ntiles, int npad, int M, int C,
+                        int H, float scale, float drop_p, unsigned long long seed, float attn_p, unsigned long long attn_seed,
+                        int precision, void* ws, size_t ws_bytes, void* counters, void* stream, bool have_n) {
   const int d = C / H;
   Carve sv(saved);
   act_t* n = sv.act((size_t)M * C);
@@ -190,7 +208,7 @@
   float* mean = sv.f32(M);
   float* rstd = sv.f32(M);
   const bool big = M > 8192;
-  CHECK(lotus_layernorm_fwd(x, nullptr, g, b, n, mean, rstd, M, C, 1e-5f, stream));
+  if (!have_n) CHECK(lotus_layernorm_fwd(x, nullptr, g, b, n, mean, rstd, M, C, 1e-5f, stream));
   CHECK(lotus_linear_fwd(n, wqkv, bqkv, nullptr, qkv, nullptr, M, 3 * C, C, LOTUS_ACT_NONE, 0.f, 0, precision, big ? nullptr : ws,
                          big ? 0 : ws_bytes, big ? nullptr : counters, stream));
   CHECK(lotus_attention_fwd(qkv, 3L * C, 0, qkv, 3L * C, C, 2 * C, gidx, gidx, owner, tiles, ntiles, qnw, qnb, knw, knb, att, (long)C, lse,
@@ -199,13 +217,22 @@
                           big ? 0 : ws_bytes, big ? nullptr : counters, stream);
 }
 
-int lotus_selfattn_bwd(const act_t* dy, const act_t* dz_in, const act_t* x, const float* g, const float* wqkv, const float* qnw,
-                       const float* qnb, const float* knw, const float* knb, const float* wp, const float* saved, act_t* dx,
-                       float* grads, float* tmp, const int* gidx, const int* owner, const int* tiles, const int* blocks, int nblocks,
-                       const int* kext, const int* ext_pos, int n_extra, int npad, int M, int C, int H, float scale, float drop_p,
-                       unsigned long long seed, float attn_p, unsigned long long attn_seed, int precision, void* ws_main,
-                       size_t ws_main_bytes, void* ws_side, size_t ws_side_bytes, void* counters_main, void* counters_side,
-                       unsigned long long link, int join, void* stream, void* side) {
+int lotus_selfattn_fwd(const act_t* x, const float* g, const float* b, const float* wqkv, const float* bqkv, const float* qnw,
+                       const float* qnb, const float* knw, const float* knb, const float* wp, const float* bp, act_t* y,
+                       float* saved, const int* gidx, const int* owner, const int* tiles, int ntiles, int npad, int M, int C,
+                       int H, float scale, float drop_p, unsigned long long seed, float attn_p, unsigned long long attn_seed,
+                       int precision, void* ws, size_t ws_bytes, void* counters, void* stream) {
+  return selfattn_fwd(x, g, b, wqkv, bqkv, qnw, qnb, knw, knb, wp, bp, y, saved, gidx, owner, tiles, ntiles, npad, M, C, H, scale, drop_p, seed,
+                      attn_p, attn_seed, precision, ws, ws_bytes, counters, stream, false);
+}
+
+static int selfattn_bwd(const act_t* dy, const act_t* dz_in, const act_t* x, const float* g, const float* wqkv, const float* qnw,
+                        const float* qnb, const float* knw, const float* knb, const float* wp, const float* saved, act_t* dx,
+                        float* grads, float* tmp, const int* gidx, const int* owner, const int* tiles, const int* blocks, int nblocks,
+                        const int* kext, const int* ext_pos, int n_extra, int npad, int M, int C, int H, float scale, float drop_p,
+                        unsigned long long seed, float attn_p, unsigned long long attn_seed, int precision, void* ws_main,
+                        size_t ws_main_bytes, void* ws_side, size_t ws_side_bytes, void* counters_main, void* counters_side,
+                        unsigned long long link, int join, void* stream, void* side, LnChain* ch) {
   const int d = C / H;
   Carve sv(saved);
   const act_t* n = sv.act((size_t)M * C);
@@ -255,9 +282,21 @@
                                         gq, bq, gk, bk, 0, H, d, scale, 1e-6f, attn_p, attn_seed, noshadow(precision), 0, ws_main, ws_main_bytes, stream));
   CHECK(lotus_linear_wgrad(dqkv, n, dwqkv, dbqkv, M, 3 * C, C, 0, precision, wws, wws_bytes, wcnt, sw));
   CHECK(dgrad_ln(dqkv, wqkv, dn, x, mean, rstd, g, dy, dx, nullptr, 0.f, 0, dg, db, M, 3 * C, C, precision, big ? nullptr : ws_main,
-                 big ? 0 : ws_main_bytes, big ? nullptr : counters_main, lnp, lnp_bytes, link, stream, side));
+                 big ? 0 : ws_main_bytes, big ? nullptr : counters_main, lnp, lnp_bytes, link, stream, side, ch));
   if (side && join) CHECK(lotus_streamlink_wait(link, side, stream));
   return LOTUS_OK;
+}
+
+int lotus_selfattn_bwd(const act_t* dy, const act_t* dz_in, const act_t* x, const float* g, const float* wqkv, const float* qnw,
+                       const float* qnb, const float* knw, const float* knb, const float* wp, const float* saved, act_t* dx,
+                       float* grads, float* tmp, const int* gidx, const int* owner, const int* tiles, const int* blocks, int nblocks,
+                       const int* kext, const int* ext_pos, int n_extra, int npad, int M, int C, int H, float scale, float drop_p,
+                       unsigned long long seed, float attn_p, unsigned long long attn_seed, int precision, void* ws_main,
+                       size_t ws_main_bytes, void* ws_side, size_t ws_side_bytes, void* counters_main, void* counters_side,
+                       unsigned long long link, int join, void* stream, void* side) {
+  return selfattn_bwd(dy, dz_in, x, g, wqkv, qnw, qnb, knw, knb, wp, saved, dx, grads, tmp, gidx, owner, tiles, blocks, nblocks, kext, ext_pos,
+                      n_extra, npad, M, C, H, scale, drop_p, seed, attn_p, attn_seed, precision, ws_main, ws_main_bytes, ws_side, ws_side_bytes,
+                      counters_main, counters_side, link, join, stream, side, nullptr);
 }
 
 size_t lotus_crossattn_saved_floats(int M, int C, int H, int L) {
@@ -493,9 +532,10 @@
   return a > b ? a : b;
 }
 
-int lotus_cpe_fwd(const act_t* x, const act_t* xs, const float* cw, const float* cw_packed, const float* cb, const float* lw,
-                  const float* lb, const float* g, const float* b, act_t* y, float* saved, const int* nbr27, const int* order0,
-                  const int* tap_plan, int n, int C, int precision, void* ws, size_t ws_bytes, void* ws_conv, size_t ws_conv_bytes, void* counters, void* stream) {
+static int cpe_fwd(const act_t* x, const act_t* xs, const float* cw, const float* cw_packed, const float* cb, const float* lw,
+                   const float* lb, const float* g, const float* b, act_t* y, float* saved, const int* nbr27, const int* order0,
+                   const int* tap_plan, int n, int C, int precision, void* ws, size_t ws_bytes, void* ws_conv, size_t ws_conv_bytes, void* counters, void* stream,
+                   const float* g1, const float* b1, act_t* n1, float* mean1, float* rstd1) {
   Carve sv(saved);
   act_t* c = sv.act((size_t)n * C);
   act_t* l = sv.act((size_t)n * C);
@@ -505,14 +545,22 @@
   CHECK(lotus_subm_conv(0, xs, cw, cw_packed, cb, nullptr, c, nbr27, order0, n, 27, C, C, noshadow(precision), tap_plan, ws_conv, ws_conv_bytes, stream));
   CHECK(lotus_linear_fwd(c, lw, lb, nullptr, l, nullptr, n, C, C, LOTUS_ACT_NONE, 0.f, 0, precision, big ? nullptr : ws, big ? 0 : ws_bytes,
                          big ? nullptr : counters, stream));
+  if (g1) return lotus_layernorm_fwd2(l, x, g, b, g1, b1, y, n1, mean, rstd, mean1, rstd1, n, C, 1e-5f, stream);
   return lotus_layernorm_fwd(l, x, g, b, y, mean, rstd, n, C, 1e-5f, stream);
 }
 
-int lotus_cpe_bwd(const act_t* dy, const act_t* xs, const float* cw, const float* cw_packed, const float* lw, const float* g,
-                  const float* saved, act_t* dx_conv, int add_dy, float* grads, float* tmp, const int* nbr27, const int* order0,
-                  const int* tap_plan, const long long* code0, int n_dup, int n, int C, int precision, void* ws_main, size_t ws_main_bytes, void* ws_conv,
-                  size_t ws_conv_bytes, void* ws_side, size_t ws_side_bytes, void* counters_main, void* counters_side,
-                  unsigned long long link, int join, void* stream, void* side) {
+int lotus_cpe_fwd(const act_t* x, const act_t* xs, const float* cw, const float* cw_packed, const float* cb, const float* lw,
+                  const float* lb, const float* g, const float* b, act_t* y, float* saved, const int* nbr27, const int* order0,
+                  const int* tap_plan, int n, int C, int precision, void* ws, size_t ws_bytes, void* ws_conv, size_t ws_conv_bytes, void* counters, void* stream) {
+  return cpe_fwd(x, xs, cw, cw_packed, cb, lw, lb, g, b, y, saved, nbr27, order0, tap_plan, n, C, precision, ws, ws_bytes, ws_conv, ws_conv_bytes,
+                 counters, stream, nullptr, nullptr, nullptr, nullptr, nullptr);
+}
+
+static int cpe_bwd(const act_t* dy, const act_t* xs, const float* cw, const float* cw_packed, const float* lw, const float* g,
+                   const float* saved, act_t* dx_conv, int add_dy, float* grads, float* tmp, const int* nbr27, const int* order0,
+                   const int* tap_plan, const long long* code0, int n_dup, int n, int C, int precision, void* ws_main, size_t ws_main_bytes, void* ws_conv,
+                   size_t ws_conv_bytes, void* ws_side, size_t ws_side_bytes, void* counters_main, void* counters_side,
+                   unsigned long long link, int join, void* stream, void* side, bool have_dl) {
   Carve sv(saved);
   const act_t* c = sv.act((size_t)n * C);
   const act_t* l = sv.act((size_t)n * C);
@@ -535,7 +583,8 @@
   const size_t wws_bytes = side ? ws_side_bytes : ws_main_bytes;
   void* wcnt = side ? counters_side : counters_main;
   const bool big = n > 8192;
-  if (side) {
+  if (have_dl) {
+  } else if (side) {
     PRODUCE_THEN_FORK(lotus_layernorm_bwd(dy, l, mean, rstd, g, nullptr, dl, nullptr, nullptr, n, C, 0, nullptr, 0.f, 0, lnp, lnp_bytes, stream));
     CHECK(lotus_layernorm_bwd_params(lnp, n, C, dg, db, 0, side));
   } else {
@@ -555,6 +604,15 @@
   if (n_dup != 0) CHECK(lotus_conv_dup_mask(dx_conv, add_dy ? dy : nullptr, nbr27 + (size_t)13 * n, n, C, stream));
   if (side && join) CHECK(lotus_streamlink_wait(link, side, stream));
   return LOTUS_OK;
+}
+
+int lotus_cpe_bwd(const act_t* dy, const act_t* xs, const float* cw, const float* cw_packed, const float* lw, const float* g,
+                  const float* saved, act_t* dx_conv, int add_dy, float* grads, float* tmp, const int* nbr27, const int* order0,
+                  const int* tap_plan, const long long* code0, int n_dup, int n, int C, int precision, void* ws_main, size_t ws_main_bytes, void* ws_conv,
+                  size_t ws_conv_bytes, void* ws_side, size_t ws_side_bytes, void* counters_main, void* counters_side,
+                  unsigned long long link, int join, void* stream, void* side) {
+  return cpe_bwd(dy, xs, cw, cw_packed, lw, g, saved, dx_conv, add_dy, grads, tmp, nbr27, order0, tap_plan, code0, n_dup, n, C, precision, ws_main,
+                 ws_main_bytes, ws_conv, ws_conv_bytes, ws_side, ws_side_bytes, counters_main, counters_side, link, join, stream, side, false);
 }
 
 enum PairPtr {
@@ -571,6 +629,7 @@
 enum PairInt {
   PI_M, PI_C, PI_H, PI_HD, PI_NPAD, PI_NSTILES, PI_NEXTRA, PI_L, PI_NCATILES, PI_NCABLOCKS, PI_G, PI_KMAX, PI_NDUP, PI_SAME,
   PI_PREC, PI_KV_LD, PI_DKV_LD, PI_WS_MAIN, PI_WS_SIDE, PI_WS_CONV, PI_LINK, PI_SEED_SELF, PI_SEED_FFN1, PI_SEED_CROSS, PI_SEED_FFN2,
+  PI_LNFUSE,
   PI_COUNT
 };
 enum PairFlt { PF_DROP, PF_ATTN, PF_SCALE, PF_COUNT };
@@ -630,15 +689,24 @@
   float* sv_ffn2 = sv_cross + al64(lotus_crossattn_kv_saved_floats(M, C, H));
   const unsigned long long s_self = (unsigned long long)I[PI_SEED_SELF], s_f1 = (unsigned long long)I[PI_SEED_FFN1];
   const unsigned long long s_cross = (unsigned long long)I[PI_SEED_CROSS], s_f2 = (unsigned long long)I[PI_SEED_FFN2];
-  CHECK(lotus_cpe_fwd(PPTR(const act_t*, PP_X), PPTR(const act_t*, PP_XS), PPTR(const float*, PP_CW), PPTR(const float*, PP_CWP),
-                      PPTR(const float*, PP_CB), PPTR(const float*, PP_LW), PPTR(const float*, PP_LB), PPTR(const float*, PP_G0),
-                      PPTR(const float*, PP_B0), x1, sv_cpe, PPTR(const int*, PP_NBR27), PPTR(const int*, PP_ORDER0), PPTR(const int*, PP_TAPPLAN), M, C, prec, ws, ws_b,
-                      PPTR(void*, PP_WS_CONV), (size_t)I[PI_WS_CONV], cnt, st));
-  CHECK(lotus_selfattn_fwd(x1, PPTR(const float*, PP_G1), PPTR(const float*, PP_B1), PPTR(const float*, PP_WQKV), PPTR(const float*, PP_BQKV),
-                           PPTR(const float*, PP_QNW), PPTR(const float*, PP_QNB), PPTR(const float*, PP_KNW), PPTR(const float*, PP_KNB),
-                           PPTR(const float*, PP_WP), PPTR(const float*, PP_BP), x2, sv_self, PPTR(const int*, PP_GIDX),
-                           PPTR(const int*, PP_OWNER), PPTR(const int*, PP_STILES), (int)I[PI_NSTILES], npad, M, C, H, scale, drop, s_self,
-                           attn_p, pair_mix(s_self, 1), prec, ws, ws_b, cnt, st));
+  const bool lnf = I[PI_LNFUSE] != 0;
+  Carve svs(sv_self);
+  act_t* n1 = svs.act((size_t)M * C);
+  svs.act((size_t)M * 3 * C);
+  svs.act((size_t)M * C);
+  svs.f32((size_t)npad * H);
+  float* mean1 = svs.f32(M);
+  float* rstd1 = svs.f32(M);
+  CHECK(cpe_fwd(PPTR(const act_t*, PP_X), PPTR(const act_t*, PP_XS), PPTR(const float*, PP_CW), PPTR(const float*, PP_CWP),
+                PPTR(const float*, PP_CB), PPTR(const float*, PP_LW), PPTR(const float*, PP_LB), PPTR(const float*, PP_G0),
+                PPTR(const float*, PP_B0), x1, sv_cpe, PPTR(const int*, PP_NBR27), PPTR(const int*, PP_ORDER0), PPTR(const int*, PP_TAPPLAN), M, C, prec, ws, ws_b,
+                PPTR(void*, PP_WS_CONV), (size_t)I[PI_WS_CONV], cnt, st, lnf ? PPTR(const float*, PP_G1) : nullptr, PPTR(const float*, PP_B1), n1,
+                mean1, rstd1));
+  CHECK(selfattn_fwd(x1, PPTR(const float*, PP_G1), PPTR(const float*, PP_B1), PPTR(const float*, PP_WQKV), PPTR(const float*, PP_BQKV),
+                     PPTR(const float*, PP_QNW), PPTR(const float*, PP_QNB), PPTR(const float*, PP_KNW), PPTR(const float*, PP_KNB),
+                     PPTR(const float*, PP_WP), PPTR(const float*, PP_BP), x2, sv_self, PPTR(const int*, PP_GIDX),
+                     PPTR(const int*, PP_OWNER), PPTR(const int*, PP_STILES), (int)I[PI_NSTILES], npad, M, C, H, scale, drop, s_self,
+                     attn_p, pair_mix(s_self, 1), prec, ws, ws_b, cnt, st, lnf));
   CHECK(lotus_ffn_fwd(x2, PPTR(const float*, PP_G2), PPTR(const float*, PP_B2), PPTR(const float*, PP_W1), PPTR(const float*, PP_B1F),
                       PPTR(const float*, PP_W2), PPTR(const float*, PP_B2F), x3, sv_ffn1, M, C, Hd, drop, s_f1, pair_mix(s_f1, 1), prec, ws,
                       ws_b, cnt, st));
@@ -709,15 +777,35 @@
   CHECK(lotus_ffn_bwd(d3, hand ? dz_ffn1 : nullptr, x2, PPTR(const float*, PP_G2), PPTR(const float*, PP_W1), PPTR(const float*, PP_W2), sv_ffn1,
                       d2, hand ? dz_self : nullptr, hand ? drop : 0.f, s_self, g_ffn1, t_ffn1, M, C, Hd, drop, s_f1, pair_mix(s_f1, 1), prec, wm,
                       wm_b, wsd, wsd_b, cm, cs, link, 0, st, side));
-  CHECK(lotus_selfattn_bwd(d2, hand ? dz_self : nullptr, x1, PPTR(const float*, PP_G1), PPTR(const float*, PP_WQKV), PPTR(const float*, PP_QNW),
-                           PPTR(const float*, PP_QNB), PPTR(const float*, PP_KNW), PPTR(const float*, PP_KNB), PPTR(const float*, PP_WP), sv_self,
-                           d1, g_self, t_self, PPTR(const int*, PP_GIDX), PPTR(const int*, PP_OWNER), PPTR(const int*, PP_STILES),
-                           PPTR(const int*, PP_SBLOCKS), (int)I[PI_NSTILES], PPTR(const int*, PP_KEXT), PPTR(const int*, PP_EXTPOS), n_extra, npad,
-                           M, C, H, scale, drop, s_self, attn_p, pair_mix(s_self, 1), prec, wm, wm_b, wsd, wsd_b, cm, cs, link, 0, st, side));
-  return lotus_cpe_bwd(d1, PPTR(const act_t*, PP_XS), PPTR(const float*, PP_CW), PPTR(const float*, PP_CWP), PPTR(const float*, PP_LW),
-                       PPTR(const float*, PP_G0), sv_cpe, same ? PPTR(act_t*, PP_DX) : PPTR(act_t*, PP_DXS), same, g_cpe, t_cpe,
-                       PPTR(const int*, PP_NBR27), PPTR(const int*, PP_ORDER0), PPTR(const int*, PP_TAPPLAN), PPTR(const long long*, PP_CODE0), (int)I[PI_NDUP], M, C, prec, wm,
-                       wm_b, PPTR(void*, PP_WS_CONV), (size_t)I[PI_WS_CONV], wsd, wsd_b, cm, cs, link, 0, st, side);
+  LnChain chain;
+  LnChain* ch = nullptr;
+  if (I[PI_LNFUSE] != 0) {
+    Carve svc(sv_cpe);
+    svc.act((size_t)M * C);
+    chain.l = svc.act((size_t)M * C);
+    chain.mean0 = svc.f32(M);
+    chain.rstd0 = svc.f32(M);
+    chain.g0 = PPTR(const float*, PP_G0);
+    Carve tpc(t_cpe);
+    chain.dl = tpc.act((size_t)M * C);
+    tpc.act((size_t)M * C);
+    tpc.act((size_t)M * C);
+    chain.lnp0 = tpc.f32(0);
+    chain.lnp0_bytes = lotus_layernorm_bwd_workspace(M, C);
+    chain.dg0 = g_cpe;
+    chain.db0 = g_cpe + al4(C);
+    chain.chained = 0;
+    ch = &chain;
+  }
+  CHECK(selfattn_bwd(d2, hand ? dz_self : nullptr, x1, PPTR(const float*, PP_G1), PPTR(const float*, PP_WQKV), PPTR(const float*, PP_QNW),
+                     PPTR(const float*, PP_QNB), PPTR(const float*, PP_KNW), PPTR(const float*, PP_KNB), PPTR(const float*, PP_WP), sv_self,
+                     d1, g_self, t_self, PPTR(const int*, PP_GIDX), PPTR(const int*, PP_OWNER), PPTR(const int*, PP_STILES),
+                     PPTR(const int*, PP_SBLOCKS), (int)I[PI_NSTILES], PPTR(const int*, PP_KEXT), PPTR(const int*, PP_EXTPOS), n_extra, npad,
+                     M, C, H, scale, drop, s_self, attn_p, pair_mix(s_self, 1), prec, wm, wm_b, wsd, wsd_b, cm, cs, link, 0, st, side, ch));
+  return cpe_bwd(d1, PPTR(const act_t*, PP_XS), PPTR(const float*, PP_CW), PPTR(const float*, PP_CWP), PPTR(const float*, PP_LW),
+                 PPTR(const float*, PP_G0), sv_cpe, same ? PPTR(act_t*, PP_DX) : PPTR(act_t*, PP_DXS), same, g_cpe, t_cpe,
+                 PPTR(const int*, PP_NBR27), PPTR(const int*, PP_ORDER0), PPTR(const int*, PP_TAPPLAN), PPTR(const long long*, PP_CODE0), (int)I[PI_NDUP], M, C, prec, wm,
+                 wm_b, PPTR(void*, PP_WS_CONV), (size_t)I[PI_WS_CONV], wsd, wsd_b, cm, cs, link, 0, st, side, ch && ch->chained);
 }
 #undef PPTR
 
diff --git a/robot-3dlotus_amd/csrc/gemm.hip b/robot-3dlotus_amd/csrc/gemm.hip
--- a/robot-3dlotus_amd/csrc/gemm.hip
+++ b/robot-3dlotus_amd/csrc/gemm.hip
@@ -821,6 +821,22 @@
                         act_t* dx, float* dgamma, float* dbeta, int M, int C, int accumulate, act_t* dz, float drop_p,
                         unsigned long long drop_seed, void* workspace, size_t workspace_bytes, void* stream);
 int lotus_layernorm_bwd_parts(int M, int C);
+static int dgrad_ln_epilogue(const act_t* dy, const float* w, const act_t* x, const float* mean, const float* rstd, const float* gamma,
+                             const act_t* add, act_t* dx, act_t* dz, float dz_p, unsigned long long dz_seed, int M, int N, int K,
+                             int precision, void* ln_workspace, size_t ln_workspace_bytes, void* stream) {
+  if (precision != 0 || LOTUS_ACT_IS_BF16 || (size_t)cdiv(M, 128) * 2 * K * sizeof(float) > ln_workspace_bytes) return LOTUS_GEMM_DMA_NA;
+  GemmP p;
+  memset(&p, 0, sizeof(p));
+  p.A = dy; p.B = w; p.C = dx; p.M = M; p.N = K; p.K = N;
+  p.lda = N; p.ldb = K; p.ldc = K;
+  p.act = LOTUS_ACT_NONE; p.residual = add;
+  p.klen = cdiv(N, GEMM_KALIGN) * GEMM_KALIGN;
+  p.a_vec = vec_ok(dy, N); p.b_vec = vec_ok(w, K); p.prec = 0;
+  set_drop(p, dz ? dz_p : 0.f, dz_seed);
+  p.ln_x = x; p.ln_mean = mean; p.ln_rstd = rstd; p.ln_gamma = gamma; p.ln_part = (float*)ln_workspace; p.ln_dz = dz;
+  if (!(p.a_vec && p.b_vec && vec_ok(dx, K) && vec_ok(x, K) && (!add || vec_ok(add, K)))) return LOTUS_GEMM_DMA_NA;
+  return launch_gemm_dma(p, 1, 1, (hipStream_t)stream);
+}
 int lotus_linear_dgrad_ln(const act_t* dy, const float* w, const act_t* x, const float* mean, const float* rstd, const float* gamma,
                           const act_t* add, act_t* dx, act_t* dn, act_t* dz, float dz_p, unsigned long long dz_seed, int M, int N,
                           int K, int precision, void* workspace, size_t workspace_bytes, void* counters, void* ln_workspace,
@@ -829,20 +845,9 @@
                   "lotus_linear_dgrad_ln: bad arguments");
   LOTUS_CHECK_ARG(!dz || dz_p > 0.f, "lotus_linear_dgrad_ln: dz needs dz_p > 0");
   if (M == 0) { *nparts = 0; return LOTUS_OK; }
-  if (precision == 0 && !LOTUS_ACT_IS_BF16 && (size_t)cdiv(M, 128) * 2 * K * sizeof(float) <= ln_workspace_bytes) {
-    GemmP p;
-    memset(&p, 0, sizeof(p));
-    p.A = dy; p.B = w; p.C = dx; p.M = M; p.N = K; p.K = N;
-    p.lda = N; p.ldb = K; p.ldc = K;
-    p.act = LOTUS_ACT_NONE; p.residual = add;
-    p.klen = cdiv(N, GEMM_KALIGN) * GEMM_KALIGN;
-    p.a_vec = vec_ok(dy, N); p.b_vec = vec_ok(w, K); p.prec = 0;
-    set_drop(p, dz ? dz_p : 0.f, dz_seed);
-    p.ln_x = x; p.ln_mean = mean; p.ln_rstd = rstd; p.ln_gamma = gamma; p.ln_part = (float*)ln_workspace; p.ln_dz = dz;
-    if (p.a_vec && p.b_vec && vec_ok(dx, K) && vec_ok(x, K) && (!add || vec_ok(add, K))) {
-      const int rc = launch_gemm_dma(p, 1, 1, (hipStream_t)stream);
-      if (rc != LOTUS_GEMM_DMA_NA) { *nparts = cdiv(M, 128); return rc; }
-    }
+  {
+    const int rc = dgrad_ln_epilogue(dy, w, x, mean, rstd, gamma, add, dx, dz, dz_p, dz_seed, M, N, K, precision, ln_workspace, ln_workspace_bytes, stream);
+    if (rc != LOTUS_GEMM_DMA_NA) { *nparts = cdiv(M, 128); return rc; }
   }
   StopEventOnLast stop_ev;
   int rc = lotus_linear_dgrad(dy, w, dn, nullptr, nullptr, M, N, K, LOTUS_ACT_NONE, 0.f, 0, precision, workspace, workspace_bytes, counters, stream);
@@ -851,6 +856,36 @@
   rc = lotus_layernorm_bwd(dn, x, mean, rstd, gamma, add, dx, nullptr, nullptr, M, K, 0, dz, dz ? dz_p : 0.f, dz_seed, ln_workspace,
                            ln_workspace_bytes, stream);
   *nparts = lotus_layernorm_bwd_parts(M, K);
+  return rc;
+}
+
+int lotus_layernorm_bwd2(const act_t* dn, const act_t* x1, const float* mean1, const float* rstd1, const float* g1, const act_t* add,
+                         act_t* dx1, act_t* dz, float drop_p, unsigned long long drop_seed, const act_t* l, const float* mean0,
+                         const float* rstd0, const float* g0, act_t* dl, int M, int C, void* workspace1, size_t workspace1_bytes,
+                         void* workspace0, size_t workspace0_bytes, void* stream);
+int lotus_linear_dgrad_ln2(const act_t* dy, const float* w, const act_t* x, const float* mean, const float* rstd, const float* gamma,
+                           const act_t* add, act_t* dx, act_t* dn, act_t* dz, float dz_p, unsigned long long dz_seed, const act_t* l,
+                           const float* mean0, const float* rstd0, const float* gamma0, act_t* dl, int M, int N, int K, int precision,
+                           void* workspace, size_t workspace_bytes, void* counters, void* ln_workspace, size_t ln_workspace_bytes,
+                           void* ln0_workspace, size_t ln0_workspace_bytes, int* nparts, int* chained, void* stream) {
+  LOTUS_CHECK_ARG(dy && w && x && mean && rstd && gamma && dx && dn && nparts && chained && ln_workspace && ln0_workspace && l && mean0 &&
+                      rstd0 && gamma0 && dl && M >= 0 && N > 0 && K > 0,
+                  "lotus_linear_dgrad_ln2: bad arguments");
+  LOTUS_CHECK_ARG(!dz || dz_p > 0.f, "lotus_linear_dgrad_ln2: dz needs dz_p > 0");
+  *chained = 0;
+  if (M == 0) { *nparts = 0; return LOTUS_OK; }
+  {
+    const int rc = dgrad_ln_epilogue(dy, w, x, mean, rstd, gamma, add, dx, dz, dz_p, dz_seed, M, N, K, precision, ln_workspace, ln_workspace_bytes, stream);
+    if (rc != LOTUS_GEMM_DMA_NA) { *nparts = cdiv(M, 128); return rc; }
+  }
+  StopEventOnLast stop_ev;
+  int rc = lotus_linear_dgrad(dy, w, dn, nullptr, nullptr, M, N, K, LOTUS_ACT_NONE, 0.f, 0, precision, workspace, workspace_bytes, counters, stream);
+  if (rc) return rc;
+  stop_ev.last();
+  rc = lotus_layernorm_bwd2(dn, x, mean, rstd, gamma, add, dx, dz, dz ? dz_p : 0.f, dz_seed, l, mean0, rstd0, gamma0, dl, M, K, ln_workspace,
+                            ln_workspace_bytes, ln0_workspace, ln0_workspace_bytes, stream);
+  *nparts = lotus_layernorm_bwd_parts(M, K);
+  *chained = 1;
   return rc;
 }
 
diff --git a/robot-3dlotus_amd/csrc/lotus_rename_b16.h b/robot-3dlotus_amd/csrc/lotus_rename_b16.h
--- a/robot-3dlotus_amd/csrc/lotus_rename_b16.h
+++ b/robot-3dlotus_amd/csrc/lotus_rename_b16.h
@@ -57,13 +57,16 @@
 #define lotus_ffn_ws_main_bytes lotus_b16_ffn_ws_main_bytes
 #define lotus_ffn_ws_side_bytes lotus_b16_ffn_ws_side_bytes
 #define lotus_layernorm_bwd lotus_b16_layernorm_bwd
+#define lotus_layernorm_bwd2 lotus_b16_layernorm_bwd2
 #define lotus_layernorm_bwd_params lotus_b16_layernorm_bwd_params
 #define lotus_layernorm_bwd_params_n lotus_b16_layernorm_bwd_params_n
 #define lotus_layernorm_bwd_parts lotus_b16_layernorm_bwd_parts
 #define lotus_layernorm_bwd_workspace lotus_b16_layernorm_bwd_workspace
 #define lotus_layernorm_fwd lotus_b16_layernorm_fwd
+#define lotus_layernorm_fwd2 lotus_b16_layernorm_fwd2
 #define lotus_linear_dgrad lotus_b16_linear_dgrad
 #define lotus_linear_dgrad_ln lotus_b16_linear_dgrad_ln
+#define lotus_linear_dgrad_ln2 lotus_b16_linear_dgrad_ln2
 #define lotus_linear_fwd lotus_b16_linear_fwd
 #define lotus_linear_wgrad lotus_b16_linear_wgrad
 #define lotus_linear_wgrad_workspace lotus_b16_linear_wgrad_workspace
diff --git a/robot-3dlotus_amd/csrc/norm.hip b/robot-3dlotus_amd/csrc/norm.hip
--- a/robot-3dlotus_amd/csrc/norm.hip
+++ b/robot-3dlotus_amd/csrc/norm.hip
@@ -159,6 +159,233 @@
     float s = 0.f;
     for (int r = 0; r < rpb; ++r) s += red[(long)(r * 2 + which) * p.C + col];
     p.part[((long)blockIdx.x * 2 + which) * p.C + col] = s;
+  }
+}
+
+__device__ __forceinline__ float act_rt(float v) { return LOTUS_ACT_IS_BF16 ? (float)(__bf16)v : v; }
+
+struct Ln2P {
+  const act_t* l;
+  const act_t* res;
+  const float* g0;
+  const float* b0;
+  const float* g1;
+  const float* b1;
+  act_t* y;
+  act_t* n;
+  float* mean0;
+  float* rstd0;
+  float* mean1;
+  float* rstd1;
+  int M, C, LPR, NV;
+  float eps;
+};
+
+__global__ __launch_bounds__(256) void ln_fwd2_kernel(Ln2P p) {
+  LOTUS_T_PRIO();
+  const int rpb = 256 / p.LPR;
+  const int row = blockIdx.x * rpb + threadIdx.x / p.LPR;
+  const int l = threadIdx.x % p.LPR;
+  const bool valid = row < p.M;
+  const int c4 = p.C / 4;
+  float4 v[4];
+  float s = 0.f;
+#pragma unroll
+  for (int j = 0; j < 4; ++j) {
+    v[j] = make_float4(0.f, 0.f, 0.f, 0.f);
+    const int q = l + j * p.LPR;
+    if (valid && j < p.NV && q < c4) {
+      v[j] = ld4q(p.l + (long)row * p.C, q);
+      s += v[j].x + v[j].y + v[j].z + v[j].w;
+    }
+  }
+  float mean = group_sum(s, p.LPR) / p.C;
+  float ss = 0.f;
+#pragma unroll
+  for (int j = 0; j < 4; ++j) {
+    const int q = l + j * p.LPR;
+    if (valid && j < p.NV && q < c4) {
+      const float a = v[j].x - mean, b = v[j].y - mean, c = v[j].z - mean, d = v[j].w - mean;
+      ss += a * a + b * b + c * c + d * d;
+    }
+  }
+  float rstd = rsqrtf(group_sum(ss, p.LPR) / p.C + p.eps);
+  if (valid && l == 0) {
+    p.mean0[row] = mean;
+    p.rstd0[row] = rstd;
+  }
+  s = 0.f;
+#pragma unroll
+  for (int j = 0; j < 4; ++j) {
+    const int q = l + j * p.LPR;
+    if (valid && j < p.NV && q < c4) {
+      const float4 g = ld4q(p.g0, q);
+      const float4 b = ld4q(p.b0, q);
+      float4 o;
+      o.x = (v[j].x - mean) * rstd * g.x + b.x;
+      o.y = (v[j].y - mean) * rstd * g.y + b.y;
+      o.z = (v[j].z - mean) * rstd * g.z + b.z;
+      o.w = (v[j].w - mean) * rstd * g.w + b.w;
+      const float4 r = ld4q(p.res + (long)row * p.C, q);
+      o.x += r.x; o.y += r.y; o.z += r.z; o.w += r.w;
+      st4q(p.y + (long)row * p.C, q, o);
+      v[j] = make_float4(act_rt(o.x), act_rt(o.y), act_rt(o.z), act_rt(o.w));
+      s += v[j].x + v[j].y + v[j].z + v[j].w;
+    }
+  }
+  mean = group_sum(s, p.LPR) / p.C;
+  ss = 0.f;
+#pragma unroll
+  for (int j = 0; j < 4; ++j) {
+    const int q = l + j * p.LPR;
+    if (valid && j < p.NV && q < c4) {
+      const float a = v[j].x - mean, b = v[j].y - mean, c = v[j].z - mean, d = v[j].w - mean;
+      ss += a * a + b * b + c * c + d * d;
+    }
+  }
+  rstd = rsqrtf(group_sum(ss, p.LPR) / p.C + p.eps);
+  if (!valid) return;
+  if (l == 0) {
+    p.mean1[row] = mean;
+    p.rstd1[row] = rstd;
+  }
+#pragma unroll
+  for (int j = 0; j < 4; ++j) {
+    const int q = l + j * p.LPR;
+    if (j < p.NV && q < c4) {
+      const float4 g = ld4q(p.g1, q);
+      const float4 b = ld4q(p.b1, q);
+      float4 o;
+      o.x = (v[j].x - mean) * rstd * g.x + b.x;
+      o.y = (v[j].y - mean) * rstd * g.y + b.y;
+      o.z = (v[j].z - mean) * rstd * g.z + b.z;
+      o.w = (v[j].w - mean) * rstd * g.w + b.w;
+      st4q(p.n + (long)row * p.C, q, o);
+    }
+  }
+}
+
+struct LnBwd2P {
+  LnBwdP a;
+  const act_t* l;
+  const float* mean0;
+  const float* rstd0;
+  const float* g0;
+  act_t* dl;
+  float* part0;
+};
+
+__global__ __launch_bounds__(256) void ln_bwd2_kernel(LnBwd2P pp) {
+  LOTUS_T_PRIO();
+  extern __shared__ float red[];
+  const LnBwdP& p = pp.a;
+  const int rpb = 256 / p.LPR;
+  const int rslot = threadIdx.x / p.LPR, l = threadIdx.x % p.LPR;
+  const int c4 = p.C / 4;
+  float4 pg[4], pb[4], pg0[4], pb0[4];
+#pragma unroll
+  for (int j = 0; j < 4; ++j) pg[j] = pb[j] = pg0[j] = pb0[j] = make_float4(0.f, 0.f, 0.f, 0.f);
+  for (int row0 = blockIdx.x * rpb; row0 < p.M; row0 += gridDim.x * rpb) {
+    const int row = row0 + rslot;
+    const bool valid = row < p.M;
+    const float mean = valid ? p.mean[row] : 0.f, rstd = valid ? p.rstd[row] : 0.f;
+    const float mean0 = valid ? pp.mean0[row] : 0.f, rstd0 = valid ? pp.rstd0[row] : 0.f;
+    float4 xh[4], g[4], av[4], lv[4], d[4];
+    float s1 = 0.f, s2 = 0.f;
+#pragma unroll
+    for (int j = 0; j < 4; ++j) {
+      const int q = l + j * p.LPR;
+      xh[j] = g[j] = av[j] = lv[j] = d[j] = make_float4(0.f, 0.f, 0.f, 0.f);
+      if (valid && j < p.NV && q < c4) {
+        const float4 xv = ld4q(p.x + (long)row * p.C, q);
+        const float4 dv = ld4q(p.dy + (long)row * p.C, q);
+        if (p.add) av[j] = ld4q(p.add + (long)row * p.C, q);
+        lv[j] = ld4q(pp.l + (long)row * p.C, q);
+        const float4 gm = ld4q(p.gamma, q);
+        xh[j] = make_float4((xv.x - mean) * rstd, (xv.y - mean) * rstd, (xv.z - mean) * rstd, (xv.w - mean) * rstd);
+        pg[j].x += dv.x * xh[j].x; pg[j].y += dv.y * xh[j].y; pg[j].z += dv.z * xh[j].z; pg[j].w += dv.w * xh[j].w;
+        pb[j].x += dv.x; pb[j].y += dv.y; pb[j].z += dv.z; pb[j].w += dv.w;
+        g[j] = make_float4(dv.x * gm.x, dv.y * gm.y, dv.z * gm.z, dv.w * gm.w);
+        s1 += g[j].x + g[j].y + g[j].z + g[j].w;
+        s2 += g[j].x * xh[j].x + g[j].y * xh[j].y + g[j].z * xh[j].z + g[j].w * xh[j].w;
+      }
+    }
+    s1 = group_sum(s1, p.LPR) / p.C;
+    s2 = group_sum(s2, p.LPR) / p.C;
+#pragma unroll
+    for (int j = 0; j < 4; ++j) {
+      const int q = l + j * p.LPR;
+      if (valid && j < p.NV && q < c4) {
+        float4 o;
+        o.x = rstd * (g[j].x - s1 - xh[j].x * s2);
+        o.y = rstd * (g[j].y - s1 - xh[j].y * s2);
+        o.z = rstd * (g[j].z - s1 - xh[j].z * s2);
+        o.w = rstd * (g[j].w - s1 - xh[j].w * s2);
+        o.x += av[j].x; o.y += av[j].y; o.z += av[j].z; o.w += av[j].w;
+        st4q(p.dx + (long)row * p.C, q, o);
+        d[j] = make_float4(act_rt(o.x), act_rt(o.y), act_rt(o.z), act_rt(o.w));
+        if (p.dz) {
+          const unsigned long long e = (unsigned long long)row * p.C + 4 * q;
+          float dm[4];
+          dropout_scale4(p.drop_seed, e, p.drop_thresh, p.drop_inv_keep, dm);
+          const float4 z = make_float4(o.x * dm[0], o.y * dm[1], o.z * dm[2], o.w * dm[3]);
+          st4q(p.dz + (long)row * p.C, q, z);
+        }
+      }
+    }
+    s1 = 0.f;
+    s2 = 0.f;
+#pragma unroll
+    for (int j = 0; j < 4; ++j) {
+      const int q = l + j * p.LPR;
+      xh[j] = g[j] = av[j] = make_float4(0.f, 0.f, 0.f, 0.f);
+      if (valid && j < p.NV && q < c4) {
+        const float4 xv = lv[j];
+        const float4 dv = d[j];
+        const float4 gm = ld4q(pp.g0, q);
+        xh[j] = make_float4((xv.x - mean0) * rstd0, (xv.y - mean0) * rstd0, (xv.z - mean0) * rstd0, (xv.w - mean0) * rstd0);
+        pg0[j].x += dv.x * xh[j].x; pg0[j].y += dv.y * xh[j].y; pg0[j].z += dv.z * xh[j].z; pg0[j].w += dv.w * xh[j].w;
+        pb0[j].x += dv.x; pb0[j].y += dv.y; pb0[j].z += dv.z; pb0[j].w += dv.w;
+        g[j] = make_float4(dv.x * gm.x, dv.y * gm.y, dv.z * gm.z, dv.w * gm.w);
+        s1 += g[j].x + g[j].y + g[j].z + g[j].w;
+        s2 += g[j].x * xh[j].x + g[j].y * xh[j].y + g[j].z * xh[j].z + g[j].w * xh[j].w;
+      }
+    }
+    s1 = group_sum(s1, p.LPR) / p.C;
+    s2 = group_sum(s2, p.LPR) / p.C;
+#pragma unroll
+    for (int j = 0; j < 4; ++j) {
+      const int q = l + j * p.LPR;
+      if (valid && j < p.NV && q < c4) {
+        float4 o;
+        o.x = rstd0 * (g[j].x - s1 - xh[j].x * s2);
+        o.y = rstd0 * (g[j].y - s1 - xh[j].y * s2);
+        o.z = rstd0 * (g[j].z - s1 - xh[j].z * s2);
+        o.w = rstd0 * (g[j].w - s1 - xh[j].w * s2);
+        o.x += av[j].x; o.y += av[j].y; o.z += av[j].z; o.w += av[j].w;
+        st4q(pp.dl + (long)row * p.C, q, o);
+      }
+    }
+  }
+#pragma unroll
+  for (int set = 0; set < 2; ++set) {
+    float* part = set ? pp.part0 : p.part;
+    if (set) __syncthreads();
+#pragma unroll
+    for (int j = 0; j < 4; ++j) {
+      const int q = l + j * p.LPR;
+      if (j < p.NV && q < c4) {
+        st4q(red + (long)(rslot * 2 + 0) * p.C, q, set ? pg0[j] : pg[j]);
+        st4q(red + (long)(rslot * 2 + 1) * p.C, q, set ? pb0[j] : pb[j]);
+      }
+    }
+    __syncthreads();
+    for (int c = threadIdx.x; c < 2 * p.C; c += 256) {
+      const int which = c / p.C, col = c % p.C;
+      float s = 0.f;
+      for (int r = 0; r < rpb; ++r) s += red[(long)(r * 2 + which) * p.C + col];
+      part[((long)blockIdx.x * 2 + which) * p.C + col] = s;
+    }
   }
 }
 
@@ -657,6 +884,47 @@
   return LOTUS_OK;
 }
 
+int lotus_layernorm_fwd2(const act_t* l, const act_t* res, const float* g0, const float* b0, const float* g1, const float* b1,
+                         act_t* y, act_t* n, float* mean0, float* rstd0, float* mean1, float* rstd1, int M, int C, float eps,
+                         void* stream) {
+  Ln2P p;
+  p.l = l; p.res = res; p.g0 = g0; p.b0 = b0; p.g1 = g1; p.b1 = b1; p.y = y; p.n = n;
+  p.mean0 = mean0; p.rstd0 = rstd0; p.mean1 = mean1; p.rstd1 = rstd1; p.M = M; p.C = C; p.eps = eps;
+  LOTUS_CHECK_ARG(l && res && g0 && b0 && g1 && b1 && y && n && mean0 && rstd0 && mean1 && rstd1 && M >= 0,
+                  "lotus_layernorm_fwd2: bad arguments");
+  LOTUS_CHECK_ARG(ln_geometry(C, &p.LPR, &p.NV) == 0, "lotus_layernorm_fwd2: unsupported C=%d", C);
+  if (M == 0) return LOTUS_OK;
+  LOTUS_LAUNCH(ln_fwd2_kernel, dim3(cdiv(M, 256 / p.LPR)), dim3(256), 0, (hipStream_t)stream, p);
+  LOTUS_LAUNCH_CHECK("lotus_layernorm_fwd2");
+  return LOTUS_OK;
+}
+
+int lotus_layernorm_bwd2(const act_t* dn, const act_t* x1, const float* mean1, const float* rstd1, const float* g1, const act_t* add,
+                         act_t* dx1, act_t* dz, float drop_p, unsigned long long drop_seed, const act_t* l, const float* mean0,
+                         const float* rstd0, const float* g0, act_t* dl, int M, int C, void* workspace1, size_t workspace1_bytes,
+                         void* workspace0, size_t workspace0_bytes, void* stream) {
+  LnBwd2P pp;
+  LnBwdP& p = pp.a;
+  p.dz = (dz && drop_p > 0.f) ? dz : nullptr;
+  p.drop_seed = drop_seed;
+  lotus_drop_setup(drop_p, &p.drop_thresh, &p.drop_inv_keep);
+  LOTUS_CHECK_ARG(!dz || drop_p > 0.f, "lotus_layernorm_bwd2: dz needs drop_p > 0");
+  p.dy = dn; p.x = x1; p.mean = mean1; p.rstd = rstd1; p.gamma = g1; p.add = add; p.dx = dx1;
+  p.part = (float*)workspace1; p.M = M; p.C = C;
+  pp.l = l; pp.mean0 = mean0; pp.rstd0 = rstd0; pp.g0 = g0; pp.dl = dl; pp.part0 = (float*)workspace0;
+  LOTUS_CHECK_ARG(dn && x1 && mean1 && rstd1 && g1 && dx1 && l && mean0 && rstd0 && g0 && dl && M >= 0,
+                  "lotus_layernorm_bwd2: bad arguments");
+  LOTUS_CHECK_ARG(ln_geometry_bwd(C, &p.LPR, &p.NV) == 0, "lotus_layernorm_bwd2: unsupported C=%d", C);
+  const int rpb = 256 / p.LPR;
+  const int grid = ln_bwd_grid(M, rpb);
+  const size_t need = (size_t)grid * 2 * C * sizeof(float);
+  LOTUS_CHECK_ARG(workspace1 && workspace0 && workspace1 != workspace0 && workspace1_bytes >= need && workspace0_bytes >= need,
+                  "lotus_layernorm_bwd2: workspace too small");
+  LOTUS_LAUNCH(ln_bwd2_kernel, dim3(grid), dim3(256), (size_t)rpb * 2 * C * sizeof(float), (hipStream_t)stream, pp);
+  LOTUS_LAUNCH_CHECK("lotus_layernorm_bwd2");
+  return LOTUS_OK;
+}
+
 size_t lotus_batchnorm_workspace(int M, int C) { return (size_t)BN_MAX_GRID * 2 * C * sizeof(double); }
 
 int lotus_batchnorm_stats(const act_t* x, double* sums, int M, int C, void* workspace, size_t workspace_bytes,
diff --git a/robot-3dlotus_amd/ops.py b/robot-3dlotus_amd/ops.py
--- a/robot-3dlotus_amd/ops.py
+++ b/robot-3dlotus_amd/ops.py
@@ -466,6 +466,55 @@
          _counters(x.device) if nb else None, lws, lws.numel(), int(nparts.ctypes.data))
     call("lotus_layernorm_bwd_params_n", lws, int(nparts[0]), K, dg, db, 0)
     return dx, dg, db, dz, int(nparts[0])
+
+
+def ln_fwd2(l, res, g0, b0, g1, b1, eps=1e-5):
+    M, C = l.shape
+    y, n = torch.empty_like(l), torch.empty_like(l)
+    st = [torch.empty(M, dtype=torch.float32, device=l.device) for _ in range(4)]
+    call("lotus_layernorm_fwd2", l, res, g0, b0, g1, b1, y, n, st[0], st[1], st[2], st[3], M, C, float(eps))
+    return (y, n) + tuple(st)
+
+
+def ln_bwd2(dn, x1, mean1, rstd1, g1, l, mean0, rstd0, g0, add=None, drop=None):
+    M, C = x1.shape
+    dev = x1.device
+    dx1, dl = torch.empty_like(x1), torch.empty_like(x1)
+    dz = torch.empty_like(x1) if drop else None
+    dp, dseed = drop if drop else (0.0, 0)
+    nbytes = query("lotus_layernorm_bwd_workspace", M, C)
+    w1 = torch.empty(nbytes, dtype=torch.uint8, device=dev)
+    w0 = torch.empty(nbytes, dtype=torch.uint8, device=dev)
+    call("lotus_layernorm_bwd2", dn, x1, mean1, rstd1, g1, add, dx1, dz, float(dp), int(dseed), l, mean0, rstd0, g0, dl, M, C, w1, nbytes,
+         w0, nbytes)
+    pg = [torch.empty(C, dtype=torch.float32, device=dev) for _ in range(4)]
+    call("lotus_layernorm_bwd_params", w1, M, C, pg[0], pg[1], 0)
+    call("lotus_layernorm_bwd_params", w0, M, C, pg[2], pg[3], 0)
+    return (dx1, dz, dl) + tuple(pg)
+
+
+def linear_dgrad_ln2(dy, w, x, mean, rstd, g, l, mean0, rstd0, g0, add=None, drop=None):
+    import numpy as np
+    M, N = dy.shape
+    K = w.shape[1]
+    dev = x.device
+    dx, dn, dl = torch.empty_like(x), torch.empty_like(x), torch.empty_like(x)
+    dz = torch.empty_like(x) if drop else None
+    dp, dseed = drop if drop else (0.0, 0)
+    nbytes = query("lotus_layernorm_bwd_workspace", M, K)
+    lws = torch.empty(nbytes, dtype=torch.uint8, device=dev)
+    lws0 = torch.empty(nbytes, dtype=torch.uint8, device=dev)
+    nb = query("lotus_linear_workspace", M, N, K) if M <= 8192 else 0
+    ws = WS.get(nb, dev, slot=5) if nb else None
+    out = np.zeros(2, dtype=np.int32)
+    call("lotus_linear_dgrad_ln2", dy, w, x, mean, rstd, g, add, dx, dn, dz, float(dp), int(dseed), l, mean0, rstd0, g0, dl, M, N, K,
+         _pa(None), ws, nb, _counters(dev) if nb else None, lws, nbytes, lws0, nbytes, int(out.ctypes.data), int(out.ctypes.data) + 4)
+    pg = [torch.empty(K, dtype=torch.float32, device=dev) for _ in range(4)]
+    call("lotus_layernorm_bwd_params_n", lws, int(out[0]), K, pg[0], pg[1], 0)
+    if not out[1]:
+        return dx, pg[0], pg[1], dz, False, None, None, None
+    call("lotus_layernorm_bwd_params", lws0, M, K, pg[2], pg[3], 0)
+    return dx, pg[0], pg[1], dz, True, dl, pg[2], pg[3]
 
 
 def conv_weight_t(w, prec=None):
@@ -1332,10 +1381,22 @@
              "CKNW CKNB CWP2 CBP2 G4 B4 W3 B3F W4 B4F NBR27 ORDER0 TAPPLAN CODE0 GIDX OWNER STILES SBLOCKS KEXT EXTPOS CATILES CABLOCKS WS_MAIN "
              "WS_SIDE WS_CONV CNT_MAIN CNT_SIDE STREAM SIDE DY DX DXS DKV GRADS TMP").split()
 _PI_NAMES = ("M C H HD NPAD NSTILES NEXTRA L NCATILES NCABLOCKS G KMAX NDUP SAME PREC KV_LD DKV_LD WS_MAIN WS_SIDE WS_CONV LINK SEED_SELF "
-             "SEED_FFN1 SEED_CROSS SEED_FFN2").split()
+             "SEED_FFN1 SEED_CROSS SEED_FFN2 LNFUSE").split()
 _PAIR_PARAM_SLOTS = ("CW CB LW LB G0 B0 G1 B1 WQKV BQKV QNW QNB KNW KNB WP BP G2 B2 W1 B1F W2 B2F G3 B3 WQ BQ CQNW CQNB CKNW CKNB CWP2 CBP2 "
                      "G4 B4 W3 B3F W4 B4F").split()
 _PAIR_LINEAR = (2, 8, 14, 18, 20, 24, 30, 34, 36)
+
+
+_LN_FUSION = True
+
+
+def set_ln_fusion(on):
+    global _LN_FUSION
+    _LN_FUSION = bool(on)
+
+
+def ln_fusion_enabled():
+    return _LN_FUSION and not _capi.BF16
 
 
 def pair_enabled(rows, rows0=None):
@@ -1419,7 +1480,8 @@
                       ("NEXTRA", lvl.n_extra), ("L", L), ("NCATILES", lvl_ca.n_ca_tiles), ("NCABLOCKS", lvl_ca.n_ca_blocks),
                       ("G", lvl_ca.ca_groups), ("KMAX", lvl_ca.ca_kmax), ("NDUP", lvl.n_dup & 0xFFFFFFFF), ("SAME", 1 if same else 0),
                       ("PREC", pc), ("KV_LD", kv.stride(0)), ("WS_MAIN", ws.numel()), ("WS_CONV", wc.numel()),
-                      ("SEED_SELF", s_self), ("SEED_FFN1", s_f1), ("SEED_CROSS", s_cross), ("SEED_FFN2", s_f2)):
+                      ("SEED_SELF", s_self), ("SEED_FFN1", s_f1), ("SEED_CROSS", s_cross), ("SEED_FFN2", s_f2),
+                      ("LNFUSE", 1 if ln_fusion_enabled() else 0)):
             I[PI[k]] = v_
         F = np.array([float(drop_p), float(attn_p), float((C // H) ** -0.5)], dtype=np.float64)
         _capi.call_raw("lotus_pair_fwd", P.ctypes.data, I.ctypes.data, F.ctypes.data)
```
